# 4l3x4ndre/Metadata-Augmented-UNET-for-LST-NDVI

Hardware: AMD Instinct MI355X
Metric: train images/sec (256x256x6->2 U-Net, B=32/GPU) (higher is better)
Workload: dtype bf16; 1 GPU; metadata-unet base_filters=64, 32x6x256x256 tiles + 4-dim metadata per GPU, fwd+MSE+bwd+AdamW (src/train.py:243-256); global_batch=32, parallelism=dp1, sync_bn=False, launch=hipGraph replay of the captured step

## Files before the change

### include/mau_hip.h

```cpp
#ifndef MAU_HIP_H
#define MAU_HIP_H

#include <stddef.h>
#include <stdint.h>

#ifdef __cplusplus
extern "C" {
#endif

#define MAU_F32 0
#define MAU_BF16 1
#define MAU_F16 2

#define MAU_OK 0
#define MAU_ERR_ARG 1
#define MAU_ERR_HIP 2
#define MAU_ERR_DEVICE 3

typedef void* mau_stream_t;

#define MAU_ABI_VERSION 5
int mau_abi_version(void);
const char* mau_last_error(void);
int mau_device_check(void);

int mau_nchw_to_nhwc(const float* src, void* dst, int dtype, int N, int C, int H, int W, int ld,
                     mau_stream_t stream);
int mau_nhwc_to_nchw(const void* src, float* dst, int dtype, int N, int C, int H, int W, int ld,
                     mau_stream_t stream);

int mau_pack_tile_onehot(const unsigned char* cls_a, const unsigned char* cls_b, const float* cont,
                         const unsigned char* flip, void* out, int ldo, int dtype, int N, int H, int W,
                         int num_classes, int ncont, mau_stream_t stream);
int mau_flip_rows(const float* src, float* dst, const unsigned char* flip, int N, int C, int H, int W,
                  mau_stream_t stream);

int mau_conv3x3_kc(int dtype);
size_t mau_conv3x3_packed_elems(int dtype, int nout, int nin);
int mau_conv3x3_pack_weights(const float* w_oihw, void* wf, void* wd, int dtype, int Cout, int Cin,
                             mau_stream_t stream);
size_t mau_conv3x3_pack_desc_bytes(void);
int mau_conv3x3_pack_desc_fill(void* descs_host, int index, const float* w_oihw, void* wf, void* wd, int dtype, int Cout,
                               int Cin, int tile0, int* next_tile_host);
int mau_conv3x3_pack_weights_multi(const void* descs, int n, int total_tiles, int dtype, mau_stream_t stream);
int mau_conv3x3_num_pixel_tiles(int dtype, int N, int H, int W, int Cout);
int mau_conv3x3_fwd_pool(const void* x, int ldx, int C0, const void* wpk, const float* bias, const float* post_scale,
                         const float* post_shift, void* y, int ldy, int Cout, void* pooled, int ldpool, int dtype, int N, int H,
                         int W, mau_stream_t stream);
int mau_conv3x3_variant(int dtype, int N, int H, int W, int Cin, int Cout, int* tile_rows_host, int* waves_host, int* cout_block_host,
                        int* k_groups_host);
int mau_conv3x3_first_max_channels(void);
int mau_conv3x3_first_rows(int N, int H, int W);
size_t mau_conv3x3_first_wgrad_ws_elems(int N, int H, int W, int Cout);
int mau_conv3x3_first_wgrad(const void* x8, const void* dz, int lddz, float* dw_oihw, float* ws, int Cin, int Cout, int dtype, int N,
                            int H, int W, mau_stream_t stream);
int mau_conv3x3_first_fwd(const float* x_nchw, int Cin, const float* w_oihw, const float* bias, const float* post_scale,
                          const float* post_shift, void* y, int ldy, int Cout, float* slab, void* x8, int dtype, int N, int H,
                          int W, mau_stream_t stream);
int mau_conv3x3_fwd(const void* x, int ldx, int C0, const float* emb, void* emb_ws, int E, const void* wpk,
                    const float* bias, const float* post_scale, const float* post_shift, void* y, int ldy,
                    int Cout, float* slab, int dtype, int N, int H, int W, mau_stream_t stream);
int mau_conv3x3_fwd2(const void* x, int ldx, int C0, const void* x1, int ldx1, int C1, const float* emb, void* emb_ws,
                     int E, const void* wpk, const float* bias, const float* post_scale, const float* post_shift,
                     void* y, int ldy, int Cout, float* slab, int dtype, int N, int H, int W, mau_stream_t stream);
int mau_conv3x3_wgrad_splits(int dtype, int N, int H, int W, int Cout, int Cin);
size_t mau_conv3x3_wgrad_acc_elems(int dtype, int N, int H, int W, int Cout, int Cin);
int mau_conv3x3_wgrad(const void* x, int ldx, int C0, const float* emb, void* emb_ws, int E, const void* dy,
                      int lddy, int Cout, float* acc, int dtype, int N, int H, int W, mau_stream_t stream);
int mau_conv3x3_wgrad2(const void* x, int ldx, int C0, const void* x1, int ldx1, int C1, const float* emb, void* emb_ws,
                       int E, const void* dy, int lddy, int Cout, float* acc, int dtype, int N, int H, int W,
                       mau_stream_t stream);
int mau_conv3x3_unpack_wgrad(const float* acc, int nsplit, float* dw_oihw, int Cout, int Cin,
                             mau_stream_t stream);

size_t mau_reduce_rows_ws_elems(int rows, int M);
int mau_reduce_tickets_elems(void);
int mau_reduce_rows_f64(const float* slab, int rows, int M, int ldrow, double* sums, double* ws, unsigned* tickets,
                        mau_stream_t stream);
int mau_reduce_rows_f64_f32(const float* slab, int rows, int M, int ldrow, double* sums, float* sums32,
                            double* ws, unsigned* tickets, double append, mau_stream_t stream);
int mau_reduce_rows_f32(const float* slab, int rows, int M, int ldrow, float* out, double* ws, unsigned* tickets,
                        mau_stream_t stream);
int mau_bn_stats_sums_f64(const float* slab, int rows, int C, double* sums, double* ws, unsigned* tickets, double append,
                          mau_stream_t stream);
int mau_bn_finalize_train(const double* sums, double count, const float* gamma, const float* beta,
                          float* running_mean, float* running_var, int64_t* num_batches_tracked,
                          float momentum, float eps, float* scale, float* shift, float* mean,
                          float* invstd, int C, mau_stream_t stream);
size_t mau_bn_stats_ws_elems(int rows, int C);
int mau_bn_stats_finalize_train(const float* slab, int rows, double count, const float* gamma, const float* beta,
                                float* running_mean, float* running_var, int64_t* num_batches_tracked,
                                float momentum, float eps, float* scale, float* shift, float* mean, float* invstd,
                                double* ws, unsigned* tickets, int C, mau_stream_t stream);
int mau_bn_coeffs_eval(const float* gamma, const float* beta, const float* running_mean,
                       const float* running_var, float eps, float* scale, float* shift, float* mean,
                       float* invstd, int C, mau_stream_t stream);
int mau_bn_relu_apply(const void* y, int ldy, const float* scale, const float* shift, void* a, int lda,
                      int dtype, int64_t npix, int C, mau_stream_t stream);
int mau_bn_relu_apply_pool(const void* y, int ldy, const float* scale, const float* shift, void* a, int lda,
                           void* pooled, int ldp, unsigned short* argidx, int dtype, int N, int H, int W, int C,
                           mau_stream_t stream);
int mau_bn_relu_bwd_reduce(const void* da, int ldda, const void* y, int ldy, const float* scale,
                           const float* shift, const float* mean, const float* invstd, float* slab,
                           int ldslab, int dtype, int64_t npix, int C, mau_stream_t stream);
int mau_bn_relu_bwd_apply(const void* da, int ldda, const void* y, int ldy, const float* scale,
                          const float* shift, const float* mean, const float* invstd, const double* sums,
                          double count, void* dy, int lddy, int dtype, int64_t npix, int C,
                          mau_stream_t stream);
int mau_bn_bwd_rows(int64_t npix);

int mau_pool_bn_bwd_reduce(const void* y, int ldy, const void* dpl, int lddpl, const unsigned short* argidx,
                           const void* dskip, int lddskip,
                           const float* scale, const float* shift, const float* mean, const float* invstd, float* slab,
                           int ldslab, int dtype, int N, int H, int W, int C, mau_stream_t stream);
int mau_pool_bn_bwd_apply(const void* y, int ldy, const void* dpl, int lddpl, const unsigned short* argidx,
                          const void* dskip, int lddskip,
                          const float* scale, const float* shift, const float* mean, const float* invstd,
                          const double* sums, double count, void* dy, int lddy, int dtype, int N, int H, int W, int C,
                          mau_stream_t stream);
int mau_head_bn_max_channels(void);
int mau_head_bn_fwd(const void* y, int ldy, const float* scale, const float* shift, const float* w, const float* b, float* out,
                    int tanh0, int dtype, int N, int HW, int C, int Co, mau_stream_t stream);
int mau_head_bn_bwd_reduce(const void* y, int ldy, const float* scale, const float* shift, const float* mean,
                           const float* invstd, const float* w, const float* out, const float* dout, float* bn_slab,
                           int ldslab, float* head_slab, int tanh0, int dtype, int N, int HW, int C, int Co,
                           mau_stream_t stream);
int mau_head_bn_bwd_apply(const void* y, int ldy, const float* scale, const float* shift, const float* mean,
                          const float* invstd, const double* sums, double count, const float* w, const float* out,
                          const float* dout, void* dy, int lddy, int tanh0, int dtype, int N, int HW, int C, int Co,
                          mau_stream_t stream);

int mau_sum_tensors_max(void);
int mau_sum_tensors(const void* const* srcs, const int* lds, int k, void* dst, int lddst, int dtype, int64_t npix, int C,
                    mau_stream_t stream);

int mau_emb_fold_fwd(const float* w, const float* emb, float* weff, int Cout, int Ct, int E, int N, int Ep, mau_stream_t stream);
size_t mau_emb_fold_ws_elems(int Cout, int N, int E);
int mau_emb_fold_bwd(const float* w, const float* emb, const float* dweff, float* dw, float* demb, float* ws, int Cout, int Ct, int E,
                     int N, int Ep, mau_stream_t stream);

int mau_maxpool2x2_fwd(const void* x, int ldx, void* y, int ldy, int dtype, int N, int H, int W, int C,
                       mau_stream_t stream);
int mau_maxpool2x2_bwd(const void* x, int ldx, const void* dy, int lddy, void* dx, int lddx, int dtype,
                       int N, int H, int W, int C, mau_stream_t stream);
int mau_maxpool2x2_bwd_add(const void* x, int ldx, const void* dy, int lddy, const void* dskip, int lddskip, void* dx,
                           int lddx, int dtype, int N, int H, int W, int C, mau_stream_t stream);

int mau_resize_bilinear_fwd(const void* src, int ldsrc, int h, int w, void* dst, int lddst, int choff,
                            int dtype, int N, int H, int W, int C, mau_stream_t stream);
int mau_resize_bilinear_bn_fwd(const void* y, int ldy, int h, int w, const float* scale, const float* shift, void* dst,
                               int lddst, int choff, int dtype, int N, int H, int W, int C, mau_stream_t stream);
int mau_resize_bilinear_bwd(const void* ddst, int ldddst, int choff, int H, int W, void* dsrc, int lddsrc,
                            int dtype, int N, int h, int w, int C, mau_stream_t stream);
int mau_copy_channels(const void* src, int ldsrc, void* dst, int lddst, int choff, int zero_to, int dtype,
                      int64_t npix, int C, mau_stream_t stream);
int mau_bcast_fill(const float* emb, void* dst, int lddst, int choff, int zero_to, int dtype, int N, int HW,
                   int E, mau_stream_t stream);
size_t mau_bcast_bwd_ws_elems(int N, int HW, int E);
int mau_bcast_bwd(const void* dx, int lddx, int choff, float* demb, float* ws, int dtype, int N, int HW, int E,
                  mau_stream_t stream);

int mau_head_fwd(const void* a, int lda, const float* w, const float* b, float* out, int tanh0, int dtype,
                 int N, int HW, int C, int Co, mau_stream_t stream);
size_t mau_head_mean_ws_elems(int N, int HW, int Co);
int mau_head_mean(const void* a, int lda, const float* w, const float* b, const double* scale, const double* shift,
                  double* means, double* ws, unsigned* tickets, int tanh0, int dtype, int N, int HW, int C, int Co,
                  mau_stream_t stream);
int mau_head_bwd(const void* a, int lda, const float* w, const float* out, const float* dout, void* da,
                 int ldda, float* slab, int tanh0, int dtype, int N, int HW, int C, int Co,
                 mau_stream_t stream);
int mau_head_bwd_rows(int N, int HW);
int mau_head_bwd_rowlen(int C, int Co);

int mau_meta_mlp_fwd(const float* md, const float* w0, const float* b0, const float* w2, const float* b2,
                     float* hidden, float* emb, int N, int F, int Hd, int D, mau_stream_t stream);
int mau_meta_mlp_bwd(const float* md, const float* w0, const float* w2, const float* hidden,
                     const float* demb, float* dw0, float* db0, float* dw2, float* db2, float* dhidden_ws,
                     int N, int F, int Hd, int D, mau_stream_t stream);

int mau_lstm_max_hidden(void);
int mau_lstm_fwd(const float* x, const float* w_ih, const float* w_hh, const float* b_ih, const float* b_hh,
                 float* h_last, float* gates, float* cells, int B, int T, int H, mau_stream_t stream);
size_t mau_lstm_bwd_ws_elems(int B, int T, int H);
int mau_lstm_bwd(const float* x, const float* w_hh, const float* gates, const float* cells, const float* dh_last,
                 float* dw_ih, float* dw_hh, float* db_ih, float* db_hh, float* ws, int B, int T, int H,
                 mau_stream_t stream);

int mau_linear_fwd(const float* x, const float* w, const float* b, float* out, int N, int F, int D, mau_stream_t stream);
int mau_linear_bwd(const float* x, const float* w, const float* dout, float* dx, float* dw, float* db, int N, int F,
                   int D, mau_stream_t stream);

size_t mau_adamw_pack_desc_bytes(void);
int mau_adamw_pack_desc_fill(void* descs_host, int index, float* w, const float* grad, float* exp_avg, float* exp_avg_sq,
                             void* wf, void* wd, int Cout, int Cin, int tile0, int* next_tile_host);
int mau_adamw_pack_step(const void* descs, int n, int total_tiles, int dtype, const float* step, float lr, float beta1,
                        float beta2, float eps, float weight_decay, mau_stream_t stream);

#define MAU_OPT_ADAMW 0
#define MAU_OPT_ADAM 1
#define MAU_OPT_SGD 2
int mau_opt_pack_desc_fill(void* descs_host, int index, float* w, const float* grad, float* m, float* v, void* wf, void* wd,
                           int Cout, int Cin, int tile0, int* next_tile_host);
int mau_opt_pack_step(const void* descs, int n, int total_tiles, int dtype, int rule, const float* step, const float* grad_scale,
                      float lr, float beta1_or_momentum, float beta2, float eps, float weight_decay, int nesterov,
                      mau_stream_t stream);

int mau_grad_norm_chunk(void);
size_t mau_grad_norm_seg_bytes(void);
int mau_grad_norm_seg_fill(void* segs_host, int index, const float* ptr, int64_t n, int block0, int* next_block_host);
int mau_grad_norm_clip(const void* segs, int nsegs, int total_blocks, double* ws, unsigned* tickets, float max_norm,
                       float* norm_out, float* coef_out, mau_stream_t stream);

int mau_eval_metrics_row_elems(int ncls);
int mau_eval_metrics_chunks(int H, int W);
size_t mau_eval_metrics_ws_elems(int B, int C, int H, int W, int ncls);
int mau_eval_metrics(const float* out, const float* tgt, const unsigned char* cls, const double* scale, const double* shift,
                     double* rows, double* ws, unsigned* tickets, int B, int C, int H, int W, int ncls, mau_stream_t stream);

int mau_mse_blocks(int64_t n);
int mau_mse_fwd_bwd(const float* out, const float* tgt, double* partial, float* loss, float* dout, int64_t n,
                    mau_stream_t stream);

int mau_l1_gradient_blocks(int64_t n);
int mau_l1_gradient_loss(const float* out, const float* tgt, double* partial, float* terms, float* dout, float w_l1,
                         float w_grad, int B, int C, int H, int W, mau_stream_t stream);

size_t mau_ssim_ws_elems(int B, int C, int H, int W);
int mau_ssim_loss(const float* out, const float* tgt, double* ws, float* per_image, float* loss, int prep, int B, int C,
                  int H, int W, mau_stream_t stream);

#ifdef __cplusplus
}
#endif
#endif
```

### metadata-augmented-unet-for-lst-ndvi_amd/_lib.py

```python
from __future__ import annotations

import ctypes as C
import os

import torch

_HERE = os.path.dirname(os.path.abspath(__file__))
LIB_PATH = os.environ.get("MAU_LIB") or os.path.join(_HERE, "libmau_hip.so")

MAU_F32 = 0
MAU_BF16 = 1
MAU_F16 = 2
MAU_OPT_ADAMW, MAU_OPT_ADAM, MAU_OPT_SGD = 0, 1, 2

_p, _i, _i64, _f, _d, _sz = C.c_void_p, C.c_int, C.c_int64, C.c_float, C.c_double, C.c_size_t

PROTOTYPES = {
    "mau_abi_version": (_i, []),
    "mau_last_error": (C.c_char_p, []),
    "mau_device_check": (_i, []),
    "mau_nchw_to_nhwc": (_i, [_p, _p, _i, _i, _i, _i, _i, _i, _p]),
    "mau_pack_tile_onehot": (_i, [_p, _p, _p, _p, _p, _i, _i, _i, _i, _i, _i, _i, _p]),
    "mau_flip_rows": (_i, [_p, _p, _p, _i, _i, _i, _i, _p]),
    "mau_nhwc_to_nchw": (_i, [_p, _p, _i, _i, _i, _i, _i, _i, _p]),
    "mau_conv3x3_kc": (_i, [_i]),
    "mau_conv3x3_packed_elems": (_sz, [_i, _i, _i]),
    "mau_conv3x3_pack_weights": (_i, [_p, _p, _p, _i, _i, _i, _p]),
    "mau_conv3x3_pack_desc_bytes": (_sz, []),
    "mau_conv3x3_pack_desc_fill": (_i, [_p, _i, _p, _p, _p, _i, _i, _i, _i, _p]),
    "mau_conv3x3_pack_weights_multi": (_i, [_p, _i, _i, _i, _p]),
    "mau_conv3x3_num_pixel_tiles": (_i, [_i, _i, _i, _i, _i]),
    "mau_conv3x3_variant": (_i, [_i, _i, _i, _i, _i, _i, _p, _p, _p, _p]),
    "mau_conv3x3_first_max_channels": (_i, []),
    "mau_conv3x3_first_rows": (_i, [_i, _i, _i]),
    "mau_conv3x3_first_wgrad_ws_elems": (_sz, [_i, _i, _i, _i]),
    "mau_conv3x3_first_wgrad": (_i, [_p, _p, _i, _p, _p, _i, _i, _i, _i, _i, _i, _p]),
    "mau_conv3x3_first_fwd": (_i, [_p, _i, _p, _p, _p, _p, _p, _i, _i, _p, _p, _i, _i, _i, _i, _p]),
    "mau_conv3x3_fwd": (_i, [_p, _i, _i, _p, _p, _i, _p, _p, _p, _p, _p, _i, _i, _p, _i, _i, _i, _i, _p]),
    "mau_conv3x3_fwd_pool": (_i, [_p, _i, _i, _p, _p, _p, _p, _p, _i, _i, _p, _i, _i, _i, _i, _i, _p]),
    "mau_conv3x3_fwd2": (_i, [_p, _i, _i, _p, _i, _i, _p, _p, _i, _p, _p, _p, _p, _p, _i, _i, _p, _i, _i, _i, _i, _p]),
    "mau_conv3x3_wgrad_splits": (_i, [_i, _i, _i, _i, _i, _i]),
    "mau_conv3x3_wgrad_acc_elems": (_sz, [_i, _i, _i, _i, _i, _i]),
    "mau_conv3x3_wgrad": (_i, [_p, _i, _i, _p, _p, _i, _p, _i, _i, _p, _i, _i, _i, _i, _p]),
    "mau_conv3x3_wgrad2": (_i, [_p, _i, _i, _p, _i, _i, _p, _p, _i, _p, _i, _i, _p, _i, _i, _i, _i, _p]),
    "mau_conv3x3_unpack_wgrad": (_i, [_p, _i, _p, _i, _i, _p]),
    "mau_reduce_rows_ws_elems": (_sz, [_i, _i]),
    "mau_reduce_tickets_elems": (_i, []),
    "mau_reduce_rows_f64": (_i, [_p, _i, _i, _i, _p, _p, _p, _p]),
    "mau_reduce_rows_f64_f32": (_i, [_p, _i, _i, _i, _p, _p, _p, _p, _d, _p]),
    "mau_reduce_rows_f32": (_i, [_p, _i, _i, _i, _p, _p, _p, _p]),
    "mau_bn_stats_sums_f64": (_i, [_p, _i, _i, _p, _p, _p, _d, _p]),
    "mau_bn_finalize_train": (_i, [_p, _d, _p, _p, _p, _p, _p, _f, _f, _p, _p, _p, _p, _i, _p]),
    "mau_bn_stats_ws_elems": (_sz, [_i, _i]),
    "mau_bn_stats_finalize_train": (_i, [_p, _i, _d, _p, _p, _p, _p, _p, _f, _f, _p, _p, _p, _p, _p, _p, _i, _p]),
    "mau_bn_coeffs_eval": (_i, [_p, _p, _p, _p, _f, _p, _p, _p, _p, _i, _p]),
    "mau_bn_relu_apply": (_i, [_p, _i, _p, _p, _p, _i, _i, _i64, _i, _p]),
    "mau_bn_relu_apply_pool": (_i, [_p, _i, _p, _p, _p, _i, _p, _i, _p, _i, _i, _i, _i, _i, _p]),
    "mau_bn_relu_bwd_reduce": (_i, [_p, _i, _p, _i, _p, _p, _p, _p, _p, _i, _i, _i64, _i, _p]),
    "mau_bn_relu_bwd_apply": (_i, [_p, _i, _p, _i, _p, _p, _p, _p, _p, _d, _p, _i, _i, _i64, _i, _p]),
    "mau_bn_bwd_rows": (_i, [_i64]),
    "mau_pool_bn_bwd_reduce": (_i, [_p, _i, _p, _i, _p, _p, _i, _p, _p, _p, _p, _p, _i, _i, _i, _i, _i, _i, _p]),
    "mau_pool_bn_bwd_apply": (_i, [_p, _i, _p, _i, _p, _p, _i, _p, _p, _p, _p, _p, _d, _p, _i, _i, _i, _i, _i, _i, _p]),
    "mau_head_bn_max_channels": (_i, []),
    "mau_head_bn_fwd": (_i, [_p, _i, _p, _p, _p, _p, _p, _i, _i, _i, _i, _i, _i, _p]),
    "mau_head_bn_bwd_reduce": (_i, [_p, _i, _p, _p, _p, _p, _p, _p, _p, _p, _i, _p, _i, _i, _i, _i, _i, _i, _p]),
    "mau_head_bn_bwd_apply": (_i, [_p, _i, _p, _p, _p, _p, _p, _d, _p, _p, _p, _p, _i, _i, _i, _i, _i, _i, _i, _p]),
    "mau_resize_bilinear_bn_fwd": (_i, [_p, _i, _i, _i, _p, _p, _p, _i, _i, _i, _i, _i, _i, _i, _p]),
    "mau_maxpool2x2_fwd": (_i, [_p, _i, _p, _i, _i, _i, _i, _i, _i, _p]),
    "mau_maxpool2x2_bwd": (_i, [_p, _i, _p, _i, _p, _i, _i, _i, _i, _i, _i, _p]),
    "mau_maxpool2x2_bwd_add": (_i, [_p, _i, _p, _i, _p, _i, _p, _i, _i, _i, _i, _i, _i, _p]),
    "mau_resize_bilinear_fwd": (_i, [_p, _i, _i, _i, _p, _i, _i, _i, _i, _i, _i, _i, _p]),
    "mau_resize_bilinear_bwd": (_i, [_p, _i, _i, _i, _i, _p, _i, _i, _i, _i, _i, _i, _p]),
    "mau_copy_channels": (_i, [_p, _i, _p, _i, _i, _i, _i, _i64, _i, _p]),
    "mau_bcast_fill": (_i, [_p, _p, _i, _i, _i, _i, _i, _i, _i, _p]),
    "mau_bcast_bwd_ws_elems": (_sz, [_i, _i, _i]),
    "mau_bcast_bwd": (_i, [_p, _i, _i, _p, _p, _i, _i, _i, _i, _p]),
    "mau_head_fwd": (_i, [_p, _i, _p, _p, _p, _i, _i, _i, _i, _i, _i, _p]),
    "mau_head_mean_ws_elems": (_sz, [_i, _i, _i]),
    "mau_head_mean": (_i, [_p, _i, _p, _p, _p, _p, _p, _p, _p, _i, _i, _i, _i, _i, _i, _p]),
    "mau_head_bwd": (_i, [_p, _i, _p, _p, _p, _p, _i, _p, _i, _i, _i, _i, _i, _i, _p]),
    "mau_head_bwd_rows": (_i, [_i, _i]),
    "mau_head_bwd_rowlen": (_i, [_i, _i]),
    "mau_meta_mlp_fwd": (_i, [_p, _p, _p, _p, _p, _p, _p, _i, _i, _i, _i, _p]),
    "mau_meta_mlp_bwd": (_i, [_p, _p, _p, _p, _p, _p, _p, _p, _p, _p, _i, _i, _i, _i, _p]),
    "mau_lstm_max_hidden": (_i, []),
    "mau_lstm_fwd": (_i, [_p, _p, _p, _p, _p, _p, _p, _p, _i, _i, _i, _p]),
    "mau_lstm_bwd_ws_elems": (_sz, [_i, _i, _i]),
    "mau_lstm_bwd": (_i, [_p, _p, _p, _p, _p, _p, _p, _p, _p, _p, _i, _i, _i, _p]),
    "mau_linear_fwd": (_i, [_p, _p, _p, _p, _i, _i, _i, _p]),
    "mau_linear_bwd": (_i, [_p, _p, _p, _p, _p, _p, _i, _i, _i, _p]),
    "mau_adamw_pack_desc_bytes": (_sz, []),
    "mau_adamw_pack_desc_fill": (_i, [_p, _i, _p, _p, _p, _p, _p, _p, _i, _i, _i, _p]),
    "mau_adamw_pack_step": (_i, [_p, _i, _i, _i, _p, _f, _f, _f, _f, _f, _p]),
    "mau_opt_pack_desc_fill": (_i, [_p, _i, _p, _p, _p, _p, _p, _p, _i, _i, _i, _p]),
    "mau_opt_pack_step": (_i, [_p, _i, _i, _i, _i, _p, _p, _f, _f, _f, _f, _f, _i, _p]),
    "mau_grad_norm_chunk": (_i, []),
    "mau_grad_norm_seg_bytes": (_sz, []),
    "mau_grad_norm_seg_fill": (_i, [_p, _i, _p, _i64, _i, _p]),
    "mau_grad_norm_clip": (_i, [_p, _i, _i, _p, _p, _f, _p, _p, _p]),
    "mau_sum_tensors_max": (_i, []),
    "mau_sum_tensors": (_i, [_p, _p, _i, _p, _i, _i, _i64, _i, _p]),
    "mau_emb_fold_fwd": (_i, [_p, _p, _p, _i, _i, _i, _i, _i, _p]),
    "mau_emb_fold_ws_elems": (_sz, [_i, _i, _i]),
    "mau_emb_fold_bwd": (_i, [_p, _p, _p, _p, _p, _p, _i, _i, _i, _i, _i, _p]),
    "mau_eval_metrics_row_elems": (_i, [_i]),
    "mau_eval_metrics_chunks": (_i, [_i, _i]),
    "mau_eval_metrics_ws_elems": (_sz, [_i, _i, _i, _i, _i]),
    "mau_eval_metrics": (_i, [_p, _p, _p, _p, _p, _p, _p, _p, _i, _i, _i, _i, _i, _p]),
    "mau_mse_blocks": (_i, [_i64]),
    "mau_l1_gradient_blocks": (_i, [_i64]),
    "mau_l1_gradient_loss": (_i, [_p, _p, _p, _p, _p, _f, _f, _i, _i, _i, _i, _p]),
    "mau_ssim_ws_elems": (_sz, [_i, _i, _i, _i]),
    "mau_ssim_loss": (_i, [_p, _p, _p, _p, _p, _i, _i, _i, _i, _i, _p]),
    "mau_mse_fwd_bwd": (_i, [_p, _p, _p, _p, _p, _i64, _p]),
}


class MauError(RuntimeError):
    pass


def _load():
    if not os.path.exists(LIB_PATH):
        raise ImportError(
            f"{LIB_PATH} not found: the MI355X-native HIP library has not been built "
            f"(run `python -c 'import __graft_entry__ as g; g.build()'` or `make -C {os.path.join(_HERE, 'csrc')}`). "
            "There is no CPU or PyTorch fallback for this path.")
    lib = C.CDLL(LIB_PATH)
    missing = [n for n in PROTOTYPES if not hasattr(lib, n)]
    if missing:
        raise ImportError(f"{LIB_PATH} does not export {missing}; rebuild it")
    for name, (res, args) in PROTOTYPES.items():
        fn = getattr(lib, name)
        fn.restype = res
        fn.argtypes = args
    return lib


lib = _load()


def check(status: int, what: str = ""):
    if status != 0:
        msg = lib.mau_last_error()
        raise MauError(f"libmau_hip {what} failed (status {status}): {msg.decode() if msg else '?'}")


def conv3x3_variant(dtype: int, N: int, H: int, W: int, Cout: int, Cin: int = 0):
    th, nw, bn, kg = C.c_int(), C.c_int(), C.c_int(), C.c_int()
    check(lib.mau_conv3x3_variant(dtype, N, H, W, Cin, Cout, C.byref(th), C.byref(nw), C.byref(bn), C.byref(kg)), "mau_conv3x3_variant")
    return th.value, nw.value, bn.value, kg.value


def call(name: str, *args):
    check(getattr(lib, name)(*args), name)
```

### metadata-augmented-unet-for-lst-ndvi_amd/csrc/bn.hip

```cpp
#include <stdlib.h>
#include "mau_common.h"

namespace mau {

template <int G, typename Load>
__device__ __forceinline__ void ordered_group(int& k, int end, Load load, double& s0, double& s1) {
  for (; k + 8 * (G - 1) + 4 < end; k += 8 * G) {
    double a[G], b[G];
#pragma unroll
    for (int i = 0; i < G; ++i) {
      a[i] = load(k + 8 * i);
      b[i] = load(k + 8 * i + 4);
    }
#pragma unroll
    for (int i = 0; i < G; ++i) {
      s0 += a[i];
      s1 += b[i];
    }
  }
}
template <typename Load>
__device__ __forceinline__ void ordered_pair_sum(int first, int end, Load load, double& s0, double& s1) {
  int k = first;
#ifndef MAU_REDUCE_SERIAL
  ordered_group<16>(k, end, load, s0, s1);
  ordered_group<4>(k, end, load, s0, s1);
#endif
  for (; k + 4 < end; k += 8) {
    s0 += load(k);
    s1 += load(k + 4);
  }
  if (k < end) s0 += load(k);
}

template <typename InT, typename OutT>
__global__ __launch_bounds__(256) void reduce_rows_kernel(const InT* __restrict__ slab, int rows, int M, int ldrow,
                                                          OutT* __restrict__ out, int ldout, float* __restrict__ out32) {
  __shared__ double part[4][64];
  const int col = blockIdx.x * 64 + (threadIdx.x & 63);
  const int rl = threadIdx.x >> 6;
  const int per = (rows + gridDim.y - 1) / gridDim.y;
  const int r0 = blockIdx.y * per, r1 = min(rows, r0 + per);
  double s0 = 0.0, s1 = 0.0;
  if (col < M) {
    if (r0 + rl < r1) ordered_pair_sum(r0 + rl, r1, [&](int r) { return (double)slab[(size_t)r * ldrow + col]; }, s0, s1);
  }
  part[rl][threadIdx.x & 63] = s0 + s1;
  __syncthreads();
  if (rl == 0 && col < M) {
    const double v = part[0][threadIdx.x] + part[1][threadIdx.x] + part[2][threadIdx.x] + part[3][threadIdx.x];
    out[(size_t)blockIdx.y * ldout + col] = (OutT)v;
    if (out32 != nullptr) out32[col] = (float)v;
  }
}

constexpr int REDUCE_MAX_CHUNKS = 128;
static int reduce_chunks(int rows) {
  int c = rows / 32;
  if (c > REDUCE_MAX_CHUNKS) c = REDUCE_MAX_CHUNKS;
  return c < 1 ? 1 : c;
}

template <typename OutT>
static int reduce_rows_launch(const float* slab, int rows, int M, int ldrow, OutT* out, double* ws, hipStream_t st,
                              float* out32 = nullptr) {
  const int chunks = reduce_chunks(rows);
  float* const none = nullptr;
  if (chunks == 1 || ws == nullptr) {
    MAU_LAUNCH((reduce_rows_kernel<float, OutT>), dim3(ceil_div(M, 64), 1), dim3(256), 0, st, slab, rows, M, ldrow, out, M, out32);
  } else {
    MAU_LAUNCH((reduce_rows_kernel<float, double>), dim3(ceil_div(M, 64), chunks), dim3(256), 0, st, slab, rows, M, ldrow, ws, M, none);
    MAU_LAUNCH((reduce_rows_kernel<double, OutT>), dim3(ceil_div(M, 64), 1), dim3(256), 0, st, (const double*)ws, chunks, M, M, out, M, out32);
  }
  return check_launch("reduce_rows_kernel");
}


template <typename OutT>
__global__ __launch_bounds__(256) void reduce_rows_fused_kernel(const float* __restrict__ slab, int rows, int M, int ldrow, int split,
                                                                int gap, double* __restrict__ part, unsigned* __restrict__ tickets,
                                                                OutT* __restrict__ out, float* __restrict__ out32, double append) {
  __shared__ double ps[4][64];
  const int cl = threadIdx.x & 63, rl = threadIdx.x >> 6;
  const int j = blockIdx.x * 64 + cl;
  const int col = j < split ? j : j - split + gap;
  const int chunks = gridDim.y;
  const int per = (rows + chunks - 1) / chunks;
  const int r0 = blockIdx.y * per, r1 = min(rows, r0 + per);
  double s0 = 0.0, s1 = 0.0;
  if (j < M) {
    if (r0 + rl < r1) ordered_pair_sum(r0 + rl, r1, [&](int r) { return (double)slab[(size_t)r * ldrow + col]; }, s0, s1);
  }
  ps[rl][cl] = s0 + s1;
  __syncthreads();
  if (rl == 0 && j < M) part[(size_t)blockIdx.y * M + j] = ps[0][cl] + ps[1][cl] + ps[2][cl] + ps[3][cl];
  if (!last_block_of(tickets + blockIdx.x, (unsigned)chunks)) return;
  s0 = s1 = 0.0;
  if (j < M) {
    if (rl < chunks) ordered_pair_sum(rl, chunks, [&](int k) { return part[(size_t)k * M + j]; }, s0, s1);
  }
  ps[rl][cl] = s0 + s1;
  __syncthreads();
  if (rl == 0 && j < M) {
    const double v = ps[0][cl] + ps[1][cl] + ps[2][cl] + ps[3][cl];
    out[j] = (OutT)v;
    if (out32 != nullptr) out32[j] = (float)v;
  }
  if (append > 0.0 && blockIdx.x == 0 && threadIdx.x == 0) out[M] = (OutT)append;
}

template <typename OutT>
static int reduce_rows_fused_launch(const float* slab, int rows, int M, int ldrow, int split, int gap, OutT* out, double* ws,
                                    unsigned* tickets, hipStream_t st, float* out32 = nullptr, double append = 0.0) {
  const int chunks = reduce_chunks(rows);
  MAU_LAUNCH((reduce_rows_fused_kernel<OutT>), dim3(ceil_div(M, 64), chunks), dim3(256), 0, st, slab, rows, M, ldrow, split, gap, ws,
             tickets, out, out32, append);
  return check_launch("reduce_rows_fused_kernel");
}

__global__ void bn_finalize_train_kernel(const double* __restrict__ sums, double count, const float* __restrict__ gamma,
                                         const float* __restrict__ beta, float* __restrict__ rmean, float* __restrict__ rvar,
                                         int64_t* nbt, float momentum, float eps, float* __restrict__ scale,
                                         float* __restrict__ shift, float* __restrict__ mean_o, float* __restrict__ invstd_o,
                                         int C) {
  const int c = blockIdx.x * blockDim.x + threadIdx.x;
  if (c == 0 && nbt) *nbt += 1;
  if (c >= C) return;
  if (count <= 0.0) count = sums[2 * C];
  const double mean = sums[c] / count;
  double var = sums[C + c] / count - mean * mean;
  if (var < 0.0) var = 0.0;
  const float invstd = (float)(1.0 / sqrt(var + (double)eps));
  const float sc = gamma[c] * invstd;
  scale[c] = sc;
  shift[c] = beta[c] - (float)mean * sc;
  mean_o[c] = (float)mean;
  invstd_o[c] = invstd;
  if (rmean) {
    const double unbiased = count > 1.0 ? var * (count / (count - 1.0)) : var;
    rmean[c] = (1.f - momentum) * rmean[c] + momentum * (float)mean;
    rvar[c] = (1.f - momentum) * rvar[c] + momentum * (float)unbiased;
  }
}

__global__ __launch_bounds__(256) void bn_finalize_from_partials_kernel(const double* __restrict__ part, int chunks, int ldp, double count,
                                                 const float* __restrict__ gamma, const float* __restrict__ beta,
                                                 float* __restrict__ rmean, float* __restrict__ rvar, int64_t* nbt, float momentum,
                                                 float eps, float* __restrict__ scale, float* __restrict__ shift,
                                                 float* __restrict__ mean_o, float* __restrict__ invstd_o, int C) {
  __shared__ double ps[4][64], pq[4][64];
  const int cl = threadIdx.x & 63, kl = threadIdx.x >> 6;
  const int c = blockIdx.x * 64 + cl;
  if (blockIdx.x == 0 && threadIdx.x == 0 && nbt) *nbt += 1;
  double s0 = 0.0, q0 = 0.0, s1 = 0.0, q1 = 0.0;
  if (c < C && kl < chunks) {
    ordered_pair_sum(kl, chunks, [&](int k) { return part[(size_t)k * 2 * ldp + c]; }, s0, s1);
    ordered_pair_sum(kl, chunks, [&](int k) { return part[(size_t)k * 2 * ldp + ldp + c]; }, q0, q1);
  }
  ps[kl][cl] = s0 + s1;
  pq[kl][cl] = q0 + q1;
  __syncthreads();
  if (kl != 0 || c >= C) return;
  const double s = (ps[0][cl] + ps[1][cl]) + (ps[2][cl] + ps[3][cl]);
  const double q = (pq[0][cl] + pq[1][cl]) + (pq[2][cl] + pq[3][cl]);
  const double mean = s / count;
  double var = q / count - mean * mean;
  if (var < 0.0) var = 0.0;
  const float invstd = (float)(1.0 / sqrt(var + (double)eps));
  const float sc = gamma[c] * invstd;
  scale[c] = sc;
  shift[c] = beta[c] - (float)mean * sc;
  mean_o[c] = (float)mean;
  invstd_o[c] = invstd;
  if (rmean) {
    const double unbiased = count > 1.0 ? var * (count / (count - 1.0)) : var;
    rmean[c] = (1.f - momentum) * rmean[c] + momentum * (float)mean;
    rvar[c] = (1.f - momentum) * rvar[c] + momentum * (float)unbiased;
  }
}

__global__ __launch_bounds__(256) void bn_stats_finalize_fused_kernel(const float* __restrict__ slab, int rows, int cpad,
                                                                      double* __restrict__ part, unsigned* __restrict__ tickets,
                                                                      double count, const float* __restrict__ gamma,
                                                                      const float* __restrict__ beta, float* __restrict__ rmean,
                                                                      float* __restrict__ rvar, int64_t* nbt, float momentum,
                                                                      float eps, float* __restrict__ scale, float* __restrict__ shift,
                                                                      float* __restrict__ mean_o, float* __restrict__ invstd_o, int C) {
  __shared__ double ps[4][64], pq[4][64];
  const int cl = threadIdx.x & 63, kl = threadIdx.x >> 6;
  const int c = blockIdx.x * 64 + cl;
  const int chunks = gridDim.y, ld = 2 * cpad;
  const int per = (rows + chunks - 1) / chunks;
  const int r0 = blockIdx.y * per, r1 = min(rows, r0 + per);
  double s0 = 0.0, q0 = 0.0, s1 = 0.0, q1 = 0.0;
  if (r0 + kl < r1) {
    ordered_pair_sum(r0 + kl, r1, [&](int r) { return (double)slab[(size_t)r * ld + c]; }, s0, s1);
    ordered_pair_sum(r0 + kl, r1, [&](int r) { return (double)slab[(size_t)r * ld + cpad + c]; }, q0, q1);
  }
  ps[kl][cl] = s0 + s1;
  pq[kl][cl] = q0 + q1;
  __syncthreads();
  if (kl == 0) {
    part[(size_t)blockIdx.y * ld + c] = ps[0][cl] + ps[1][cl] + ps[2][cl] + ps[3][cl];
    part[(size_t)blockIdx.y * ld + cpad + c] = pq[0][cl] + pq[1][cl] + pq[2][cl] + pq[3][cl];
  }
  if (!last_block_of(tickets + blockIdx.x, (unsigned)chunks)) return;
  if (blockIdx.x == 0 && threadIdx.x == 0 && nbt) *nbt += 1;
  s0 = q0 = s1 = q1 = 0.0;
  if (c < C && kl < chunks) {
    ordered_pair_sum(kl, chunks, [&](int k) { return part[(size_t)k * ld + c]; }, s0, s1);
    ordered_pair_sum(kl, chunks, [&](int k) { return part[(size_t)k * ld + cpad + c]; }, q0, q1);
  }
  ps[kl][cl] = s0 + s1;
  pq[kl][cl] = q0 + q1;
  __syncthreads();
  if (kl != 0 || c >= C) return;
  const double s = (ps[0][cl] + ps[1][cl]) + (ps[2][cl] + ps[3][cl]);
  const double q = (pq[0][cl] + pq[1][cl]) + (pq[2][cl] + pq[3][cl]);
  const double mean = s / count;
  double var = q / count - mean * mean;
  if (var < 0.0) var = 0.0;
  const float invstd = (float)(1.0 / sqrt(var + (double)eps));
  const float sc = gamma[c] * invstd;
  scale[c] = sc;
  shift[c] = beta[c] - (float)mean * sc;
  mean_o[c] = (float)mean;
  invstd_o[c] = invstd;
  if (rmean) {
    const double unbiased = count > 1.0 ? var * (count / (count - 1.0)) : var;
    rmean[c] = (1.f - momentum) * rmean[c] + momentum * (float)mean;
    rvar[c] = (1.f - momentum) * rvar[c] + momentum * (float)unbiased;
  }
}

__global__ void bn_coeffs_eval_kernel(const float* __restrict__ gamma, const float* __restrict__ beta,
                                      const float* __restrict__ rmean, const float* __restrict__ rvar, float eps,
                                      float* __restrict__ scale, float* __restrict__ shift, float* __restrict__ mean_o,
                                      float* __restrict__ invstd_o, int C) {
  const int c = blockIdx.x * blockDim.x + threadIdx.x;
  if (c >= C) return;
  const float is = 1.f / sqrtf(rvar[c] + eps);
  const float sc = gamma[c] * is;
  scale[c] = sc;
  shift[c] = beta[c] - rmean[c] * sc;
  if (mean_o) mean_o[c] = rmean[c];
  if (invstd_o) invstd_o[c] = is;
}

struct PixVec {
  int nvl, PS, v, ps;
  __device__ __forceinline__ PixVec(int nv) {
    nvl = nv < 256 ? nv : 256;
    PS = 256 / nvl;
    v = threadIdx.x % nvl;
    ps = threadIdx.x / nvl;
  }
};
static inline int pixvec_pixels_per_block(int nv, int64_t npix, int max_per_thread, int min_blocks = 2048) {
  const int nvl = nv < 256 ? nv : 256;
  const int ps = 256 / nvl;
  int per_thread = max_per_thread;
  while (per_thread > 8 && npix / ((int64_t)ps * per_thread) < min_blocks) per_thread >>= 1;
  return ps * per_thread;
}

template <typename T>
__global__ __launch_bounds__(256) void bn_relu_apply_kernel(const T* __restrict__ y, int ldy, const float* __restrict__ scale,
                                                            const float* __restrict__ shift, T* __restrict__ a, int lda,
                                                            int64_t npix, int C, int C8, int pixb) {
  const int nv = C8 >> 3;
  const PixVec m(nv);
  if (m.ps >= m.PS) return;
  const int64_t p0 = (int64_t)blockIdx.x * pixb;
  const int64_t p1 = p0 + pixb < npix ? p0 + pixb : npix;
  for (int vv = m.v; vv < nv; vv += m.nvl) {
    const int c = vv * 8;
    float sc[8], sh[8];
#pragma unroll
    for (int j = 0; j < 8; ++j) {
      sc[j] = coef(scale, c + j, C);
      sh[j] = coef(shift, c + j, C);
    }
    int64_t pix = p0 + m.ps;
    for (; pix + 3 * m.PS < p1; pix += 4 * m.PS) {
      F8 v[4];
#pragma unroll
      for (int u = 0; u < 4; ++u) v[u] = load8<T>(y + (pix + u * m.PS) * ldy + c);
#pragma unroll
      for (int u = 0; u < 4; ++u) {
        F8 o;
#pragma unroll
        for (int j = 0; j < 8; ++j) o.v[j] = fmaxf(fmaf(v[u].v[j], sc[j], sh[j]), 0.f);
        store8<T>(a + (pix + u * m.PS) * lda + c, o);
      }
    }
    for (; pix < p1; pix += m.PS) {
      const F8 v = load8<T>(y + pix * ldy + c);
      F8 o;
#pragma unroll
      for (int j = 0; j < 8; ++j) o.v[j] = fmaxf(fmaf(v.v[j], sc[j], sh[j]), 0.f);
      store8<T>(a + pix * lda + c, o);
    }
  }
}

template <typename T>
__global__ __launch_bounds__(256) void bn_relu_apply_pool_kernel(const T* __restrict__ y, int ldy, const float* __restrict__ scale,
                                                                 const float* __restrict__ shift, T* __restrict__ a, int lda,
                                                                 T* __restrict__ pl, int ldp, unsigned short* __restrict__ argidx, int H, int W,
                                                                 int C, int C8) {
  const int nv = C8 >> 3, Wc = (W + 1) >> 1, Ho = H >> 1, Wo = W >> 1;
  const int idx = blockIdx.x * 256 + threadIdx.x;
  if (idx >= Wc * nv) return;
  const int xo = idx / nv, c = (idx - xo * nv) * 8;
  const int yo = blockIdx.y, n = blockIdx.z;
  float sc[8], sh[8];
#pragma unroll
  for (int j = 0; j < 8; ++j) {
    sc[j] = coef(scale, c + j, C);
    sh[j] = coef(shift, c + j, C);
  }
  const int y0 = 2 * yo, x0 = 2 * xo;
  const bool hasx = x0 + 1 < W, hasy = y0 + 1 < H;
  const size_t row0 = ((size_t)n * H + y0) * W, row1 = row0 + W;
  F8 v[4];
  v[0] = load8<T>(y + (row0 + x0) * ldy + c);
  v[1] = hasx ? load8<T>(y + (row0 + x0 + 1) * ldy + c) : zero8();
  v[2] = hasy ? load8<T>(y + (row1 + x0) * ldy + c) : zero8();
  v[3] = (hasx && hasy) ? load8<T>(y + (row1 + x0 + 1) * ldy + c) : zero8();
  F8 o[4];
#pragma unroll
  for (int u = 0; u < 4; ++u)
#pragma unroll
    for (int j = 0; j < 8; ++j) o[u].v[j] = fmaxf(fmaf(v[u].v[j], sc[j], sh[j]), 0.f);
  store8<T>(a + (row0 + x0) * lda + c, o[0]);
  if (hasx) store8<T>(a + (row0 + x0 + 1) * lda + c, o[1]);
  if (hasy) store8<T>(a + (row1 + x0) * lda + c, o[2]);
  if (hasx && hasy) store8<T>(a + (row1 + x0 + 1) * lda + c, o[3]);
  if (yo < Ho && xo < Wo) {
    F8 m;
    unsigned bits = 0;
#pragma unroll
    for (int j = 0; j < 8; ++j) {
      const float a0 = opaque((float)(T)opaque(o[0].v[j])), a1 = opaque((float)(T)opaque(o[1].v[j]));
      const float a2 = opaque((float)(T)opaque(o[2].v[j])), a3 = opaque((float)(T)opaque(o[3].v[j]));
      unsigned arg = 0;
      float mx = a0;
      arg = a1 > mx ? 1u : arg;
      mx = fmaxf(mx, a1);
      arg = a2 > mx ? 2u : arg;
      mx = fmaxf(mx, a2);
      arg = a3 > mx ? 3u : arg;
      mx = fmaxf(mx, a3);
      m.v[j] = mx;
      bits |= arg << (2 * j);
    }
    store8<T>(pl + (((size_t)n * Ho + yo) * Wo + xo) * ldp + c, m);
    if (argidx != nullptr) argidx[(((size_t)n * Ho + yo) * Wo + xo) * nv + (c >> 3)] = (unsigned short)bits;
  }
}


template <typename T>
__global__ __launch_bounds__(256) void bn_relu_bwd_reduce_kernel(const T* __restrict__ da, int ldda, const T* __restrict__ y,
                                                                 int ldy, const float* __restrict__ scale,
                                                                 const float* __restrict__ shift, const float* __restrict__ mean,
                                                                 const float* __restrict__ invstd, float* __restrict__ slab,
                                                                 int ldslab, int64_t npix, int C) {
  __shared__ float red[2][32][64 + 1];
  const int cv = threadIdx.x & 7, ps = threadIdx.x >> 3;
  const int c0 = blockIdx.y * 64 + cv * 8;
  const int64_t p0 = (int64_t)blockIdx.x * BWD_PIX_PER_BLOCK;
  const int64_t p1 = p0 + BWD_PIX_PER_BLOCK < npix ? p0 + BWD_PIX_PER_BLOCK : npix;
  float s1[8], s2[8], sc[8], sh[8], mu[8], is[8];
#pragma unroll
  for (int j = 0; j < 8; ++j) {
    s1[j] = s2[j] = 0.f;
    const int cc = c0 + j;
    sc[j] = coef(scale, cc, C);
    sh[j] = coef(shift, cc, C);
    mu[j] = coef(mean, cc, C);
    is[j] = coef(invstd, cc, C);
  }
  if (c0 < C) {
    int64_t p = p0 + ps;
    for (; p + 32 < p1; p += 64) {
      F8 g[2], v[2];
#pragma unroll
      for (int u = 0; u < 2; ++u) {
        g[u] = load8<T>(da + (p + 32 * u) * ldda + c0);
        v[u] = load8<T>(y + (p + 32 * u) * ldy + c0);
      }
#pragma unroll
      for (int u = 0; u < 2; ++u)
#pragma unroll
        for (int j = 0; j < 8; ++j) {
          const float act = fmaf(v[u].v[j], sc[j], sh[j]);
          const float dz = act > 0.f ? g[u].v[j] : 0.f;
          s1[j] += dz;
          s2[j] = fmaf(dz, (v[u].v[j] - mu[j]) * is[j], s2[j]);
        }
    }
    for (; p < p1; p += 32) {
      const F8 g = load8<T>(da + p * ldda + c0);
      const F8 v = load8<T>(y + p * ldy + c0);
#pragma unroll
      for (int j = 0; j < 8; ++j) {
        const float act = fmaf(v.v[j], sc[j], sh[j]);
        const float dz = act > 0.f ? g.v[j] : 0.f;
        s1[j] += dz;
        s2[j] = fmaf(dz, (v.v[j] - mu[j]) * is[j], s2[j]);
      }
    }
  }
#pragma unroll
  for (int j = 0; j < 8; ++j) {
    red[0][ps][cv * 8 + j] = s1[j];
    red[1][ps][cv * 8 + j] = s2[j];
  }
  __syncthreads();
  if (threadIdx.x < 128) {
    const int which = threadIdx.x >> 6, c = threadIdx.x & 63;
    float s = 0.f;
#pragma unroll 8
    for (int r = 0; r < 32; ++r) s += red[which][r][c];
    const int cc = blockIdx.y * 64 + c;
    if (cc < ldslab) slab[((size_t)blockIdx.x * 2 + which) * ldslab + cc] = s;
  }
}

template <typename T, bool NT>
__global__ __launch_bounds__(256) void bn_relu_bwd_apply_kernel(const T* __restrict__ da, int ldda, const T* __restrict__ y,
                                                                int ldy, const float* __restrict__ scale,
                                                                const float* __restrict__ shift, const float* __restrict__ mean,
                                                                const float* __restrict__ invstd, const double* __restrict__ sums,
                                                                double inv_count, T* __restrict__ dy, int lddy, int64_t npix,
                                                                int C, int C8, int pixb) {
  const int nv = C8 >> 3;
  const PixVec m(nv);
  if (m.ps >= m.PS) return;
  if (inv_count <= 0.0) inv_count = 1.0 / sums[2 * C];
  const int64_t p0 = (int64_t)blockIdx.x * pixb;
  const int64_t p1 = p0 + pixb < npix ? p0 + pixb : npix;
  for (int vv = m.v; vv < nv; vv += m.nvl) {
    const int c = vv * 8;
    float sc[8], sh[8], k0[8], k1[8];
    double d1[8], d2[8];
#pragma unroll
    for (int j = 0; j < 8; ++j) {
      sc[j] = coef(scale, c + j, C);
      sh[j] = coef(shift, c + j, C);
      k0[j] = coef(mean, c + j, C);
      k1[j] = coef(invstd, c + j, C);
      d1[j] = coef(sums, c + j, C);
      d2[j] = coef(sums + C, c + j, C);
    }
#pragma unroll
    for (int j = 0; j < 8; ++j) {
      const float mu = k0[j], is = k1[j];
      const float m1 = (float)(d1[j] * inv_count), m2 = (float)(d2[j] * inv_count);
      k1[j] = __fmul_rn(__fmul_rn(sc[j], m2), is);
      k0[j] = fmaf(sc[j], m1, -__fmul_rn(k1[j], mu));
    }
    int64_t pix = p0 + m.ps;
    for (; pix + 3 * m.PS < p1; pix += 4 * m.PS) {
      F8 g[4], v[4];
#pragma unroll
      for (int u = 0; u < 4; ++u) {
        g[u] = NT ? load8_nt<T>(da + (pix + u * m.PS) * ldda + c) : load8<T>(da + (pix + u * m.PS) * ldda + c);
        v[u] = NT ? load8_nt<T>(y + (pix + u * m.PS) * ldy + c) : load8<T>(y + (pix + u * m.PS) * ldy + c);
      }
#pragma unroll
      for (int u = 0; u < 4; ++u) {
        F8 o;
#pragma unroll
        for (int j = 0; j < 8; ++j) {
          const float act = fmaf(v[u].v[j], sc[j], sh[j]);
          const float dz = act > 0.f ? g[u].v[j] : 0.f;
          o.v[j] = fmaf(sc[j], dz, -fmaf(k1[j], v[u].v[j], k0[j]));
        }
        if (NT) store8_nt<T>(dy + (pix + u * m.PS) * lddy + c, o); else store8<T>(dy + (pix + u * m.PS) * lddy + c, o);
      }
    }
    for (; pix < p1; pix += m.PS) {
      const F8 g = load8<T>(da + pix * ldda + c);
      const F8 v = load8<T>(y + pix * ldy + c);
      F8 o;
#pragma unroll
      for (int j = 0; j < 8; ++j) {
        const float act = fmaf(v.v[j], sc[j], sh[j]);
        const float dz = act > 0.f ? g.v[j] : 0.f;
        o.v[j] = fmaf(sc[j], dz, -fmaf(k1[j], v.v[j], k0[j]));
      }
      store8<T>(dy + pix * lddy + c, o);
    }
  }
}

}

using namespace mau;

extern "C" {

size_t mau_reduce_rows_ws_elems(int rows, int M) { return (size_t)reduce_chunks(rows) * M; }

int mau_reduce_tickets_elems(void) { return 64; }

#define MAU_REQUIRE_TICKETS(M) MAU_REQUIRE(tickets == nullptr || ceil_div((M), 64) <= mau_reduce_tickets_elems(), "reduce_rows: more than 4096 columns")

int mau_reduce_rows_f64(const float* slab, int rows, int M, int ldrow, double* sums, double* ws, unsigned* tickets,
                        mau_stream_t stream) {
  MAU_REQUIRE(slab && sums && rows > 0 && M > 0 && ldrow >= M, "reduce_rows: bad arguments");
  MAU_REQUIRE_TICKETS(M);
  if (tickets && ws) return reduce_rows_fused_launch<double>(slab, rows, M, ldrow, M, 0, sums, ws, tickets, (hipStream_t)stream);
  return reduce_rows_launch<double>(slab, rows, M, ldrow, sums, ws, (hipStream_t)stream);
}

int mau_reduce_rows_f64_f32(const float* slab, int rows, int M, int ldrow, double* sums, float* sums32, double* ws,
                            unsigned* tickets, double append, mau_stream_t stream) {
  MAU_REQUIRE(slab && sums && sums32 && rows > 0 && M > 0 && ldrow >= M, "reduce_rows: bad arguments");
  MAU_REQUIRE_TICKETS(M);
  MAU_REQUIRE(append <= 0.0 || (tickets && ws), "reduce_rows: the appended count needs the single-launch form (ws and tickets)");
  if (tickets && ws)
    return reduce_rows_fused_launch<double>(slab, rows, M, ldrow, M, 0, sums, ws, tickets, (hipStream_t)stream, sums32, append);
  return reduce_rows_launch<double>(slab, rows, M, ldrow, sums, ws, (hipStream_t)stream, sums32);
}

int mau_reduce_rows_f32(const float* slab, int rows, int M, int ldrow, float* out, double* ws, unsigned* tickets,
                        mau_stream_t stream) {
  MAU_REQUIRE(slab && out && rows > 0 && M > 0 && ldrow >= M, "reduce_rows: bad arguments");
  MAU_REQUIRE_TICKETS(M);
  if (tickets && ws) return reduce_rows_fused_launch<float>(slab, rows, M, ldrow, M, 0, out, ws, tickets, (hipStream_t)stream);
  return reduce_rows_launch<float>(slab, rows, M, ldrow, out, ws, (hipStream_t)stream);
}

int mau_bn_stats_sums_f64(const float* slab, int rows, int C, double* sums, double* ws, unsigned* tickets, double append,
                          mau_stream_t stream) {
  MAU_REQUIRE(slab && sums && ws && tickets && rows > 0 && C > 0, "bn_stats_sums: bad arguments");
  MAU_REQUIRE_TICKETS(2 * C);
  const int cpad = round_up(C, 64);
  return reduce_rows_fused_launch<double>(slab, rows, 2 * C, 2 * cpad, C, cpad, sums, ws, tickets, (hipStream_t)stream, nullptr, append);
}

int mau_bn_finalize_train(const double* sums, double count, const float* gamma, const float* beta,
                          float* running_mean, float* running_var, int64_t* nbt, float momentum, float eps,
                          float* scale, float* shift, float* mean, float* invstd, int C, mau_stream_t stream) {
  MAU_REQUIRE(sums && gamma && beta && scale && shift && mean && invstd && C > 0 && count >= 0, "bn_finalize_train: bad arguments");
  MAU_REQUIRE((running_mean == nullptr) == (running_var == nullptr), "bn_finalize_train: running_mean/var must come together");
  MAU_LAUNCH(bn_finalize_train_kernel, dim3(ceil_div(C, 256)), dim3(256), 0, (hipStream_t)stream, sums, count, gamma,
                     beta, running_mean, running_var, nbt, momentum, eps, scale, shift, mean, invstd, C);
  return check_launch("bn_finalize_train_kernel");
}

size_t mau_bn_stats_ws_elems(int rows, int C) { return (size_t)reduce_chunks(rows) * 2 * round_up(C, 64); }

int mau_bn_stats_finalize_train(const float* slab, int rows, double count, const float* gamma, const float* beta,
                                float* running_mean, float* running_var, int64_t* nbt, float momentum, float eps,
                                float* scale, float* shift, float* mean, float* invstd, double* ws, unsigned* tickets, int C,
                                mau_stream_t stream) {
  MAU_REQUIRE(slab && ws && gamma && beta && scale && shift && mean && invstd && rows > 0 && C > 0 && count > 0, "bn_stats_finalize_train: bad arguments");
  MAU_REQUIRE((running_mean == nullptr) == (running_var == nullptr), "bn_stats_finalize_train: running_mean/var must come together");
  hipStream_t st = (hipStream_t)stream;
  const int cpad = round_up(C, 64), M = 2 * cpad, chunks = reduce_chunks(rows);
  MAU_REQUIRE_TICKETS(cpad);
  if (tickets) {
    MAU_LAUNCH(bn_stats_finalize_fused_kernel, dim3(cpad / 64, chunks), dim3(256), 0, st, slab, rows, cpad, ws, tickets, count, gamma,
               beta, running_mean, running_var, nbt, momentum, eps, scale, shift, mean, invstd, C);
    return check_launch("bn_stats_finalize_fused_kernel");
  }
  MAU_LAUNCH((reduce_rows_kernel<float, double>), dim3(ceil_div(M, 64), chunks), dim3(256), 0, st, slab, rows, M, M, ws, M, (float*)nullptr);
  MAU_LAUNCH(bn_finalize_from_partials_kernel, dim3(ceil_div(C, 64)), dim3(256), 0, st, (const double*)ws, chunks, cpad, count, gamma,
             beta, running_mean, running_var, nbt, momentum, eps, scale, shift, mean, invstd, C);
  return check_launch("bn_stats_finalize_train");
}

int mau_bn_coeffs_eval(const float* gamma, const float* beta, const float* running_mean, const float* running_var,
                       float eps, float* scale, float* shift, float* mean, float* invstd, int C, mau_stream_t stream) {
  MAU_REQUIRE(gamma && beta && running_mean && running_var && scale && shift && C > 0, "bn_coeffs_eval: bad arguments");
  MAU_LAUNCH(bn_coeffs_eval_kernel, dim3(ceil_div(C, 256)), dim3(256), 0, (hipStream_t)stream, gamma, beta,
                     running_mean, running_var, eps, scale, shift, mean, invstd, C);
  return check_launch("bn_coeffs_eval_kernel");
}

int mau_bn_relu_apply(const void* y, int ldy, const float* scale, const float* shift, void* a, int lda, int dtype,
                      int64_t npix, int C, mau_stream_t stream) {
  MAU_REQUIRE(y && a && scale && shift && npix > 0 && C > 0, "bn_relu_apply: bad arguments");
  const int C8 = round_up(C, 8);
  MAU_REQUIRE(ldy % 8 == 0 && lda % 8 == 0 && ldy >= C8 && lda >= C8, "bn_relu_apply: bad ld");
  const bool big = npix >= (int64_t)1 << 20;
  const int pixb = pixvec_pixels_per_block(C8 / 8, npix, big ? 8 : 32, big ? 2048 : 256);
  MAU_DISPATCH_DTYPE(dtype, MAU_LAUNCH(bn_relu_apply_kernel<T>, dim3(ceil_div(npix, pixb)), dim3(256), 0, (hipStream_t)stream,
                                               (const T*)y, ldy, scale, shift, (T*)a, lda, npix, C, C8, pixb));
  return check_launch("bn_relu_apply_kernel");
}

int mau_bn_relu_apply_pool(const void* y, int ldy, const float* scale, const float* shift, void* a, int lda, void* pooled,
                           int ldp, unsigned short* argidx, int dtype, int N, int H, int W, int C, mau_stream_t stream) {
  MAU_REQUIRE(y && a && pooled && scale && shift && N > 0 && H >= 2 && W >= 2 && C > 0, "bn_relu_apply_pool: bad arguments");
  const int C8 = round_up(C, 8);
  MAU_REQUIRE(ldy % 8 == 0 && lda % 8 == 0 && ldp % 8 == 0 && ldy >= C8 && lda >= C8 && ldp >= C8, "bn_relu_apply_pool: bad ld");
  MAU_REQUIRE((H + 1) / 2 <= 65535 && N <= 65535, "bn_relu_apply_pool: H/2 and N must fit a grid dimension");
  dim3 grid(ceil_div(((W + 1) / 2) * (C8 / 8), 256), (H + 1) / 2, N);
  MAU_DISPATCH_DTYPE(dtype, MAU_LAUNCH(bn_relu_apply_pool_kernel<T>, grid, dim3(256), 0, (hipStream_t)stream, (const T*)y, ldy, scale,
                                       shift, (T*)a, lda, (T*)pooled, ldp, argidx, H, W, C, C8));
  return check_launch("bn_relu_apply_pool_kernel");
}

int mau_bn_bwd_rows(int64_t npix) { return ceil_div(npix, BWD_PIX_PER_BLOCK); }

int mau_bn_relu_bwd_reduce(const void* da, int ldda, const void* y, int ldy, const float* scale, const float* shift,
                           const float* mean, const float* invstd, float* slab, int ldslab, int dtype, int64_t npix,
                           int C, mau_stream_t stream) {
  MAU_REQUIRE(da && y && scale && shift && mean && invstd && slab && npix > 0 && C > 0, "bn_relu_bwd_reduce: bad arguments");
  MAU_REQUIRE(ldda % 8 == 0 && ldy % 8 == 0 && ldslab >= C, "bn_relu_bwd_reduce: bad ld");
  dim3 grid(mau_bn_bwd_rows(npix), ceil_div(C, 64));
  MAU_DISPATCH_DTYPE(dtype, MAU_LAUNCH(bn_relu_bwd_reduce_kernel<T>, grid, dim3(256), 0, (hipStream_t)stream,
                                               (const T*)da, ldda, (const T*)y, ldy, scale, shift, mean, invstd, slab,
                                               ldslab, npix, C));
  return check_launch("bn_relu_bwd_reduce_kernel");
}

int mau_bn_relu_bwd_apply(const void* da, int ldda, const void* y, int ldy, const float* scale, const float* shift,
                          const float* mean, const float* invstd, const double* sums, double count, void* dy, int lddy,
                          int dtype, int64_t npix, int C, mau_stream_t stream) {
  MAU_REQUIRE(da && y && dy && sums && npix > 0 && C > 0 && count >= 0, "bn_relu_bwd_apply: bad arguments");
  const int C8 = round_up(C, 8);
  MAU_REQUIRE(ldda % 8 == 0 && ldy % 8 == 0 && lddy % 8 == 0 && lddy >= C8, "bn_relu_bwd_apply: bad ld");
  const int pixb = pixvec_pixels_per_block(C8 / 8, npix, 64, 256);
  MAU_DISPATCH_DTYPE(dtype, MAU_LAUNCH((bn_relu_bwd_apply_kernel<T, false>), dim3(ceil_div(npix, pixb)), dim3(256), 0, (hipStream_t)stream,
                                               (const T*)da, ldda, (const T*)y, ldy, scale, shift, mean, invstd, sums,
                                               count > 0 ? 1.0 / count : 0.0, (T*)dy, lddy, npix, C, C8, pixb));
  return check_launch("bn_relu_bwd_apply_kernel");
}

}
```

### metadata-augmented-unet-for-lst-ndvi_amd/csrc/bn_fused.hip

```cpp
#include "mau_common.h"

namespace mau {

template <typename T>
__device__ __forceinline__ float round_to(float v) {
  return opaque((float)(T)opaque(v));
}

typedef float f2 __attribute__((ext_vector_type(2)));
__device__ __forceinline__ f2 pk_fma(f2 a, f2 b, f2 c) { return __builtin_elementwise_fma(a, b, c); }
__device__ __forceinline__ f2 splat(float v) { return f2{v, v}; }
template <typename T>
__device__ __forceinline__ f2 round_to2(f2 v) {
  if constexpr (sizeof(T) == 4) return v;
  else if constexpr (__is_same(T, bf16)) {
    typedef __bf16 b2 __attribute__((ext_vector_type(2)));
    asm("" : "+v"(v));
    f2 r = __builtin_convertvector(__builtin_convertvector(v, b2), f2);
    asm("" : "+v"(r));
    return r;
  } else return f2{round_to<T>(v[0]), round_to<T>(v[1])};
}
template <typename T>
struct P4 {
  f2 p[4];
  __device__ __forceinline__ static P4 load(const T* ptr) {
    const F8 v = load8<T>(ptr);
    P4 r;
#pragma unroll
    for (int i = 0; i < 4; ++i) r.p[i] = f2{v.v[2 * i], v.v[2 * i + 1]};
    return r;
  }
};

struct Coef8 {
  float sc[8], sh[8], mu[8], is[8];
  __device__ __forceinline__ void load(const float* scale, const float* shift, const float* mean, const float* invstd, int c0, int C) {
#pragma unroll
    for (int j = 0; j < 8; ++j) {
      sc[j] = coef(scale, c0 + j, C);
      sh[j] = coef(shift, c0 + j, C);
      mu[j] = mean ? coef(mean, c0 + j, C) : 0.f;
      is[j] = invstd ? coef(invstd, c0 + j, C) : 0.f;
    }
  }
};

template <typename T>
struct PoolLoads {
  F8 g, sk;
  unsigned bits;
  bool inpool;
  int me;
};
template <typename T, bool POOL, bool SKIP>
__device__ __forceinline__ PoolLoads<T> pool_load(const T* __restrict__ dpl, int lddpl, const unsigned short* __restrict__ argidx, int nv,
                                                  const T* __restrict__ dskip, int lddskip, int n, int yi, int xi, int H, int W, int c0) {
  PoolLoads<T> L;
  const int Ho = H >> 1, Wo = W >> 1, yo = yi >> 1, xo = xi >> 1;
  L.inpool = POOL && yo < Ho && xo < Wo;
  L.me = (yi & 1) * 2 + (xi & 1);
  L.bits = 0;
  if constexpr (POOL) {
    const int yc = yo < Ho ? yo : Ho - 1, xc = xo < Wo ? xo : Wo - 1;
    const size_t win = ((size_t)n * Ho + yc) * Wo + xc;
    L.g = load8<T>(dpl + win * lddpl + c0);
    L.bits = argidx[win * nv + (c0 >> 3)];
  }
  if constexpr (SKIP) L.sk = load8<T>(dskip + (((size_t)n * H + yi) * W + xi) * lddskip + c0);
  return L;
}
template <typename T, bool POOL, bool SKIP>
__device__ __forceinline__ F8 pool_eval(const PoolLoads<T>& L) {
  F8 o;
#pragma unroll
  for (int j = 0; j < 8; ++j) {
    float r = 0.f;
    if constexpr (POOL) r = (L.inpool && (int)((L.bits >> (2 * j)) & 3u) == L.me) ? L.g.v[j] : 0.f;
    if constexpr (SKIP) r += L.sk.v[j];
    o.v[j] = round_to<T>(r);
  }
  return o;
}

__device__ __forceinline__ void bn_sums_to_slab(float (*red)[32][64 + 1], const float* s1, const float* s2, int cv, int ps, float* slab,
                                                int ldslab) {
#pragma unroll
  for (int j = 0; j < 8; ++j) {
    red[0][ps][cv * 8 + j] = s1[j];
    red[1][ps][cv * 8 + j] = s2[j];
  }
  __syncthreads();
  if (threadIdx.x < 128) {
    const int which = threadIdx.x >> 6, c = threadIdx.x & 63;
    float s = 0.f;
#pragma unroll 8
    for (int r = 0; r < 32; ++r) s += red[which][r][c];
    const int cc = blockIdx.y * 64 + c;
    if (cc < ldslab) slab[((size_t)blockIdx.x * 2 + which) * ldslab + cc] = s;
  }
}

__device__ __forceinline__ void advance32(int& n, int& yi, int& xi, int H, int W) {
  xi += 32;
  while (xi >= W) {
    xi -= W;
    if (++yi == H) {
      yi = 0;
      ++n;
    }
  }
}
template <typename T, bool POOL, bool SKIP>
__global__ __launch_bounds__(256) void pool_bn_bwd_reduce_kernel(const T* __restrict__ y, int ldy, const T* __restrict__ dpl, int lddpl,
                                                                 const unsigned short* __restrict__ argidx,
                                                                 const T* __restrict__ dskip, int lddskip, const float* __restrict__ scale,
                                                                 const float* __restrict__ shift, const float* __restrict__ mean,
                                                                 const float* __restrict__ invstd, float* __restrict__ slab, int ldslab,
                                                                 int H, int W, int64_t npix, int C) {
  __shared__ float red[2][32][64 + 1];
  const int cv = threadIdx.x & 7, ps = threadIdx.x >> 3;
  const int c0 = blockIdx.y * 64 + cv * 8;
  const int64_t p0 = (int64_t)blockIdx.x * BWD_PIX_PER_BLOCK;
  const int64_t p1 = p0 + BWD_PIX_PER_BLOCK < npix ? p0 + BWD_PIX_PER_BLOCK : npix;
  Coef8 k;
  k.load(scale, shift, mean, invstd, c0, C);
  float s1[8], s2[8];
#pragma unroll
  for (int j = 0; j < 8; ++j) s1[j] = s2[j] = 0.f;
  auto accumulate = [&](const F8& v, const F8& g) {
#pragma unroll
    for (int j = 0; j < 8; ++j) {
      const float act = fmaf(v.v[j], k.sc[j], k.sh[j]);
      const float dz = act > 0.f ? g.v[j] : 0.f;
      s1[j] += dz;
      s2[j] = fmaf(dz, (v.v[j] - k.mu[j]) * k.is[j], s2[j]);
    }
  };
  if (c0 < C) {
    int64_t p = p0 + ps;
    const int HW = H * W, nv = (C + 7) >> 3;
    int n = (int)(p / HW), r = (int)(p - (int64_t)n * HW);
    int yi = r / W, xi = r - yi * W;
    for (; p + 32 < p1; p += 64) {
      int n2 = n, yi2 = yi, xi2 = xi;
      advance32(n2, yi2, xi2, H, W);
      const F8 va = load8<T>(y + p * ldy + c0), vb = load8<T>(y + (p + 32) * ldy + c0);
      const PoolLoads<T> La = pool_load<T, POOL, SKIP>(dpl, lddpl, argidx, nv, dskip, lddskip, n, yi, xi, H, W, c0);
      const PoolLoads<T> Lb = pool_load<T, POOL, SKIP>(dpl, lddpl, argidx, nv, dskip, lddskip, n2, yi2, xi2, H, W, c0);
      accumulate(va, pool_eval<T, POOL, SKIP>(La));
      accumulate(vb, pool_eval<T, POOL, SKIP>(Lb));
      n = n2, yi = yi2, xi = xi2;
      advance32(n, yi, xi, H, W);
    }
    for (; p < p1; p += 32) {
      const F8 v = load8<T>(y + p * ldy + c0);
      const PoolLoads<T> L = pool_load<T, POOL, SKIP>(dpl, lddpl, argidx, nv, dskip, lddskip, n, yi, xi, H, W, c0);
      accumulate(v, pool_eval<T, POOL, SKIP>(L));
      advance32(n, yi, xi, H, W);
    }
  }
  bn_sums_to_slab(red, s1, s2, cv, ps, slab, ldslab);
}

struct Apply8 {
  float sc[8], sh[8], k0[8], k1[8];
  __device__ __forceinline__ void load(const float* scale, const float* shift, const float* mean, const float* invstd, const double* sums,
                                       double inv_count, int c0, int C) {
    double d1[8], d2[8];
#pragma unroll
    for (int j = 0; j < 8; ++j) {
      sc[j] = coef(scale, c0 + j, C);
      sh[j] = coef(shift, c0 + j, C);
      k0[j] = coef(mean, c0 + j, C);
      k1[j] = coef(invstd, c0 + j, C);
      d1[j] = coef(sums, c0 + j, C);
      d2[j] = coef(sums + C, c0 + j, C);
    }
#pragma unroll
    for (int j = 0; j < 8; ++j) {
      const float mu = k0[j], is = k1[j];
      const float m1 = (float)(d1[j] * inv_count), m2 = (float)(d2[j] * inv_count);
      k1[j] = __fmul_rn(__fmul_rn(sc[j], m2), is);
      k0[j] = fmaf(sc[j], m1, -__fmul_rn(k1[j], mu));
    }
  }
  __device__ __forceinline__ float dy(int j, float yv, float da) const {
    const float act = fmaf(yv, sc[j], sh[j]);
    const float dz = act > 0.f ? da : 0.f;
    return fmaf(sc[j], dz, -fmaf(k1[j], yv, k0[j]));
  }
};

template <typename T, bool POOL, bool SKIP>
__global__ __launch_bounds__(256) void pool_bn_bwd_apply_kernel(const T* __restrict__ y, int ldy, const T* __restrict__ dpl, int lddpl,
                                                                const unsigned short* __restrict__ argidx,
                                                                const T* __restrict__ dskip, int lddskip, const float* __restrict__ scale,
                                                                const float* __restrict__ shift, const float* __restrict__ mean,
                                                                const float* __restrict__ invstd, const double* __restrict__ sums,
                                                                double inv_count, T* __restrict__ dyo, int lddy, int H, int W, int C, int C8,
                                                                int RY) {
  const int nv = C8 >> 3, Wc = (W + 1) >> 1, Hc = (H + 1) >> 1, Ho = H >> 1, Wo = W >> 1;
  const int idx = blockIdx.x * 256 + threadIdx.x;
  if (idx >= Wc * nv) return;
  const int xo = idx / nv, c = (idx - xo * nv) * 8;
  const int n = blockIdx.z;
  if (inv_count <= 0.0) inv_count = 1.0 / sums[2 * C];
  Apply8 k;
  k.load(scale, shift, mean, invstd, sums, inv_count, c, C);
  const int x0 = 2 * xo;
  const bool hasx = x0 + 1 < W;
  const int x1 = hasx ? x0 + 1 : x0;
  const int xpc = xo < Wo ? xo : Wo - 1;
  for (int yo = blockIdx.y * RY; yo < min(Hc, (int)(blockIdx.y + 1) * RY); ++yo) {
    const int y0 = 2 * yo;
    const bool hasy = y0 + 1 < H;
    const size_t row0 = ((size_t)n * H + y0) * W, row1 = ((size_t)n * H + (hasy ? y0 + 1 : y0)) * W;
    F8 v[4], d[4], g;
    v[0] = load8<T>(y + (row0 + x0) * ldy + c);
    v[1] = load8<T>(y + (row0 + x1) * ldy + c);
    v[2] = load8<T>(y + (row1 + x0) * ldy + c);
    v[3] = load8<T>(y + (row1 + x1) * ldy + c);
    if constexpr (SKIP) {
      d[0] = load8<T>(dskip + (row0 + x0) * lddskip + c);
      d[1] = load8<T>(dskip + (row0 + x1) * lddskip + c);
      d[2] = load8<T>(dskip + (row1 + x0) * lddskip + c);
      d[3] = load8<T>(dskip + (row1 + x1) * lddskip + c);
    }
    const bool inpool = POOL && yo < Ho && xo < Wo;
    unsigned bits = 0;
    if constexpr (POOL) {
      const size_t win = ((size_t)n * Ho + (yo < Ho ? yo : Ho - 1)) * Wo + xpc;
      g = load8<T>(dpl + win * lddpl + c);
      bits = argidx[win * nv + (c >> 3)];
    }
    F8 o[4];
#pragma unroll
    for (int j = 0; j < 8; ++j) {
      const int arg = inpool ? (int)((bits >> (2 * j)) & 3u) : -1;
#pragma unroll
      for (int u = 0; u < 4; ++u) {
        float r = 0.f;
        if constexpr (POOL) r = arg == u ? g.v[j] : 0.f;
        if constexpr (SKIP) r += d[u].v[j];
        o[u].v[j] = k.dy(j, v[u].v[j], round_to<T>(r));
      }
    }
    store8<T>(dyo + (row0 + x0) * lddy + c, o[0]);
    if (hasx) store8<T>(dyo + (row0 + x0 + 1) * lddy + c, o[1]);
    if (hasy) store8<T>(dyo + (row1 + x0) * lddy + c, o[2]);
    if (hasx && hasy) store8<T>(dyo + (row1 + x0 + 1) * lddy + c, o[3]);
  }
}

__device__ __forceinline__ void pos_step32(int& n, int& q, int HW) {
  q += 32;
  const bool w = q >= HW;
  q -= w ? HW : 0;
  n += w ? 1 : 0;
}

template <typename T, int MC, bool EX, bool BN = true>
__global__ __launch_bounds__(256) void head_bn_fwd_kernel(const T* __restrict__ y, int ldy, const float* __restrict__ scale,
                                                          const float* __restrict__ shift, const float* __restrict__ w,
                                                          const float* __restrict__ b, float* __restrict__ out, int tanh0, int HW, int C,
                                                          int Co, int64_t npix, int pixb) {
  const int sub = threadIdx.x & 7, ps = threadIdx.x >> 3;
  float wr[MC][8];
#pragma unroll
  for (int o = 0; o < MC; ++o)
#pragma unroll
    for (int j = 0; j < 8; ++j) wr[o][j] = (EX || o < Co) ? coef(w + o * C, sub * 8 + j, C) : 0.f;
  Coef8 k;
  if (BN) k.load(scale, shift, nullptr, nullptr, sub * 8, C);
  float bo[MC];
#pragma unroll
  for (int o = 0; o < MC; ++o) bo[o] = (EX || o < Co) ? b[o] : 0.f;
  const int64_t p0 = (int64_t)blockIdx.x * pixb;
  const int64_t p1 = p0 + pixb < npix ? p0 + pixb : npix;
  int n = (int)((p0 + ps) / HW);
  int q = (int)((p0 + ps) - (int64_t)n * HW);
  for (int64_t p = p0 + ps; p - ps < p1; p += 128) {
    F8 x[4];
    int nn[4], qq[4];
#pragma unroll
    for (int u = 0; u < 4; ++u) {
      const int64_t pix = p + 32 * u;
      const int64_t pc = pix < npix ? pix : npix - 1;
      x[u] = load8<T>(y + pc * ldy + (sub * 8 < C ? sub * 8 : 0));
      nn[u] = n;
      qq[u] = q;
      pos_step32(n, q, HW);
    }
    float acc[4][MC];
#pragma unroll
    for (int u = 0; u < 4; ++u) {
#pragma unroll
      for (int o = 0; o < MC; ++o) acc[u][o] = 0.f;
      if (sub * 8 < C) {
#pragma unroll
        for (int j = 0; j < 8; ++j) {
          const float a = BN ? round_to<T>(fmaxf(fmaf(x[u].v[j], k.sc[j], k.sh[j]), 0.f)) : x[u].v[j];
#pragma unroll
          for (int o = 0; o < MC; ++o) acc[u][o] = fmaf(a, wr[o][j], acc[u][o]);
        }
      }
#pragma unroll
      for (int o = 0; o < MC; ++o) {
        acc[u][o] += __shfl_xor(acc[u][o], 1);
        acc[u][o] += __shfl_xor(acc[u][o], 2);
        acc[u][o] += __shfl_xor(acc[u][o], 4);
      }
    }
    const int us = sub & 3;
    const int nu = us == 0 ? nn[0] : us == 1 ? nn[1] : us == 2 ? nn[2] : nn[3];
    const int qu = us == 0 ? qq[0] : us == 1 ? qq[1] : us == 2 ? qq[2] : qq[3];
    const bool live = sub < 4 && p + 32 * us < p1;
#pragma unroll
    for (int o = 0; o < MC; ++o) {
      if (EX || o < Co) {
        float r = us == 0 ? acc[0][o] : us == 1 ? acc[1][o] : us == 2 ? acc[2][o] : acc[3][o];
        r += bo[o];
        if (o == 0 && tanh0) r = tanhf(r);
        if (live) out[((size_t)nu * Co + o) * HW + qu] = r;
      }
    }
  }
}

template <int MC, bool EX>
__device__ __forceinline__ void head_dz(const float* __restrict__ out, const float* __restrict__ dout, int tanh0, int Co, int HW, int n,
                                        int q, float* dz) {
  const size_t base = (size_t)n * Co * HW + q;
  const float t = out[base];
  const float f0 = tanh0 ? fmaf(-t, t, 1.f) : 1.f;
#pragma unroll
  for (int o = 0; o < MC; ++o) {
    const float g = dout[base + (size_t)((EX || o < Co) ? o : Co - 1) * HW];
    dz[o] = (EX || o < Co) ? (o == 0 ? g * f0 : g) : 0.f;
  }
}

#ifndef MAU_HEAD_WAVES
#define MAU_HEAD_WAVES 3
#endif
template <typename T, int MC, bool EX>
__global__ __launch_bounds__(256, MAU_HEAD_WAVES) void head_bn_bwd_reduce_kernel(const T* __restrict__ y, int ldy, const float* __restrict__ scale,
                                                                 const float* __restrict__ shift, const float* __restrict__ mean,
                                                                 const float* __restrict__ invstd, const float* __restrict__ w,
                                                                 const float* __restrict__ out, const float* __restrict__ dout,
                                                                 float* __restrict__ bn_slab, int ldslab, float* __restrict__ head_slab,
                                                                 int tanh0, int HW, int C, int C8, int Co, int64_t npix) {
  __shared__ float red[2][32][64 + 1];
  __shared__ float hred[32 * HEAD_MAX_CO * 65];
  const int cv = threadIdx.x & 7, ps = threadIdx.x >> 3;
  const int c0 = cv * 8;
  const int64_t p0 = (int64_t)blockIdx.x * BWD_PIX_PER_BLOCK;
  const int64_t p1 = p0 + BWD_PIX_PER_BLOCK < npix ? p0 + BWD_PIX_PER_BLOCK : npix;
  const int rowlen = Co * (C8 + 8);
  float* row = head_slab + (size_t)blockIdx.x * rowlen;
  Coef8 k;
  k.load(scale, shift, mean, invstd, c0, C);
  f2 sc2[4], sh2[4], mu2[4], is2[4], s1p[4], s2p[4], dwq[MC][4], wq[MC][4];
  float dbp[MC];
#pragma unroll
  for (int i = 0; i < 4; ++i) {
    sc2[i] = f2{k.sc[2 * i], k.sc[2 * i + 1]};
    sh2[i] = f2{k.sh[2 * i], k.sh[2 * i + 1]};
    mu2[i] = f2{k.mu[2 * i], k.mu[2 * i + 1]};
    is2[i] = f2{k.is[2 * i], k.is[2 * i + 1]};
    s1p[i] = s2p[i] = f2{0.f, 0.f};
  }
#pragma unroll
  for (int o = 0; o < MC; ++o) {
    dbp[o] = 0.f;
#pragma unroll
    for (int i = 0; i < 4; ++i) {
      dwq[o][i] = f2{0.f, 0.f};
      wq[o][i] = f2{o < Co ? coef(w + o * C, c0 + 2 * i, C) : 0.f, o < Co ? coef(w + o * C, c0 + 2 * i + 1, C) : 0.f};
    }
  }
  auto one = [&](const P4<T>& v, const float* dz) {
#pragma unroll
    for (int o = 0; o < MC; ++o) dbp[o] += dz[o];
#pragma unroll
    for (int i = 0; i < 4; ++i) {
      const f2 act = pk_fma(v.p[i], sc2[i], sh2[i]);
      const f2 a = round_to2<T>(f2{fmaxf(act[0], 0.f), fmaxf(act[1], 0.f)});
      f2 s = f2{0.f, 0.f};
#pragma unroll
      for (int o = 0; o < MC; ++o)
        if (EX || o < Co) {
          s = pk_fma(splat(dz[o]), wq[o][i], s);
          dwq[o][i] = pk_fma(splat(dz[o]), a, dwq[o][i]);
        }
      const f2 da = round_to2<T>(s);
      const f2 dzb = f2{act[0] > 0.f ? da[0] : 0.f, act[1] > 0.f ? da[1] : 0.f};
      s1p[i] += dzb;
      s2p[i] = pk_fma(dzb, (v.p[i] - mu2[i]) * is2[i], s2p[i]);
    }
  };
  struct Raw {
    P4<T> v;
    float t, g[MC];
  };
  auto fetch = [&](int64_t pa, int na, int qa, Raw& r) {
    r.v = P4<T>::load(y + pa * ldy + c0);
    const size_t base = (size_t)na * Co * HW + qa;
    r.t = out[base];
#pragma unroll
    for (int o = 0; o < MC; ++o) r.g[o] = dout[base + (size_t)((EX || o < Co) ? o : Co - 1) * HW];
  };
  auto eval = [&](const Raw& r) {
    float dz[MC];
    const float f0 = tanh0 ? fmaf(-r.t, r.t, 1.f) : 1.f;
#pragma unroll
    for (int o = 0; o < MC; ++o) dz[o] = (EX || o < Co) ? (o == 0 ? r.g[o] * f0 : r.g[o]) : 0.f;
    one(r.v, dz);
  };
  if (c0 < C8) {
    int n = (int)((p0 + ps) / HW);
    int q = (int)((p0 + ps) - (int64_t)n * HW);
    int64_t p = p0 + ps;
    if (p + 32 < p1) {
      Raw a, b;
      int n2 = n, q2 = q;
      pos_step32(n2, q2, HW);
      fetch(p, n, q, a);
      fetch(p + 32, n2, q2, b);
      n = n2;
      q = q2;
      pos_step32(n, q, HW);
      for (; p + 96 < p1; p += 64) {
        Raw na, nb;
        n2 = n;
        q2 = q;
        pos_step32(n2, q2, HW);
        fetch(p + 64, n, q, na);
        fetch(p + 96, n2, q2, nb);
        eval(a);
        eval(b);
        a = na;
        b = nb;
        n = n2;
        q = q2;
        pos_step32(n, q, HW);
      }
      eval(a);
      eval(b);
      p += 64;
    }
    for (; p < p1; p += 32) {
      Raw r;
      fetch(p, n, q, r);
      eval(r);
      pos_step32(n, q, HW);
    }
  }
  float s1[8], s2[8], dwp[MC][8];
#pragma unroll
  for (int i = 0; i < 4; ++i) {
    s1[2 * i] = s1p[i][0];
    s1[2 * i + 1] = s1p[i][1];
    s2[2 * i] = s2p[i][0];
    s2[2 * i + 1] = s2p[i][1];
#pragma unroll
    for (int o = 0; o < MC; ++o) {
      dwp[o][2 * i] = dwq[o][i][0];
      dwp[o][2 * i + 1] = dwq[o][i][1];
    }
  }
#pragma unroll
  for (int o = 0; o < MC; ++o)
    if (EX || o < Co) {
#pragma unroll
      for (int j = 0; j < 8; ++j) hred[(ps * HEAD_MAX_CO + o) * 65 + cv * 8 + j] = dwp[o][j];
    }
  __syncthreads();
  for (int t = threadIdx.x; t < Co * 64; t += 256) {
    const int o = t >> 6, c = t & 63;
    float s = 0.f;
    for (int r = 0; r < 32; ++r) s += hred[(r * HEAD_MAX_CO + o) * 65 + c];
    if (c < C8) row[o * (C8 + 8) + c] = s;
  }
  __syncthreads();
  if (cv == 0) {
#pragma unroll
    for (int o = 0; o < MC; ++o)
      if (o < Co) hred[ps * HEAD_MAX_CO + o] = dbp[o];
  }
  __syncthreads();
  if (threadIdx.x < Co) {
    float s = 0.f;
    for (int r = 0; r < 32; ++r) s += hred[r * HEAD_MAX_CO + threadIdx.x];
    row[threadIdx.x * (C8 + 8) + C8] = s;
  }
  bn_sums_to_slab(red, s1, s2, cv, ps, bn_slab, ldslab);
}

template <typename T, int MC, bool EX>
__global__ __launch_bounds__(256) void head_bn_bwd_apply_kernel(const T* __restrict__ y, int ldy, const float* __restrict__ scale,
                                                                const float* __restrict__ shift, const float* __restrict__ mean,
                                                                const float* __restrict__ invstd, const double* __restrict__ sums,
                                                                double inv_count, const float* __restrict__ w, const float* __restrict__ out,
                                                                const float* __restrict__ dout, T* __restrict__ dyo, int lddy, int tanh0,
                                                                int HW, int C, int Co, int64_t npix, int pixb) {
  const int cv = threadIdx.x & 7, ps = threadIdx.x >> 3;
  const int c0 = cv * 8;
  if (c0 >= ((C + 7) & ~7)) return;
  if (inv_count <= 0.0) inv_count = 1.0 / sums[2 * C];
  Apply8 k;
  k.load(scale, shift, mean, invstd, sums, inv_count, c0, C);
  float wr[MC][8];
#pragma unroll
  for (int o = 0; o < MC; ++o)
#pragma unroll
    for (int j = 0; j < 8; ++j) wr[o][j] = o < Co ? coef(w + o * C, c0 + j, C) : 0.f;
  const int64_t p0 = (int64_t)blockIdx.x * pixb;
  const int64_t p1 = p0 + pixb < npix ? p0 + pixb : npix;
  int n = (int)((p0 + ps) / HW);
  int q = (int)((p0 + ps) - (int64_t)n * HW);
  auto one = [&](int64_t p, const F8& v, const float* dz) {
    F8 o8;
#pragma unroll
    for (int j = 0; j < 8; ++j) {
      float s = 0.f;
#pragma unroll
      for (int o = 0; o < MC; ++o)
        if (EX || o < Co) s = fmaf(dz[o], wr[o][j], s);
      o8.v[j] = k.dy(j, v.v[j], round_to<T>(s));
    }
    store8<T>(dyo + p * lddy + c0, o8);
  };
  int64_t p = p0 + ps;
  for (; p + 96 < p1; p += 128) {
    int nn[4], qq[4];
    F8 v[4];
    float dz[4][MC];
#pragma unroll
    for (int u = 0; u < 4; ++u) {
      nn[u] = n;
      qq[u] = q;
      pos_step32(n, q, HW);
    }
#pragma unroll
    for (int u = 0; u < 4; ++u) {
      v[u] = load8<T>(y + (p + 32 * u) * ldy + c0);
      head_dz<MC, EX>(out, dout, tanh0, Co, HW, nn[u], qq[u], dz[u]);
    }
#pragma unroll
    for (int u = 0; u < 4; ++u) one(p + 32 * u, v[u], dz[u]);
  }
  for (; p < p1; p += 32) {
    float dz[MC];
    const F8 v = load8<T>(y + p * ldy + c0);
    head_dz<MC, EX>(out, dout, tanh0, Co, HW, n, q, dz);
    one(p, v, dz);
    pos_step32(n, q, HW);
  }
}

int head_fwd_fast(const void* a, int lda, const float* w, const float* b, float* out, int tanh0, int dtype, int64_t npix, int HW, int C, int Co,
                  hipStream_t stream) {
  const int pixb = npix >= ((int64_t)1 << 20) ? 1024 : 128;
  const dim3 grid(ceil_div(npix, pixb));
  const float* none = nullptr;
#define MAU_HEAD_PLAIN(MC_, EX_)                                                                                                            \
  MAU_DISPATCH_DTYPE(dtype, MAU_LAUNCH((head_bn_fwd_kernel<T, MC_, EX_, false>), grid, dim3(256), 0, stream, (const T*)a, lda, none, none, w, b, out, \
                                       tanh0, HW, C, Co, npix, pixb))
  if (Co == 2) MAU_HEAD_PLAIN(2, true);
  else if (Co == 1) MAU_HEAD_PLAIN(2, false);
  else if (Co == HEAD_MAX_CO) MAU_HEAD_PLAIN(HEAD_MAX_CO, true);
  else MAU_HEAD_PLAIN(HEAD_MAX_CO, false);
#undef MAU_HEAD_PLAIN
  return check_launch("head_fwd_kernel");
}

}

using namespace mau;

extern "C" {

int mau_pool_bn_bwd_reduce(const void* y, int ldy, const void* dpl, int lddpl, const unsigned short* argidx, const void* dskip, int lddskip, const float* scale,
                           const float* shift, const float* mean, const float* invstd, float* slab, int ldslab, int dtype, int N, int H,
                           int W, int C, mau_stream_t stream) {
  MAU_REQUIRE(y && (dpl || dskip) && (!dpl || argidx) && scale && shift && mean && invstd && slab && N > 0 && H >= 2 && W >= 2 && C > 0, "pool_bn_bwd_reduce: bad arguments");
  const int C8 = round_up(C, 8);
  MAU_REQUIRE(ldy % 8 == 0 && ldy >= C8 && (!dpl || (lddpl % 8 == 0 && lddpl >= C8)) && (!dskip || (lddskip % 8 == 0 && lddskip >= C8)) && ldslab >= C,
              "pool_bn_bwd_reduce: bad ld");
  const int64_t npix = (int64_t)N * H * W;
  dim3 grid(ceil_div(npix, BWD_PIX_PER_BLOCK), ceil_div(C, 64));
#define MAU_POOL_REDUCE(P, S)                                                                                                                  \
  MAU_DISPATCH_DTYPE(dtype, MAU_LAUNCH((pool_bn_bwd_reduce_kernel<T, P, S>), grid, dim3(256), 0, (hipStream_t)stream, (const T*)y, ldy, (const T*)dpl, \
                                       lddpl, argidx, (const T*)dskip, lddskip, scale, shift, mean, invstd, slab, ldslab, H, W, npix, C))
  if (dpl && dskip) MAU_POOL_REDUCE(true, true);
  else if (dpl) MAU_POOL_REDUCE(true, false);
  else MAU_POOL_REDUCE(false, true);
#undef MAU_POOL_REDUCE
  return check_launch("pool_bn_bwd_reduce_kernel");
}

int mau_pool_bn_bwd_apply(const void* y, int ldy, const void* dpl, int lddpl, const unsigned short* argidx, const void* dskip, int lddskip, const float* scale,
                          const float* shift, const float* mean, const float* invstd, const double* sums, double count, void* dy, int lddy,
                          int dtype, int N, int H, int W, int C, mau_stream_t stream) {
  MAU_REQUIRE(y && (dpl || dskip) && (!dpl || argidx) && dy && sums && scale && shift && mean && invstd && N > 0 && H >= 2 && W >= 2 && C > 0 && count >= 0,
              "pool_bn_bwd_apply: bad arguments");
  const int C8 = round_up(C, 8);
  MAU_REQUIRE(ldy % 8 == 0 && ldy >= C8 && lddy % 8 == 0 && lddy >= C8 && (!dpl || (lddpl % 8 == 0 && lddpl >= C8)) &&
                  (!dskip || (lddskip % 8 == 0 && lddskip >= C8)), "pool_bn_bwd_apply: bad ld");
  MAU_REQUIRE((H + 1) / 2 <= 65535 && N <= 65535, "pool_bn_bwd_apply: H/2 and N must fit a grid dimension");
  const int xb = ceil_div(((W + 1) / 2) * (C8 / 8), 256), Hc = (H + 1) / 2;
  int RY = 8;
  while (RY > 1 && (int64_t)xb * ceil_div(Hc, RY) * N < 1024) RY >>= 1;
  dim3 grid(xb, ceil_div(Hc, RY), N);
#define MAU_POOL_APPLY(P, S)                                                                                                                   \
  MAU_DISPATCH_DTYPE(dtype, MAU_LAUNCH((pool_bn_bwd_apply_kernel<T, P, S>), grid, dim3(256), 0, (hipStream_t)stream, (const T*)y, ldy, (const T*)dpl, lddpl, \
                                       argidx, (const T*)dskip, lddskip, scale, shift, mean, invstd, sums, count > 0 ? 1.0 / count : 0.0, (T*)dy, lddy, \
                                       H, W, C, C8, RY))
  if (dpl && dskip) MAU_POOL_APPLY(true, true);
  else if (dpl) MAU_POOL_APPLY(true, false);
  else MAU_POOL_APPLY(false, true);
#undef MAU_POOL_APPLY
  return check_launch("pool_bn_bwd_apply_kernel");
}

int mau_head_bn_max_channels(void) { return 64; }

int mau_head_bn_fwd(const void* y, int ldy, const float* scale, const float* shift, const float* w, const float* b, float* out, int tanh0,
                    int dtype, int N, int HW, int C, int Co, mau_stream_t stream) {
  MAU_REQUIRE(y && scale && shift && w && b && out && N > 0 && HW > 0 && C > 0, "head_bn_fwd: bad arguments");
  MAU_REQUIRE(Co >= 1 && Co <= HEAD_MAX_CO && C <= mau_head_bn_max_channels(), "head_bn_fwd: out_channels in [1,%d], C <= %d", HEAD_MAX_CO,
              mau_head_bn_max_channels());
  MAU_REQUIRE(ldy % 8 == 0 && ldy >= round_up(C, 8), "head_bn_fwd: bad ld");
  MAU_REQUIRE(HW >= 32 && (int64_t)N * HW < ((int64_t)1 << 31), "head_bn_fwd: images of at least 32 pixels, fewer than 2^31 pixels in all");
  const int64_t npix = (int64_t)N * HW;
  const int pixb = npix >= ((int64_t)1 << 20) ? 1024 : 128;
  const dim3 grid(ceil_div(npix, pixb));
#define MAU_HEAD_FWD(MC_, EX_)                                                                                                              \
  MAU_DISPATCH_DTYPE(dtype, MAU_LAUNCH((head_bn_fwd_kernel<T, MC_, EX_>), grid, dim3(256), 0, (hipStream_t)stream, (const T*)y, ldy, scale, shift, w, b, \
                                       out, tanh0, HW, C, Co, npix, pixb))
  if (Co == 2) MAU_HEAD_FWD(2, true);
  else if (Co == 1) MAU_HEAD_FWD(2, false);
  else if (Co == HEAD_MAX_CO) MAU_HEAD_FWD(HEAD_MAX_CO, true);
  else MAU_HEAD_FWD(HEAD_MAX_CO, false);
#undef MAU_HEAD_FWD
  return check_launch("head_bn_fwd_kernel");
}

int mau_head_bn_bwd_reduce(const void* y, int ldy, const float* scale, const float* shift, const float* mean, const float* invstd,
                           const float* w, const float* out, const float* dout, float* bn_slab, int ldslab, float* head_slab, int tanh0,
                           int dtype, int N, int HW, int C, int Co, mau_stream_t stream) {
  MAU_REQUIRE(y && scale && shift && mean && invstd && w && out && dout && bn_slab && head_slab && N > 0 && HW > 0 && C > 0,
              "head_bn_bwd_reduce: bad arguments");
  MAU_REQUIRE(Co >= 1 && Co <= HEAD_MAX_CO && C <= mau_head_bn_max_channels(), "head_bn_bwd_reduce: out_channels in [1,%d], C <= %d", HEAD_MAX_CO,
              mau_head_bn_max_channels());
  const int C8 = round_up(C, 8);
  MAU_REQUIRE(ldy % 8 == 0 && ldy >= C8 && ldslab >= C, "head_bn_bwd_reduce: bad ld");
  MAU_REQUIRE(HW >= 32 && (int64_t)N * HW < ((int64_t)1 << 31), "head_bn_bwd_reduce: images of at least 32 pixels, fewer than 2^31 pixels in all");
  const int64_t npix = (int64_t)N * HW;
#define MAU_HEAD_RED(MC_, EX_)                                                                                                              \
  MAU_DISPATCH_DTYPE(dtype, MAU_LAUNCH((head_bn_bwd_reduce_kernel<T, MC_, EX_>), dim3(ceil_div(npix, BWD_PIX_PER_BLOCK)), dim3(256), 0, (hipStream_t)stream, \
                                       (const T*)y, ldy, scale, shift, mean, invstd, w, out, dout, bn_slab, ldslab, head_slab, tanh0, HW, C, C8, Co, npix))
  if (Co == 2) MAU_HEAD_RED(2, true);
  else if (Co == 1) MAU_HEAD_RED(2, false);
  else if (Co == HEAD_MAX_CO) MAU_HEAD_RED(HEAD_MAX_CO, true);
  else MAU_HEAD_RED(HEAD_MAX_CO, false);
#undef MAU_HEAD_RED
  return check_launch("head_bn_bwd_reduce_kernel");
}

int mau_head_bn_bwd_apply(const void* y, int ldy, const float* scale, const float* shift, const float* mean, const float* invstd,
                          const double* sums, double count, const float* w, const float* out, const float* dout, void* dy, int lddy,
                          int tanh0, int dtype, int N, int HW, int C, int Co, mau_stream_t stream) {
  MAU_REQUIRE(y && scale && shift && mean && invstd && sums && w && out && dout && dy && N > 0 && HW > 0 && C > 0 && count >= 0,
              "head_bn_bwd_apply: bad arguments");
  MAU_REQUIRE(Co >= 1 && Co <= HEAD_MAX_CO && C <= mau_head_bn_max_channels(), "head_bn_bwd_apply: out_channels in [1,%d], C <= %d", HEAD_MAX_CO,
              mau_head_bn_max_channels());
  const int C8 = round_up(C, 8);
  MAU_REQUIRE(ldy % 8 == 0 && ldy >= C8 && lddy % 8 == 0 && lddy >= C8, "head_bn_bwd_apply: bad ld");
  MAU_REQUIRE(HW >= 32 && (int64_t)N * HW < ((int64_t)1 << 31), "head_bn_bwd_apply: images of at least 32 pixels, fewer than 2^31 pixels in all");
  const int64_t npix = (int64_t)N * HW;
  const int pixb = npix >= ((int64_t)1 << 20) ? 2048 : 256;
#define MAU_HEAD_APPLY(MC_, EX_)                                                                                                            \
  MAU_DISPATCH_DTYPE(dtype, MAU_LAUNCH((head_bn_bwd_apply_kernel<T, MC_, EX_>), dim3(ceil_div(npix, pixb)), dim3(256), 0, (hipStream_t)stream, (const T*)y, ldy, \
                                       scale, shift, mean, invstd, sums, count > 0 ? 1.0 / count : 0.0, w, out, dout, (T*)dy, lddy, tanh0, HW, C, Co, npix, pixb))
  if (Co == 2) MAU_HEAD_APPLY(2, true);
  else if (Co == 1) MAU_HEAD_APPLY(2, false);
  else if (Co == HEAD_MAX_CO) MAU_HEAD_APPLY(HEAD_MAX_CO, true);
  else MAU_HEAD_APPLY(HEAD_MAX_CO, false);
#undef MAU_HEAD_APPLY
  return check_launch("head_bn_bwd_apply_kernel");
}

}
```

### metadata-augmented-unet-for-lst-ndvi_amd/csrc/mau_common.h

```cpp
#pragma once
#include <hip/hip_runtime.h>
#include <stdint.h>
#include <stdio.h>
#include "../../include/mau_hip.h"

typedef __bf16 bf16;
typedef _Float16 f16;
typedef __attribute__((ext_vector_type(8))) __bf16 bf16x8;
typedef __attribute__((ext_vector_type(8))) _Float16 f16x8;
typedef __attribute__((ext_vector_type(4))) __bf16 bf16x4;
typedef __attribute__((ext_vector_type(4))) short s16x4;
typedef __attribute__((ext_vector_type(4))) float f32x4;
typedef __attribute__((ext_vector_type(16))) float f32x16;

namespace mau {

void set_error(const char* fmt, ...);
int check_launch(const char* what);

#define MAU_LAUNCH(...)               \
  do {                                \
    (void)hipGetLastError();          \
    hipLaunchKernelGGL(__VA_ARGS__);  \
  } while (0)

#define MAU_REQUIRE(cond, ...)                      \
  do {                                              \
    if (!(cond)) {                                  \
      ::mau::set_error(__VA_ARGS__);                \
      return MAU_ERR_ARG;                           \
    }                                               \
  } while (0)

static inline int ceil_div(int64_t a, int64_t b) { return (int)((a + b - 1) / b); }
static inline int round_up(int a, int b) { return (a + b - 1) / b * b; }

struct F8 {
  float v[8];
};

__device__ __forceinline__ float opaque(float v) {
  asm("" : "+v"(v));
  return v;
}

template <typename T>
__device__ __forceinline__ F8 load8(const T* p);
template <>
__device__ __forceinline__ F8 load8<float>(const float* p) {
  F8 r;
  f32x4 a = *reinterpret_cast<const f32x4*>(p);
  f32x4 b = *reinterpret_cast<const f32x4*>(p + 4);
#pragma unroll
  for (int i = 0; i < 4; ++i) {
    r.v[i] = a[i];
    r.v[4 + i] = b[i];
  }
  return r;
}
template <>
__device__ __forceinline__ F8 load8<bf16>(const bf16* p) {
  F8 r;
  bf16x8 a = *reinterpret_cast<const bf16x8*>(p);
#pragma unroll
  for (int i = 0; i < 8; ++i) r.v[i] = (float)a[i];
  return r;
}
template <>
__device__ __forceinline__ F8 load8<f16>(const f16* p) {
  F8 r;
  f16x8 a = *reinterpret_cast<const f16x8*>(p);
#pragma unroll
  for (int i = 0; i < 8; ++i) r.v[i] = opaque((float)a[i]);
  return r;
}
template <typename T>
__device__ __forceinline__ void store8(T* p, const F8& r);
template <>
__device__ __forceinline__ void store8<float>(float* p, const F8& r) {
  f32x4 a, b;
#pragma unroll
  for (int i = 0; i < 4; ++i) {
    a[i] = r.v[i];
    b[i] = r.v[4 + i];
  }
  *reinterpret_cast<f32x4*>(p) = a;
  *reinterpret_cast<f32x4*>(p + 4) = b;
}
template <>
__device__ __forceinline__ void store8<bf16>(bf16* p, const F8& r) {
  bf16x8 a;
#pragma unroll
  for (int i = 0; i < 8; ++i) a[i] = (bf16)r.v[i];
  *reinterpret_cast<bf16x8*>(p) = a;
}

template <>
__device__ __forceinline__ void store8<f16>(f16* p, const F8& r) {
  f16x8 a;
#pragma unroll
  for (int i = 0; i < 8; ++i) a[i] = (f16)opaque(r.v[i]);
  *reinterpret_cast<f16x8*>(p) = a;
}

template <typename T>
__device__ __forceinline__ F8 load8_nt(const T* p);
template <>
__device__ __forceinline__ F8 load8_nt<float>(const float* p) {
  F8 r;
  const f32x4 a = __builtin_nontemporal_load(reinterpret_cast<const f32x4*>(p));
  const f32x4 b = __builtin_nontemporal_load(reinterpret_cast<const f32x4*>(p + 4));
#pragma unroll
  for (int i = 0; i < 4; ++i) {
    r.v[i] = a[i];
    r.v[4 + i] = b[i];
  }
  return r;
}
template <>
__device__ __forceinline__ F8 load8_nt<bf16>(const bf16* p) {
  F8 r;
  const bf16x8 a = __builtin_nontemporal_load(reinterpret_cast<const bf16x8*>(p));
#pragma unroll
  for (int i = 0; i < 8; ++i) r.v[i] = (float)a[i];
  return r;
}
template <>
__device__ __forceinline__ F8 load8_nt<f16>(const f16* p) {
  F8 r;
  const f16x8 a = __builtin_nontemporal_load(reinterpret_cast<const f16x8*>(p));
#pragma unroll
  for (int i = 0; i < 8; ++i) r.v[i] = opaque((float)a[i]);
  return r;
}
template <typename T>
__device__ __forceinline__ void store8_nt(T* p, const F8& r);
template <>
__device__ __forceinline__ void store8_nt<float>(float* p, const F8& r) {
  f32x4 a, b;
#pragma unroll
  for (int i = 0; i < 4; ++i) {
    a[i] = r.v[i];
    b[i] = r.v[4 + i];
  }
  __builtin_nontemporal_store(a, reinterpret_cast<f32x4*>(p));
  __builtin_nontemporal_store(b, reinterpret_cast<f32x4*>(p + 4));
}
template <>
__device__ __forceinline__ void store8_nt<bf16>(bf16* p, const F8& r) {
  bf16x8 a;
#pragma unroll
  for (int i = 0; i < 8; ++i) a[i] = (bf16)r.v[i];
  __builtin_nontemporal_store(a, reinterpret_cast<bf16x8*>(p));
}

template <>
__device__ __forceinline__ void store8_nt<f16>(f16* p, const F8& r) {
  f16x8 a;
#pragma unroll
  for (int i = 0; i < 8; ++i) a[i] = (f16)opaque(r.v[i]);
  __builtin_nontemporal_store(a, reinterpret_cast<f16x8*>(p));
}

__device__ __forceinline__ float coef(const float* __restrict__ p, int c, int C) {
  const float v = p[c < C ? c : C - 1];
  return c < C ? v : 0.f;
}
__device__ __forceinline__ double coef(const double* __restrict__ p, int c, int C) {
  const double v = p[c < C ? c : C - 1];
  return c < C ? v : 0.0;
}

__device__ __forceinline__ F8 zero8() {
  F8 r;
#pragma unroll
  for (int i = 0; i < 8; ++i) r.v[i] = 0.f;
  return r;
}

template <typename T>
__device__ __forceinline__ float to_f(T x) {
  return (float)x;
}

constexpr int BWD_PIX_PER_BLOCK = 1024;
constexpr int HEAD_MAX_CO = 4;
constexpr int HEAD_PIX_PER_BLOCK = BWD_PIX_PER_BLOCK;

struct DeviceShape {
  int cus, xcds, xcd_shift;
};
static inline DeviceShape device_shape() {
  static DeviceShape cache[64];
  static bool have[64];
  int dev = 0;
  if (hipGetDevice(&dev) != hipSuccess || dev < 0 || dev >= 64) return DeviceShape{256, 8, 3};
  if (!have[dev]) {
    int cus = 0;
    if (hipDeviceGetAttribute(&cus, hipDeviceAttributeMultiprocessorCount, dev) != hipSuccess || cus <= 0) cus = 256;
    int x = 1, s = 0;
    while (x < 8 && x * 2 * 32 <= cus) {
      x *= 2;
      ++s;
    }
    cache[dev] = DeviceShape{cus, x, s};
    have[dev] = true;
  }
  return cache[dev];
}
static inline int launch_cus() { return device_shape().cus; }
#define MAU_LDS_ATTR(bytes, ...)                                                                                        \
  do {                                                                                                                  \
    static bool done_[64];                                                                                              \
    int d_ = 0;                                                                                                         \
    if (hipGetDevice(&d_) == hipSuccess && d_ >= 0 && d_ < 64 && !done_[d_]) {                                          \
      (void)hipFuncSetAttribute(reinterpret_cast<const void*>(__VA_ARGS__), hipFuncAttributeMaxDynamicSharedMemorySize, \
                                (int)(bytes));                                                                          \
      done_[d_] = true;                                                                                                 \
    }                                                                                                                   \
  } while (0)

static inline int stream_grid(int64_t work_items, int block) {
  int64_t g = (work_items + block - 1) / block;
  const int64_t cap = (int64_t)device_shape().cus * 8;
  if (g > cap) g = cap;
  if (g < 1) g = 1;
  return (int)g;
}

__device__ __forceinline__ bool last_block_of(unsigned* ticket, unsigned n) {
  __shared__ unsigned s_last;
  asm volatile("s_waitcnt vmcnt(0)" ::: "memory");
  __syncthreads();
  if (threadIdx.x == 0) {
    __builtin_amdgcn_fence(__ATOMIC_RELEASE, "agent");
    asm volatile("s_waitcnt vmcnt(0)" ::: "memory");
    const unsigned t = __hip_atomic_fetch_add(ticket, 1u, __ATOMIC_RELAXED, __HIP_MEMORY_SCOPE_AGENT);
    const unsigned last = t == n - 1 ? 1u : 0u;
    if (last) {
      __builtin_amdgcn_fence(__ATOMIC_ACQUIRE, "agent");
      asm volatile("s_waitcnt vmcnt(0)" ::: "memory");
      __hip_atomic_store(ticket, 0u, __ATOMIC_RELAXED, __HIP_MEMORY_SCOPE_AGENT);
    }
    s_last = last;
  }
  __syncthreads();
  return s_last != 0;
}

int head_fwd_fast(const void* a, int lda, const float* w, const float* b, float* out, int tanh0, int dtype, int64_t npix, int HW, int C, int Co,
                  hipStream_t stream);

}

#define MAU_DISPATCH_DTYPE(dtype, ...)              \
  do {                                              \
    if ((dtype) == MAU_F32) {                       \
      using T = float;                              \
      __VA_ARGS__;                                  \
    } else if ((dtype) == MAU_BF16) {               \
      using T = bf16;                               \
      __VA_ARGS__;                                  \
    } else if ((dtype) == MAU_F16) {                \
      using T = f16;                                \
      __VA_ARGS__;                                  \
    } else {                                        \
      ::mau::set_error("bad dtype %d", (int)dtype); \
      return MAU_ERR_ARG;                           \
    }                                               \
  } while (0)
```

### metadata-augmented-unet-for-lst-ndvi_amd/functional.py

```python
from __future__ import annotations

import contextlib
import dataclasses

import os
from dataclasses import dataclass
from typing import List, Optional, Sequence, Tuple

import torch

from . import _lib
from ._lib import MAU_BF16, MAU_F16, MAU_F32, call, lib

BN_EPS = 1e-5
BN_MOMENTUM = 0.1


def pad8(c: int) -> int:
    return (c + 7) // 8 * 8


def dtype_code(dt: torch.dtype) -> int:
    if dt == torch.float32:
        return MAU_F32
    if dt == torch.bfloat16:
        return MAU_BF16
    if dt == torch.float16:
        return MAU_F16
    raise TypeError(f"unsupported activation dtype {dt}")


def _stream() -> int:
    return torch.cuda.current_stream().cuda_stream


def _require_cuda(t: torch.Tensor, what: str):
    if not t.is_cuda:
        raise RuntimeError(
            f"{what}: tensor is on '{t.device}'. This is the MI355X-native HIP path; it has no CPU "
            "fallback. Move the module and its inputs to a 'cuda' (ROCm) device.")


def _ld(t: torch.Tensor) -> int:
    n, h, w, _ = t.shape
    ld = t.stride(2)
    if t.stride(3) != 1 or t.stride(1) != w * ld or (n > 1 and t.stride(0) != h * w * ld) or ld % 8:
        raise RuntimeError(f"not an NHWC-ld tensor: shape {tuple(t.shape)} strides {t.stride()}")
    return ld


def _as_nhwc(t: torch.Tensor) -> torch.Tensor:
    try:
        _ld(t)
        if t.data_ptr() % 16 == 0:
            return t
    except RuntimeError:
        pass
    return t.contiguous()


@dataclass
class Act:
    t: torch.Tensor
    C: int
    nchw: bool = False

    @property
    def N(self):
        return self.t.shape[0]

    @property
    def H(self):
        return self.t.shape[2 if self.nchw else 1]

    @property
    def W(self):
        return self.t.shape[3 if self.nchw else 2]


_DT = {MAU_F32: torch.float32, MAU_BF16: torch.bfloat16, MAU_F16: torch.float16}
_GENERATION = [0]


_ZERO_ARENA = {"gen": -1, "buf": None, "cur": 0}


def _zero_bias_grad(n, dev):
    z = _ZERO_ARENA
    need = (n + 63) // 64 * 64
    if z["gen"] != _GENERATION[0] or z["buf"] is None or z["buf"].device != dev or z["cur"] + need > z["buf"].numel():
        z["buf"] = torch.zeros(max(8192, need), dtype=torch.float32, device=dev)
        z["cur"] = 0
        z["gen"] = _GENERATION[0]
    out = z["buf"][z["cur"]:z["cur"] + n]
    z["cur"] += need
    return out


def mark_params_updated(*_args, **_kwargs):
    _GENERATION[0] += 1


from torch.optim.optimizer import register_optimizer_step_post_hook as _reg_step_hook

_reg_step_hook(mark_params_updated)


_TICKETS = {}


def _tickets(dev) -> torch.Tensor:
    key = (dev.index if dev.index is not None else torch.cuda.current_device(), _stream())
    t = _TICKETS.get(key)
    if t is None:
        t = _TICKETS[key] = torch.zeros(lib.mau_reduce_tickets_elems(), dtype=torch.int32, device=dev)
    return t


class PackGroup:

    def __init__(self):
        self.params: List[torch.Tensor] = []
        self._state = {}
        self.fresh_after_step = -1

    def add(self, w: torch.Tensor):
        if not any(w is q for q in self.params):
            self.params.append(w)
            self._state = {}
        w._mau_group = self

    def _build(self, code: int, ptrs):
        import ctypes
        dev = self.params[0].device
        dt = _DT[code]
        wf = [torch.empty(lib.mau_conv3x3_packed_elems(code, w.shape[0], w.shape[1]), dtype=dt, device=dev) for w in self.params]
        wd = [torch.empty(lib.mau_conv3x3_packed_elems(code, w.shape[1], w.shape[0]), dtype=dt, device=dev) for w in self.params]
        nbytes = lib.mau_conv3x3_pack_desc_bytes()
        host = ctypes.create_string_buffer(nbytes * len(self.params))
        nxt = ctypes.c_int(0)
        for i, w in enumerate(self.params):
            call("mau_conv3x3_pack_desc_fill", ctypes.addressof(host), i, w.data_ptr(), wf[i].data_ptr(), wd[i].data_ptr(), code,
                 w.shape[0], w.shape[1], nxt.value, ctypes.addressof(nxt))
        table = torch.frombuffer(bytearray(host.raw), dtype=torch.uint8).to(dev)
        return {"ptrs": ptrs, "wf": wf, "wd": wd, "table": table, "tiles": nxt.value, "key": None}

    def ensure(self, code: int):
        ptrs = tuple(w.data_ptr() for w in self.params)
        st = self._state.get(code)
        if st is None or st["ptrs"] != ptrs:
            st = self._state[code] = self._build(code, ptrs)
        key = (_GENERATION[0], tuple(w._version for w in self.params))
        if st["key"] != key:
            if not (self.fresh_after_step == _GENERATION[0] and st["key"] is not None and st["key"][1] == key[1] and len(self._state) == 1):
                call("mau_conv3x3_pack_weights_multi", st["table"].data_ptr(), len(self.params), st["tiles"], code, _stream())
            st["key"] = key
            for w, f, d in zip(self.params, st["wf"], st["wd"]):
                w._mau_pack = [(key[0], w._version, w.data_ptr(), code), f, d]
        return st


def pack_conv_weights(w: torch.Tensor, code: int, forward: bool = True, dgrad: bool = False):
    cout, cin = w.shape[0], w.shape[1]
    key = (_GENERATION[0], w._version, w.data_ptr(), code)
    cache = getattr(w, "_mau_pack", None)
    if cache is not None and cache[0] == key and (cache[1] is not None or not forward) and (cache[2] is not None or not dgrad):
        return (cache[1] if forward else None), (cache[2] if dgrad else None)
    group = getattr(w, "_mau_group", None)
    if group is not None and _PACK_MULTI:
        group.ensure(code)
        cache = w._mau_pack
        return (cache[1] if forward else None), (cache[2] if dgrad else None)
    dt = _DT[code]
    if cache is None:
        cache = [None, None, None]
        try:
            w._mau_pack = cache
        except (AttributeError, RuntimeError):
            pass

    def buf(old, n):
        if old is not None and old.dtype == dt and old.device == w.device and old.numel() == n:
            return old
        return torch.empty(n, dtype=dt, device=w.device)

    stale = cache[0] != key
    need_f = forward and (stale or cache[1] is None or cache[1].dtype != dt)
    need_d = dgrad and (stale or cache[2] is None or cache[2].dtype != dt)
    wf = buf(cache[1], lib.mau_conv3x3_packed_elems(code, cout, cin)) if need_f else None
    wd = buf(cache[2], lib.mau_conv3x3_packed_elems(code, cin, cout)) if need_d else None
    if need_f or need_d:
        call("mau_conv3x3_pack_weights", w.detach().data_ptr(), wf.data_ptr() if need_f else None, wd.data_ptr() if need_d else None,
             code, cout, cin, _stream())
    if stale:
        cache[1] = wf
        cache[2] = wd
    else:
        if need_f:
            cache[1] = wf
        if need_d:
            cache[2] = wd
    cache[0] = key
    return (cache[1] if forward else None), (cache[2] if dgrad else None)


class ToNHWC(torch.autograd.Function):

    @staticmethod
    def forward(ctx, x: torch.Tensor, dt: torch.dtype):
        _require_cuda(x, "UrbanPredictor.forward(maps)")
        x = x.contiguous().float()
        N, Cc, H, W = x.shape
        ld = pad8(Cc)
        out = torch.empty((N, H, W, ld), dtype=dt, device=x.device)
        call("mau_nchw_to_nhwc", x.data_ptr(), out.data_ptr(), dtype_code(dt), N, Cc, H, W, ld, _stream())
        ctx.C = Cc
        return out

    @staticmethod
    def backward(ctx, g):
        g = _as_nhwc(g)
        N, H, W, _ = g.shape
        out = torch.empty((N, ctx.C, H, W), dtype=torch.float32, device=g.device)
        call("mau_nhwc_to_nchw", g.data_ptr(), out.data_ptr(), dtype_code(g.dtype), N, ctx.C, H, W, _ld(g), _stream())
        return out, None


def to_nchw(a: Act) -> torch.Tensor:
    t = _as_nhwc(a.t.detach())
    N, H, W, _ = t.shape
    out = torch.empty((N, a.C, H, W), dtype=torch.float32, device=t.device)
    call("mau_nhwc_to_nchw", t.data_ptr(), out.data_ptr(), dtype_code(t.dtype), N, a.C, H, W, _ld(t), _stream())
    return out


@dataclass
class BNState:
    training: bool
    C0: int
    momentum: float = BN_MOMENTUM
    eps: float = BN_EPS
    group: object = None
    comm: object = None
    world: int = 1
    grad_enabled: bool = True
    frozen: object = None
    C1: int = 0
    pool: bool = False
    out_view: object = None
    head: object = None
    up_to: object = None
    first: bool = False
    dtype: object = None
    dgrad_first: bool = False


def _all_reduce_(t: torch.Tensor, st: BNState):
    if st.comm is not None:
        st.comm.all_reduce(t, 0, _stream())
    elif st.group is not None:
        from .dist import all_reduce_sum
        all_reduce_sum(t, st.group)


_OVERLAP_WGRAD = int(os.environ.get("MAU_OVERLAP_WGRAD", "2") or 0)
_FUSED_REDUCE = True
_FUSED_BN = True
_FUSED_UP = True
_PACK_MULTI = True
_INFER_POOL_FUSED = True
_FIRST_WGRAD = True
_SIDE_STREAMS = {}


def _side_stream(dev) -> "torch.cuda.Stream":
    s = _SIDE_STREAMS.get(dev)
    if s is None:
        s = _SIDE_STREAMS[dev] = torch.cuda.Stream(device=dev)
    return s


def _join_side_when_backward_ends(dev):
    def join():
        torch.cuda.current_stream(dev).wait_stream(_side_stream(dev))

    torch.autograd.Variable._execution_engine.queue_callback(join)


_DGRAD_FIRST = None


def _conv_fwd(x, x1, st, emb, emb_ws, E, wpk, bias, post, y, Cout, slab, code, N, H, W, stream):
    scale, shift = post if post is not None else (None, None)
    call("mau_conv3x3_fwd2", x.data_ptr(), _ld(x), st.C0, x1.data_ptr() if x1 is not None else None,
         _ld(x1) if x1 is not None else 0, st.C1 if x1 is not None else 0, emb.data_ptr() if E else None,
         emb_ws.data_ptr() if E else None, E, wpk.data_ptr(), bias.data_ptr() if bias is not None else None,
         scale.data_ptr() if scale is not None else None, shift.data_ptr() if shift is not None else None,
         y.data_ptr(), _ld(y), Cout, slab.data_ptr() if slab is not None else None, code, N, H, W, stream)


class ConvBNReLU(torch.autograd.Function):

    @staticmethod
    def forward(ctx, x, x1, emb, weight, bias, gamma, beta, rmean, rvar, nbt, hw, hb, st: BNState):
        _require_cuda(x, "conv3x3")
        first = st.first
        if first:
            if x1 is not None or emb is not None or x.dim() != 4 or x.shape[1] != st.C0 or st.C0 > lib.mau_conv3x3_first_max_channels():
                raise RuntimeError("conv3x3 (first layer): expects one (N, C <= 8, H, W) fp32 input")
            xin = x.contiguous().float()
            N, _, H, W = xin.shape
            act_dt = st.dtype
        else:
            x = _as_nhwc(x)
            if x1 is not None:
                x1 = _as_nhwc(x1)
            N, H, W, _ = x.shape
            act_dt = x.dtype
        code = dtype_code(act_dt)
        dev = x.device
        Cout, Cin = weight.shape[0], weight.shape[1]
        E = 0 if emb is None else emb.shape[1]
        C1 = st.C1 if x1 is not None else 0
        if st.C0 + C1 + E != Cin:
            raise RuntimeError(f"conv3x3: input has {st.C0}+{C1}+{E} channels, weight expects {Cin}")
        if emb is not None:
            emb = emb.contiguous().float()
        ldy = pad8(Cout)
        stream = _stream()
        needs = ctx.needs_input_grad
        inference = (not st.training) and (not st.grad_enabled or not any(needs))
        emb_ws = torch.empty((N, E), dtype=act_dt, device=dev) if E else None
        f32 = dict(dtype=torch.float32, device=dev)
        dst = st.out_view
        if dst is not None and (tuple(dst.shape) != (N, H, W, ldy) or dst.dtype != act_dt or Cout % 64 != 0):
            raise RuntimeError("conv3x3: out_view must be an (N,H,W,Cout) NHWC-ld view of the activation dtype with Cout % 64 == 0")
        if sum((st.pool, st.head is not None, st.up_to is not None)) > 1 or ((st.head is not None or st.up_to is not None) and dst is not None):
            raise RuntimeError("conv3x3: pool / head / up_to are exclusive, and head / up_to write no activation (no out_view)")
        Co = tanh0 = 0
        w2 = None
        if st.head is not None:
            Co = hw.shape[0]
            tanh0 = 1 if (Co == 2 and st.head) else 0
            w2 = hw.detach().reshape(Co, Cout).contiguous().float()

        def first_fwd(post, y_, slab_, x8_):
            scale_, shift_ = post if post is not None else (None, None)
            call("mau_conv3x3_first_fwd", xin.data_ptr(), st.C0, weight.detach().data_ptr(), bias.detach().data_ptr() if bias is not None else None,
                 scale_.data_ptr() if scale_ is not None else None, shift_.data_ptr() if shift_ is not None else None, y_.data_ptr(), _ld(y_),
                 Cout, slab_.data_ptr() if slab_ is not None else None, x8_.data_ptr() if x8_ is not None else None, code, N, H, W, stream)

        def pooled_of(a):
            pl = torch.empty((N, H // 2, W // 2, ldy), dtype=act_dt, device=dev)
            call("mau_maxpool2x2_fwd", a.data_ptr(), _ld(a), pl.data_ptr(), ldy, code, N, H, W, Cout, stream)
            return pl

        def head_of(a):
            out = torch.empty((N, Co, H, W), **f32)
            call("mau_head_fwd", a.data_ptr(), _ld(a), w2.data_ptr(), hb.detach().data_ptr(), out.data_ptr(), tanh0, code, N, H * W,
                 Cout, Co, stream)
            return out

        def up_of(a):
            Hu, Wu = st.up_to
            up = torch.empty((N, Hu, Wu, ldy), dtype=act_dt, device=dev)
            call("mau_resize_bilinear_fwd", a.data_ptr(), _ld(a), H, W, up.data_ptr(), ldy, 0, code, N, Hu, Wu, Cout, stream)
            return up

        if inference:
            y = dst if dst is not None else torch.empty((N, H, W, ldy), dtype=act_dt, device=dev)
            fz = st.frozen if st.frozen is not None else {}
            fkey = (_GENERATION[0], weight._version, gamma._version, rmean._version, rvar._version)
            if "wf" not in fz or fz["wf"].dtype != act_dt or fz.get("key") != fkey:
                fz["key"] = fkey
                fz["wf"] = weight if first else pack_conv_weights(weight, code, forward=True, dgrad=False)[0]
                if "scale" not in fz or fz["scale"].device != dev or fz["scale"].numel() != Cout:
                    fz["scale"], fz["shift"] = torch.empty(Cout, **f32), torch.empty(Cout, **f32)
                call("mau_bn_coeffs_eval", gamma.data_ptr(), beta.data_ptr(), rmean.data_ptr(), rvar.data_ptr(),
                     st.eps, fz["scale"].data_ptr(), fz["shift"].data_ptr(), None, None, Cout, stream)
            pl = None
            if first:
                first_fwd((fz["scale"], fz["shift"]), y, None, None)
            elif st.pool and _INFER_POOL_FUSED and x1 is None and not E and H >= 2 and W >= 2:
                pl = torch.empty((N, H // 2, W // 2, ldy), dtype=act_dt, device=dev)
                call("mau_conv3x3_fwd_pool", x.data_ptr(), _ld(x), st.C0, fz["wf"].data_ptr(), bias.data_ptr() if bias is not None else None,
                     fz["scale"].data_ptr(), fz["shift"].data_ptr(), y.data_ptr(), _ld(y), Cout, pl.data_ptr(), ldy, code, N, H, W, stream)
            else:
                _conv_fwd(x, x1, st, emb, emb_ws, E, fz["wf"], bias, (fz["scale"], fz["shift"]), y, Cout, None, code, N, H, W, stream)
            if st.head is not None:
                out = head_of(y)
                ctx.mark_non_differentiable(out)
                return out
            if st.up_to is not None:
                up = up_of(y)
                ctx.mark_non_differentiable(up)
                return up
            ctx.mark_non_differentiable(y)
            if st.pool:
                if pl is None:
                    pl = pooled_of(y)
                ctx.mark_non_differentiable(pl)
                return y, pl
            return y
        y = torch.empty((N, H, W, ldy), dtype=act_dt, device=dev)
        need_dx = needs[0] or (x1 is not None and needs[1]) or (E > 0 and needs[2])
        if first:
            if need_dx:
                raise RuntimeError("conv3x3 (first layer): no gradient w.r.t. the network input on this path")
            wf = wd = None
            x = torch.empty((N, H, W, 8), dtype=act_dt, device=dev) if (st.grad_enabled and needs[3]) else None
        else:
            wf, wd = pack_conv_weights(weight, code, forward=True, dgrad=st.grad_enabled and need_dx)
        scale, shift = torch.empty(Cout, **f32), torch.empty(Cout, **f32)
        mean, invstd = torch.empty(Cout, **f32), torch.empty(Cout, **f32)
        npix = N * H * W
        if st.training:
            tiles = lib.mau_conv3x3_first_rows(N, H, W) if first else lib.mau_conv3x3_num_pixel_tiles(code, N, H, W, Cout)
            cpad = (Cout + 63) // 64 * 64
            slab = torch.empty((tiles, 2 * cpad), **f32)
            if first:
                first_fwd(None, y, slab, x)
            else:
                _conv_fwd(x, x1, st, emb, emb_ws, E, wf, bias, None, y, Cout, slab, code, N, H, W, stream)
            nbt_ptr = nbt.data_ptr() if nbt is not None else None
            tk = _tickets(dev).data_ptr() if _FUSED_REDUCE else None
            if st.group is None:
                ws = torch.empty(lib.mau_bn_stats_ws_elems(tiles, Cout), dtype=torch.float64, device=dev)
                call("mau_bn_stats_finalize_train", slab.data_ptr(), tiles, float(npix), gamma.data_ptr(), beta.data_ptr(),
                     rmean.data_ptr(), rvar.data_ptr(), nbt_ptr, st.momentum, st.eps, scale.data_ptr(), shift.data_ptr(),
                     mean.data_ptr(), invstd.data_ptr(), ws.data_ptr(), tk, Cout, stream)
            else:
                sums = torch.empty(2 * Cout + 1, dtype=torch.float64, device=dev)
                ws = torch.empty(lib.mau_reduce_rows_ws_elems(tiles, 2 * Cout), dtype=torch.float64, device=dev)
                call("mau_bn_stats_sums_f64", slab.data_ptr(), tiles, Cout, sums.data_ptr(), ws.data_ptr(), _tickets(dev).data_ptr(),
                     float(npix), stream)
                _all_reduce_(sums, st)
                call("mau_bn_finalize_train", sums.data_ptr(), 0.0, gamma.data_ptr(), beta.data_ptr(),
                     rmean.data_ptr(), rvar.data_ptr(), nbt_ptr, st.momentum, st.eps, scale.data_ptr(), shift.data_ptr(),
                     mean.data_ptr(), invstd.data_ptr(), Cout, stream)
        else:
            call("mau_bn_coeffs_eval", gamma.data_ptr(), beta.data_ptr(), rmean.data_ptr(), rvar.data_ptr(),
                 st.eps, scale.data_ptr(), shift.data_ptr(), mean.data_ptr(), invstd.data_ptr(), Cout, stream)
            if first:
                first_fwd(None, y, None, x)
            else:
                _conv_fwd(x, x1, st, emb, emb_ws, E, wf, bias, None, y, Cout, None, code, N, H, W, stream)

        fused = _FUSED_BN
        fuse_head = fused and st.head is not None and Cout <= lib.mau_head_bn_max_channels() and H * W >= 32
        fuse_up = fused and _FUSED_UP and st.up_to is not None and H <= st.up_to[0] and W <= st.up_to[1]
        a = pl = out = up = argidx = None
        if fuse_head:
            out = torch.empty((N, Co, H, W), **f32)
            call("mau_head_bn_fwd", y.data_ptr(), ldy, scale.data_ptr(), shift.data_ptr(), w2.data_ptr(), hb.detach().data_ptr(),
                 out.data_ptr(), tanh0, code, N, H * W, Cout, Co, stream)
        elif fuse_up:
            Hu, Wu = st.up_to
            up = torch.empty((N, Hu, Wu, ldy), dtype=act_dt, device=dev)
            call("mau_resize_bilinear_bn_fwd", y.data_ptr(), ldy, H, W, scale.data_ptr(), shift.data_ptr(), up.data_ptr(), ldy, 0, code,
                 N, Hu, Wu, Cout, stream)
        else:
            a = dst if dst is not None else torch.empty_like(y)
            lda = _ld(a)
            if st.pool and H >= 2 and W >= 2:
                pl = torch.empty((N, H // 2, W // 2, ldy), dtype=act_dt, device=dev)
                argidx = torch.empty((N, H // 2, W // 2, ldy // 8), dtype=torch.int16, device=dev) if fused else None
                call("mau_bn_relu_apply_pool", y.data_ptr(), ldy, scale.data_ptr(), shift.data_ptr(), a.data_ptr(), lda,
                     pl.data_ptr(), ldy, argidx.data_ptr() if argidx is not None else None, code, N, H, W, Cout, stream)
            else:
                call("mau_bn_relu_apply", y.data_ptr(), ldy, scale.data_ptr(), shift.data_ptr(), a.data_ptr(), lda, code,
                     npix, Cout, stream)
            if st.head is not None:
                out = head_of(a)
            elif st.up_to is not None:
                up = up_of(a)
        ctx.st = st if st.out_view is None else dataclasses.replace(st, out_view=None)
        ctx.E = E
        ctx.C1 = C1
        ctx.wd = wd
        ctx.pooled = pl is not None
        ctx.head = (Co, tanh0, tuple(hw.shape), fuse_head) if st.head is not None else None
        ctx.up = (st.up_to, fuse_up) if st.up_to is not None else None
        keep_a = a if ((pl is not None and not fused) or (st.head is not None and not fuse_head)) else None
        ctx.save_for_backward(x, x1, emb, weight, y, scale, shift, mean, invstd, keep_a, w2, out, argidx)
        if st.head is not None:
            return out
        if st.up_to is not None:
            return up
        if st.pool:
            return a, pl
        return a

    @staticmethod
    def backward(ctx, da, dpl=None):
        x, x1, emb, weight, y, scale, shift, mean, invstd, a, w2, out, argidx = ctx.saved_tensors
        st: BNState = ctx.st
        E, C1 = ctx.E, ctx.C1
        N, H, W, ldy = y.shape
        code = dtype_code(y.dtype)
        dev = y.device
        Cout, Cin = weight.shape[0], weight.shape[1]
        npix = N * H * W
        stream = _stream()
        f32 = dict(dtype=torch.float32, device=dev)
        needs = ctx.needs_input_grad
        sync = st.training and st.group is not None
        rows = lib.mau_bn_bwd_rows(npix)
        slab = torch.empty((rows, 2 * Cout), **f32)
        sums = torch.empty(2 * Cout + 1, dtype=torch.float64, device=dev)
        g32 = torch.empty(2 * Cout, **f32)
        dy = torch.empty_like(y)
        dhw = dhb = None
        cptrs = (scale.data_ptr(), shift.data_ptr(), mean.data_ptr(), invstd.data_ptr())

        def finish_sums():
            ws = torch.empty(lib.mau_reduce_rows_ws_elems(rows, 2 * Cout), dtype=torch.float64, device=dev)
            call("mau_reduce_rows_f64_f32", slab.data_ptr(), rows, 2 * Cout, 2 * Cout, sums.data_ptr(), g32.data_ptr(), ws.data_ptr(),
                 _tickets(dev).data_ptr() if (_FUSED_REDUCE or sync) else None, float(npix) if sync else 0.0, stream)
            if not st.training:
                return torch.zeros_like(sums), float(npix)
            if sync:
                _all_reduce_(sums, st)
                return sums, 0.0
            return sums, float(npix)

        fused_pool = ctx.pooled and dpl is not None and argidx is not None
        if ctx.head is not None and ctx.head[3]:
            Co, tanh0, hshape, _ = ctx.head
            dout = da.contiguous().float()
            hrows, rowlen = lib.mau_head_bwd_rows(N, H * W), lib.mau_head_bwd_rowlen(Cout, Co)
            hslab = torch.empty((hrows, rowlen), **f32)
            call("mau_head_bn_bwd_reduce", y.data_ptr(), ldy, *cptrs, w2.data_ptr(), out.data_ptr(), dout.data_ptr(), slab.data_ptr(), Cout,
                 hslab.data_ptr(), tanh0, code, N, H * W, Cout, Co, stream)
            sums_apply, count = finish_sums()
            red = torch.empty(rowlen, **f32)
            hws = torch.empty(lib.mau_reduce_rows_ws_elems(hrows, rowlen), dtype=torch.float64, device=dev)
            call("mau_reduce_rows_f32", hslab.data_ptr(), hrows, rowlen, rowlen, red.data_ptr(), hws.data_ptr(),
                 _tickets(dev).data_ptr() if _FUSED_REDUCE else None, stream)
            red = red.view(Co, pad8(Cout) + 8)
            dhw = red[:, :Cout].reshape(hshape).contiguous()
            dhb = red[:, pad8(Cout)].contiguous()
            call("mau_head_bn_bwd_apply", y.data_ptr(), ldy, *cptrs, sums_apply.data_ptr(), count, w2.data_ptr(), out.data_ptr(),
                 dout.data_ptr(), dy.data_ptr(), ldy, tanh0, code, N, H * W, Cout, Co, stream)
        elif fused_pool:
            dpl = _as_nhwc(dpl)
            dsk = _as_nhwc(da) if da is not None else None
            pargs = (y.data_ptr(), ldy, dpl.data_ptr(), _ld(dpl), argidx.data_ptr(), dsk.data_ptr() if dsk is not None else None,
                     _ld(dsk) if dsk is not None else 0)
            call("mau_pool_bn_bwd_reduce", *pargs, *cptrs, slab.data_ptr(), Cout, code, N, H, W, Cout, stream)
            sums_apply, count = finish_sums()
            call("mau_pool_bn_bwd_apply", *pargs, *cptrs, sums_apply.data_ptr(), count, dy.data_ptr(), ldy, code, N, H, W, Cout, stream)
        else:
            if ctx.head is not None:
                Co, tanh0, hshape, _ = ctx.head
                dout = da.contiguous().float()
                da = torch.empty((N, H, W, ldy), dtype=y.dtype, device=dev)
                hrows, rowlen = lib.mau_head_bwd_rows(N, H * W), lib.mau_head_bwd_rowlen(Cout, Co)
                hslab = torch.empty((hrows, rowlen), **f32)
                call("mau_head_bwd", a.data_ptr(), _ld(a), w2.data_ptr(), out.data_ptr(), dout.data_ptr(), da.data_ptr(), ldy,
                     hslab.data_ptr(), tanh0, code, N, H * W, Cout, Co, stream)
                red = torch.empty(rowlen, **f32)
                hws = torch.empty(lib.mau_reduce_rows_ws_elems(hrows, rowlen), dtype=torch.float64, device=dev)
                call("mau_reduce_rows_f32", hslab.data_ptr(), hrows, rowlen, rowlen, red.data_ptr(), hws.data_ptr(),
                     _tickets(dev).data_ptr() if _FUSED_REDUCE else None, stream)
                red = red.view(Co, pad8(Cout) + 8)
                dhw = red[:, :Cout].reshape(hshape).contiguous()
                dhb = red[:, pad8(Cout)].contiguous()
            elif ctx.up is not None:
                (Hu, Wu), _ = ctx.up
                g = _as_nhwc(da)
                da = torch.empty((N, H, W, ldy), dtype=y.dtype, device=dev)
                call("mau_resize_bilinear_bwd", g.data_ptr(), _ld(g), 0, Hu, Wu, da.data_ptr(), ldy, code, N, H, W, Cout, stream)
            elif ctx.pooled and dpl is not None:
                dpl = _as_nhwc(dpl)
                act = a
                if act is None:
                    act = torch.empty_like(y)
                    call("mau_bn_relu_apply", y.data_ptr(), ldy, scale.data_ptr(), shift.data_ptr(), act.data_ptr(), ldy, code, npix, Cout, stream)
                dsum = torch.empty((N, H, W, ldy), dtype=y.dtype, device=dev)
                if da is None:
                    call("mau_maxpool2x2_bwd", act.data_ptr(), _ld(act), dpl.data_ptr(), _ld(dpl), dsum.data_ptr(), ldy, code, N, H, W, Cout, stream)
                else:
                    da = _as_nhwc(da)
                    call("mau_maxpool2x2_bwd_add", act.data_ptr(), _ld(act), dpl.data_ptr(), _ld(dpl), da.data_ptr(), _ld(da),
                         dsum.data_ptr(), ldy, code, N, H, W, Cout, stream)
                da = dsum
            elif da is None:
                da = torch.zeros((N, H, W, ldy), dtype=y.dtype, device=dev)
            da = _as_nhwc(da)
            call("mau_bn_relu_bwd_reduce", da.data_ptr(), _ld(da), y.data_ptr(), ldy, *cptrs, slab.data_ptr(), Cout, code, npix, Cout, stream)
            sums_apply, count = finish_sums()
            call("mau_bn_relu_bwd_apply", da.data_ptr(), _ld(da), y.data_ptr(), ldy, *cptrs, sums_apply.data_ptr(), count, dy.data_ptr(), ldy,
                 code, npix, Cout, stream)
        dgamma = g32[Cout:]
        dbeta = g32[:Cout]
        dw = None
        need_dx = needs[0] or (x1 is not None and needs[1]) or (E and needs[2])
        overlap = _OVERLAP_WGRAD
        side = _side_stream(dev) if (needs[3] and overlap and (need_dx or overlap >= 2)) else None
        deferred = False
        dfull = None
        if (st.dgrad_first if _DGRAD_FIRST is None else _DGRAD_FIRST == "1") and need_dx and needs[3] and side is not None:
            dy_ready = torch.cuda.Event()
            dy_ready.record()
            wd = ctx.wd if ctx.wd is not None else pack_conv_weights(weight, code, forward=False, dgrad=True)[1]
            dfull = torch.empty((N, H, W, pad8(Cin)), dtype=y.dtype, device=dev)
            call("mau_conv3x3_fwd", dy.data_ptr(), ldy, Cout, None, None, 0, wd.data_ptr(), None, None, None, dfull.data_ptr(),
                 pad8(Cin), Cin, None, code, N, H, W, stream)
            side.wait_event(dy_ready)
        if needs[3]:
            if side is not None and dfull is None:
                side.wait_stream(torch.cuda.current_stream())
            with torch.cuda.stream(side) if side is not None else contextlib.nullcontext():
                acc = torch.empty(max(lib.mau_conv3x3_wgrad_acc_elems(code, N, H, W, Cout, Cin),
                                      lib.mau_conv3x3_first_wgrad_ws_elems(N, H, W, Cout) if st.first else 0), **f32)
                emb_ws = torch.empty((N, E), dtype=y.dtype, device=dev) if E else None
            slot = getattr(weight, "_mau_grad_slot", None)
            dw = slot.view_as(weight) if (slot is not None and weight.is_leaf and weight.grad is None and slot.device == dev) else torch.empty_like(weight)
            wstream = side.cuda_stream if side is not None else stream
            deferred = side is not None and overlap >= 2 and weight.is_leaf and weight.grad is None
            if st.first and _FIRST_WGRAD:
                call("mau_conv3x3_first_wgrad", x.data_ptr(), dy.data_ptr(), ldy, dw.data_ptr(), acc.data_ptr(), Cin, Cout, code, N, H, W, wstream)
            else:
                call("mau_conv3x3_wgrad2", x.data_ptr(), _ld(x), st.C0, x1.data_ptr() if x1 is not None else None,
                     _ld(x1) if x1 is not None else 0, C1, emb.data_ptr() if E else None,
                     emb_ws.data_ptr() if E else None, E, dy.data_ptr(), ldy, Cout, acc.data_ptr(), code, N, H, W, wstream)
                call("mau_conv3x3_unpack_wgrad", acc.data_ptr(), lib.mau_conv3x3_wgrad_splits(code, N, H, W, Cout, Cin),
                     dw.data_ptr(), Cout, Cin, wstream)
            if deferred:
                for t in (x, x1, emb, dy, dw):
                    if t is not None:
                        t.record_stream(side)
                weight._mau_grad_stream = side
                _join_side_when_backward_ends(dev)
        dx = dx1 = demb = None
        if need_dx:
            wd = ctx.wd if ctx.wd is not None else pack_conv_weights(weight, code, forward=False, dgrad=True)[1]
            ldd = pad8(Cin)
            if dfull is None:
                dfull = torch.empty((N, H, W, ldd), dtype=y.dtype, device=dev)
                call("mau_conv3x3_fwd", dy.data_ptr(), ldy, Cout, None, None, 0, wd.data_ptr(), None, None, None, dfull.data_ptr(),
                     ldd, Cin, None, code, N, H, W, stream)
            Ct = st.C0 + C1
            if E and needs[2]:
                demb = torch.empty((N, E), **f32)
                ws = torch.empty(lib.mau_bcast_bwd_ws_elems(N, H * W, E), **f32)
                call("mau_bcast_bwd", dfull.data_ptr(), ldd, Ct, demb.data_ptr(), ws.data_ptr(), code, N, H * W, E, stream)
            if C1:
                if needs[0]:
                    dx = dfull[..., :st.C0]
                if needs[1]:
                    dx1 = dfull[..., st.C0:st.C0 + pad8(C1)]
            elif needs[0]:
                dx = dfull[..., :pad8(st.C0)] if E else dfull
        if side is not None and not deferred:
            torch.cuda.current_stream().wait_stream(side)
        dbias = None
        if needs[4]:
            if st.training:
                dbias = _zero_bias_grad(Cout, dev)
            else:
                dbias = scale * dbeta
        return dx, dx1, demb, dw, dbias, dgamma, dbeta, None, None, None, dhw, dhb, None


class MaxPool2x2(torch.autograd.Function):

    @staticmethod
    def forward(ctx, x, C):
        x = _as_nhwc(x)
        N, H, W, _ = x.shape
        ldy = pad8(C)
        y = torch.empty((N, H // 2, W // 2, ldy), dtype=x.dtype, device=x.device)
        call("mau_maxpool2x2_fwd", x.data_ptr(), _ld(x), y.data_ptr(), ldy, dtype_code(x.dtype), N, H, W, C, _stream())
        ctx.save_for_backward(x)
        ctx.C = C
        return y

    @staticmethod
    def backward(ctx, dy):
        (x,) = ctx.saved_tensors
        dy = _as_nhwc(dy)
        N, H, W, _ = x.shape
        dx = torch.empty((N, H, W, pad8(ctx.C)), dtype=x.dtype, device=x.device)
        call("mau_maxpool2x2_bwd", x.data_ptr(), _ld(x), dy.data_ptr(), _ld(dy), dx.data_ptr(), pad8(ctx.C),
             dtype_code(x.dtype), N, H, W, ctx.C, _stream())
        return dx, None


class PoolSkip(torch.autograd.Function):

    @staticmethod
    def forward(ctx, x, C):
        x = _as_nhwc(x)
        N, H, W, _ = x.shape
        ldy = pad8(C)
        y = torch.empty((N, H // 2, W // 2, ldy), dtype=x.dtype, device=x.device)
        call("mau_maxpool2x2_fwd", x.data_ptr(), _ld(x), y.data_ptr(), ldy, dtype_code(x.dtype), N, H, W, C, _stream())
        ctx.save_for_backward(x)
        ctx.C = C
        return y, x.view_as(x)

    @staticmethod
    def backward(ctx, dy, dskip):
        (x,) = ctx.saved_tensors
        if dy is None:
            return dskip, None
        dy = _as_nhwc(dy)
        N, H, W, _ = x.shape
        dx = torch.empty((N, H, W, pad8(ctx.C)), dtype=x.dtype, device=x.device)
        if dskip is None:
            call("mau_maxpool2x2_bwd", x.data_ptr(), _ld(x), dy.data_ptr(), _ld(dy), dx.data_ptr(), pad8(ctx.C),
                 dtype_code(x.dtype), N, H, W, ctx.C, _stream())
        else:
            dskip = _as_nhwc(dskip)
            call("mau_maxpool2x2_bwd_add", x.data_ptr(), _ld(x), dy.data_ptr(), _ld(dy), dskip.data_ptr(), _ld(dskip),
                 dx.data_ptr(), pad8(ctx.C), dtype_code(x.dtype), N, H, W, ctx.C, _stream())
        return dx, None


def _resize_into(src, Cs, h, w, dst, choff, N, H, W, code, stream):
    if choff % 8 == 0:
        call("mau_resize_bilinear_fwd", src.data_ptr(), _ld(src), h, w, dst.data_ptr(), _ld(dst), choff, code, N, H, W, Cs, stream)
    else:
        tmp = torch.empty((N, H, W, pad8(Cs)), dtype=dst.dtype, device=dst.device)
        call("mau_resize_bilinear_fwd", src.data_ptr(), _ld(src), h, w, tmp.data_ptr(), pad8(Cs), 0, code, N, H, W, Cs, stream)
        call("mau_copy_channels", tmp.data_ptr(), pad8(Cs), dst.data_ptr(), _ld(dst), choff, 0, code, N * H * W, Cs, stream)


class RowPrefix(torch.autograd.Function):

    @staticmethod
    def forward(ctx, C, *xs):
        base = xs[0]
        ld, esz = base.stride(2), base.element_size()
        for j, t in enumerate(xs):
            if t.data_ptr() != base.data_ptr() + j * C * esz or t.stride() != base.stride() or t.shape != base.shape:
                raise RuntimeError("RowPrefix: inputs are not adjacent channel slots of one row buffer")
        N, H, W, _ = base.shape
        ctx.C, ctx.k = C, len(xs)
        return base.as_strided((N, H, W, C * len(xs)), base.stride())

    @staticmethod
    def backward(ctx, g):
        g = _as_nhwc(g)
        return (None, *[g[..., j * ctx.C:(j + 1) * ctx.C] for j in range(ctx.k)])


class Fanout(torch.autograd.Function):

    @staticmethod
    def forward(ctx, x, k: int):
        ctx.k = k
        ctx.meta = (x.shape, x.dtype, x.device)
        return tuple(x.as_strided(x.shape, x.stride()) for _ in range(k))

    @staticmethod
    def backward(ctx, *gs):
        import ctypes
        shape, dtype, dev = ctx.meta
        live = [_as_nhwc(g) for g in gs if g is not None]
        if not live:
            return None, None
        if len(live) == 1:
            return live[0], None
        N, H, W, C = shape
        ld = pad8(C)
        kmax = lib.mau_sum_tensors_max()
        out = torch.empty((N, H, W, ld), dtype=dtype, device=dev)
        while True:
            part = live[:kmax]
            ptrs = (ctypes.c_void_p * len(part))(*[g.data_ptr() for g in part])
            lds = (ctypes.c_int * len(part))(*[_ld(g) for g in part])
            call("mau_sum_tensors", ctypes.addressof(ptrs), ctypes.addressof(lds), len(part), out.data_ptr(), ld, dtype_code(dtype),
                 N * H * W, C, _stream())
            live = [out] + live[kmax:]
            if len(live) == 1:
                break
            out = torch.empty((N, H, W, ld), dtype=dtype, device=dev)
        res = live[0]
        return (res if ld == C else res[..., :C]), None


class EmbFold(torch.autograd.Function):

    @staticmethod
    def forward(ctx, weight, emb, Ct: int, Ep: int):
        _require_cuda(weight, "EmbFold")
        w = weight.detach().contiguous().float()
        e = emb.detach().contiguous().float()
        Cout, Cf = w.shape[0], w.shape[1]
        N, E = e.shape
        if Cf != Ct + E or Ep < N:
            raise RuntimeError(f"EmbFold: weight has {Cf} input channels, expected {Ct}+{E}; Ep={Ep} must cover the batch of {N}")
        weff = torch.empty((Cout, Ct + Ep, 3, 3), dtype=torch.float32, device=w.device)
        call("mau_emb_fold_fwd", w.data_ptr(), e.data_ptr(), weff.data_ptr(), Cout, Ct, E, N, Ep, _stream())
        ctx.save_for_backward(weight, emb)
        ctx.dims = (Cout, Ct, E, N, Ep)
        return weff

    @staticmethod
    def backward(ctx, dweff):
        weight, emb = ctx.saved_tensors
        Cout, Ct, E, N, Ep = ctx.dims
        dweff = dweff.contiguous().float()
        w = weight.detach().contiguous().float()
        e = emb.detach().contiguous().float()
        dw = demb = None
        if ctx.needs_input_grad[0]:
            slot = getattr(weight, "_mau_grad_slot", None)
            dw = slot.view_as(weight) if (slot is not None and weight.is_leaf and weight.grad is None and slot.device == w.device) else torch.empty_like(w)
        ws = None
        if ctx.needs_input_grad[1]:
            demb = torch.empty((N, E), dtype=torch.float32, device=w.device)
            ws = torch.empty(lib.mau_emb_fold_ws_elems(Cout, N, E), dtype=torch.float32, device=w.device)
        call("mau_emb_fold_bwd", w.data_ptr(), e.data_ptr(), dweff.data_ptr(), dw.data_ptr() if dw is not None else None,
             demb.data_ptr() if demb is not None else None, ws.data_ptr() if ws is not None else None, Cout, Ct, E, N, Ep, _stream())
        return dw, demb, None, None


_EMB_IDENTITY = {}
_EMB_FOLD = True
_EMB_FOLD_MIN_WORK = 1 << 20


def emb_identity(N: int, Ep: int, dev) -> torch.Tensor:
    key = (N, Ep, str(dev))
    t = _EMB_IDENTITY.get(key)
    if t is None:
        t = torch.zeros((N, Ep), dtype=torch.float32, device=dev)
        t[torch.arange(N), torch.arange(N)] = 1.0
        _EMB_IDENTITY[key] = t
    return t


def fold_embedding(weight: torch.Tensor, emb: torch.Tensor, Ct: int, pixels: int):
    N, E = emb.shape
    Ep = (N + 15) // 16 * 16
    if ((Ct + Ep) // 16) % 2 == 1 and Ct % 16 == 0:
        Ep += 16
    if not _EMB_FOLD or Ep + 16 > E or Ct % 8 != 0 or N * pixels < _EMB_FOLD_MIN_WORK:
        return None
    return EmbFold.apply(weight, emb, Ct, Ep), emb_identity(N, Ep, emb.device)


class UpsampleTo(torch.autograd.Function):

    @staticmethod
    def forward(ctx, low, C_low, two_step, H, W):
        low = _as_nhwc(low)
        N, h, w, _ = low.shape
        code = dtype_code(low.dtype)
        stream = _stream()
        ld = pad8(C_low)
        src, sh, sw = low, h, w
        mid = None
        if two_step and (2 * h, 2 * w) != (H, W):
            mid = torch.empty((N, 2 * h, 2 * w, ld), dtype=low.dtype, device=low.device)
            call("mau_resize_bilinear_fwd", low.data_ptr(), _ld(low), h, w, mid.data_ptr(), ld, 0, code, N, 2 * h, 2 * w, C_low, stream)
            src, sh, sw = mid, 2 * h, 2 * w
        out = torch.empty((N, H, W, ld), dtype=low.dtype, device=low.device)
        call("mau_resize_bilinear_fwd", src.data_ptr(), _ld(src), sh, sw, out.data_ptr(), ld, 0, code, N, H, W, C_low, stream)
        ctx.meta = (C_low, (h, w), (H, W), mid is not None)
        return out

    @staticmethod
    def backward(ctx, g):
        C_low, (h, w), (H, W), two = ctx.meta
        g = _as_nhwc(g)
        N = g.shape[0]
        code = dtype_code(g.dtype)
        stream = _stream()
        ld = pad8(C_low)
        gsrc, gld, sH, sW = g, _ld(g), H, W
        if two:
            dmid = torch.empty((N, 2 * h, 2 * w, ld), dtype=g.dtype, device=g.device)
            call("mau_resize_bilinear_bwd", g.data_ptr(), gld, 0, H, W, dmid.data_ptr(), ld, code, N, 2 * h, 2 * w, C_low, stream)
            gsrc, gld, sH, sW = dmid, ld, 2 * h, 2 * w
        dlow = torch.empty((N, h, w, ld), dtype=g.dtype, device=g.device)
        call("mau_resize_bilinear_bwd", gsrc.data_ptr(), gld, 0, sH, sW, dlow.data_ptr(), ld, code, N, h, w, C_low, stream)
        return dlow, None, None, None, None


class ConcatUp(torch.autograd.Function):

    @staticmethod
    def forward(ctx, low, C_low, two_step, skip_Cs, *skips):
        low = _as_nhwc(low)
        skips = [_as_nhwc(s) for s in skips]
        N, H, W, _ = skips[0].shape
        h, w = low.shape[1], low.shape[2]
        code = dtype_code(low.dtype)
        stream = _stream()
        Ctot = sum(skip_Cs) + C_low
        ld = pad8(Ctot)
        out = torch.empty((N, H, W, ld), dtype=low.dtype, device=low.device)
        choff = 0
        npix = N * H * W
        for s, cs in zip(skips, skip_Cs):
            call("mau_copy_channels", s.data_ptr(), _ld(s), out.data_ptr(), ld, choff, 0, code, npix, cs, stream)
            choff += cs
        mid = None
        src, sh, sw = low, h, w
        if two_step and (2 * h, 2 * w) != (H, W):
            mid = torch.empty((N, 2 * h, 2 * w, pad8(C_low)), dtype=low.dtype, device=low.device)
            call("mau_resize_bilinear_fwd", low.data_ptr(), _ld(low), h, w, mid.data_ptr(), pad8(C_low), 0, code, N, 2 * h, 2 * w, C_low, stream)
            src, sh, sw = mid, 2 * h, 2 * w
        _resize_into(src, C_low, sh, sw, out, choff, N, H, W, code, stream)
        if ld > Ctot:
            out[..., Ctot:].zero_()
        ctx.meta = (C_low, tuple(skip_Cs), (h, w), (H, W), mid is not None)
        return out

    @staticmethod
    def backward(ctx, g):
        C_low, skip_Cs, (h, w), (H, W), two = ctx.meta
        g = _as_nhwc(g)
        N = g.shape[0]
        code = dtype_code(g.dtype)
        stream = _stream()
        ldg = _ld(g)
        npix = N * H * W
        grads = []
        choff = 0
        for cs in skip_Cs:
            if cs % 8 == 0 and choff % 8 == 0:
                grads.append(g[..., choff:choff + cs])
            else:
                t = torch.empty((N, H, W, pad8(cs)), dtype=g.dtype, device=g.device)
                call("mau_copy_channels", g.data_ptr() + choff * g.element_size(), ldg,
                     t.data_ptr(), pad8(cs), 0, pad8(cs), code, npix, cs, stream)
                grads.append(t)
            choff += cs
        if choff % 8 == 0:
            gsrc, goff, gld = g, choff, ldg
        else:
            gsrc = torch.empty((N, H, W, pad8(C_low)), dtype=g.dtype, device=g.device)
            call("mau_copy_channels", g.data_ptr() + choff * g.element_size(), ldg, gsrc.data_ptr(), pad8(C_low), 0,
                 pad8(C_low), code, npix, C_low, stream)
            goff, gld = 0, pad8(C_low)
        if two:
            dmid = torch.empty((N, 2 * h, 2 * w, pad8(C_low)), dtype=g.dtype, device=g.device)
            call("mau_resize_bilinear_bwd", gsrc.data_ptr(), gld, goff, H, W, dmid.data_ptr(), pad8(C_low), code, N, 2 * h, 2 * w, C_low, stream)
            gsrc, goff, gld, sH, sW = dmid, 0, pad8(C_low), 2 * h, 2 * w
        else:
            sH, sW = H, W
        dlow = torch.empty((N, h, w, pad8(C_low)), dtype=g.dtype, device=g.device)
        call("mau_resize_bilinear_bwd", gsrc.data_ptr(), gld, goff, sH, sW, dlow.data_ptr(), pad8(C_low), code, N, h, w, C_low, stream)
        return (dlow, None, None, None, *grads)


class BcastCat(torch.autograd.Function):

    @staticmethod
    def forward(ctx, x, C, emb):
        x = _as_nhwc(x)
        emb = emb.contiguous().float()
        N, H, W, _ = x.shape
        E = emb.shape[1]
        ld = pad8(C + E)
        code = dtype_code(x.dtype)
        out = torch.empty((N, H, W, ld), dtype=x.dtype, device=x.device)
        stream = _stream()
        call("mau_copy_channels", x.data_ptr(), _ld(x), out.data_ptr(), ld, 0, 0, code, N * H * W, C, stream)
        call("mau_bcast_fill", emb.data_ptr(), out.data_ptr(), ld, C, ld, code, N, H * W, E, stream)
        ctx.meta = (C, E)
        return out

    @staticmethod
    def backward(ctx, g):
        C, E = ctx.meta
        g = _as_nhwc(g)
        N, H, W, _ = g.shape
        code = dtype_code(g.dtype)
        stream = _stream()
        dx = torch.empty((N, H, W, pad8(C)), dtype=g.dtype, device=g.device)
        call("mau_copy_channels", g.data_ptr(), _ld(g), dx.data_ptr(), pad8(C), 0, pad8(C), code, N * H * W, C, stream)
        demb = torch.empty((N, E), dtype=torch.float32, device=g.device)
        ws = torch.empty(lib.mau_bcast_bwd_ws_elems(N, H * W, E), dtype=torch.float32, device=g.device)
        call("mau_bcast_bwd", g.data_ptr(), _ld(g), C, demb.data_ptr(), ws.data_ptr(), code, N, H * W, E, stream)
        return dx, None, demb


class Head(torch.autograd.Function):

    @staticmethod
    def forward(ctx, a, C, weight, bias, activate=True):
        a = _as_nhwc(a)
        N, H, W, _ = a.shape
        Co = weight.shape[0]
        tanh0 = 1 if (Co == 2 and activate) else 0
        out = torch.empty((N, Co, H, W), dtype=torch.float32, device=a.device)
        w2 = weight.detach().reshape(Co, C).contiguous().float()
        call("mau_head_fwd", a.data_ptr(), _ld(a), w2.data_ptr(), bias.detach().data_ptr(), out.data_ptr(), tanh0,
             dtype_code(a.dtype), N, H * W, C, Co, _stream())
        ctx.save_for_backward(a, w2, out)
        ctx.meta = (C, Co, tanh0, tuple(weight.shape))
        return out

    @staticmethod
    def backward(ctx, dout):
        a, w2, out = ctx.saved_tensors
        C, Co, tanh0, wshape = ctx.meta
        N, H, W, _ = a.shape
        dout = dout.contiguous().float()
        da = torch.empty((N, H, W, pad8(C)), dtype=a.dtype, device=a.device)
        rows, rowlen = lib.mau_head_bwd_rows(N, H * W), lib.mau_head_bwd_rowlen(C, Co)
        slab = torch.empty((rows, rowlen), dtype=torch.float32, device=a.device)
        stream = _stream()
        call("mau_head_bwd", a.data_ptr(), _ld(a), w2.data_ptr(), out.data_ptr(), dout.data_ptr(), da.data_ptr(), pad8(C),
             slab.data_ptr(), tanh0, dtype_code(a.dtype), N, H * W, C, Co, stream)
        red = torch.empty(rowlen, dtype=torch.float32, device=a.device)
        ws = torch.empty(lib.mau_reduce_rows_ws_elems(rows, rowlen), dtype=torch.float64, device=a.device)
        call("mau_reduce_rows_f32", slab.data_ptr(), rows, rowlen, rowlen, red.data_ptr(), ws.data_ptr(),
             _tickets(a.device).data_ptr() if _FUSED_REDUCE else None, stream)
        red = red.view(Co, pad8(C) + 8)
        dw = red[:, :C].reshape(wshape).contiguous()
        db = red[:, pad8(C)].contiguous()
        return da, None, dw, db, None


class MetaMLP(torch.autograd.Function):

    @staticmethod
    def forward(ctx, md, w0, b0, w2, b2):
        _require_cuda(md, "MetadataEncoder")
        md = md.contiguous().float()
        N, F = md.shape
        Hd, D = w0.shape[0], w2.shape[0]
        hidden = torch.empty((N, Hd), dtype=torch.float32, device=md.device)
        emb = torch.empty((N, D), dtype=torch.float32, device=md.device)
        call("mau_meta_mlp_fwd", md.data_ptr(), w0.detach().data_ptr(), b0.detach().data_ptr(), w2.detach().data_ptr(),
             b2.detach().data_ptr(), hidden.data_ptr(), emb.data_ptr(), N, F, Hd, D, _stream())
        ctx.save_for_backward(md, w0, w2, hidden)
        return emb

    @staticmethod
    def backward(ctx, demb):
        md, w0, w2, hidden = ctx.saved_tensors
        demb = demb.contiguous().float()
        N, F = md.shape
        Hd, D = w0.shape[0], w2.shape[0]
        dw0, db0 = torch.empty_like(w0), torch.empty(Hd, dtype=torch.float32, device=md.device)
        dw2, db2 = torch.empty_like(w2), torch.empty(D, dtype=torch.float32, device=md.device)
        ws = torch.empty((N, Hd), dtype=torch.float32, device=md.device)
        call("mau_meta_mlp_bwd", md.data_ptr(), w0.detach().data_ptr(), w2.detach().data_ptr(), hidden.data_ptr(),
             demb.data_ptr(), dw0.data_ptr(), db0.data_ptr(), dw2.data_ptr(), db2.data_ptr(), ws.data_ptr(), N, F, Hd, D,
             _stream())
        return None, dw0, db0, dw2, db2


class LSTMLast(torch.autograd.Function):

    @staticmethod
    def forward(ctx, x, w_ih, w_hh, b_ih, b_hh):
        _require_cuda(x, "TemporalEncoder")
        x = x.contiguous().float()
        B, T = x.shape
        H = w_hh.shape[1]
        dev = x.device
        need = any(ctx.needs_input_grad[1:])
        h = torch.empty((B, H), dtype=torch.float32, device=dev)
        gates = torch.empty((B, T, 4 * H), dtype=torch.float32, device=dev) if need else None
        cells = torch.empty((B, T, H), dtype=torch.float32, device=dev) if need else None
        wi, wh = w_ih.detach().contiguous().float(), w_hh.detach().contiguous().float()
        call("mau_lstm_fwd", x.data_ptr(), wi.data_ptr(), wh.data_ptr(), b_ih.detach().data_ptr(), b_hh.detach().data_ptr(),
             h.data_ptr(), gates.data_ptr() if need else None, cells.data_ptr() if need else None, B, T, H, _stream())
        if need:
            ctx.save_for_backward(x, wh, gates, cells)
        ctx.shapes = (tuple(w_ih.shape), B, T, H)
        return h

    @staticmethod
    def backward(ctx, dh):
        x, wh, gates, cells = ctx.saved_tensors
        wshape, B, T, H = ctx.shapes
        dev = x.device
        dh = dh.contiguous().float()
        f32 = dict(dtype=torch.float32, device=dev)
        dw_ih, dw_hh = torch.empty(4 * H, **f32), torch.empty((4 * H, H), **f32)
        db_ih, db_hh = torch.empty(4 * H, **f32), torch.empty(4 * H, **f32)
        ws = torch.empty(lib.mau_lstm_bwd_ws_elems(B, T, H), **f32)
        call("mau_lstm_bwd", x.data_ptr(), wh.data_ptr(), gates.data_ptr(), cells.data_ptr(), dh.data_ptr(), dw_ih.data_ptr(),
             dw_hh.data_ptr(), db_ih.data_ptr(), db_hh.data_ptr(), ws.data_ptr(), B, T, H, _stream())
        return None, dw_ih.view(wshape), dw_hh, db_ih, db_hh


class Linear(torch.autograd.Function):

    @staticmethod
    def forward(ctx, x, w, b):
        _require_cuda(x, "Linear")
        x = x.contiguous().float()
        N, F = x.shape
        D = w.shape[0]
        out = torch.empty((N, D), dtype=torch.float32, device=x.device)
        wc = w.detach().contiguous().float()
        call("mau_linear_fwd", x.data_ptr(), wc.data_ptr(), b.detach().data_ptr() if b is not None else None, out.data_ptr(), N, F, D, _stream())
        ctx.save_for_backward(x, wc)
        ctx.has_bias = b is not None
        return out

    @staticmethod
    def backward(ctx, dout):
        x, wc = ctx.saved_tensors
        N, F = x.shape
        D = wc.shape[0]
        dout = dout.contiguous().float()
        dx = torch.empty_like(x) if ctx.needs_input_grad[0] else None
        dw, db = torch.empty_like(wc), torch.empty(D, dtype=torch.float32, device=x.device)
        call("mau_linear_bwd", x.data_ptr(), wc.data_ptr(), dout.data_ptr(), dx.data_ptr() if dx is not None else None, dw.data_ptr(),
             db.data_ptr(), N, F, D, _stream())
        return dx, dw, (db if ctx.has_bias else None)


class MSELoss(torch.autograd.Function):

    @staticmethod
    def forward(ctx, out, tgt):
        _require_cuda(out, "compute_loss_mse")
        out = out.contiguous().float()
        tgt = tgt.contiguous().float()
        n = out.numel()
        partial = torch.empty(lib.mau_mse_blocks(n), dtype=torch.float64, device=out.device)
        loss = torch.empty(1, dtype=torch.float32, device=out.device)
        dout = torch.empty_like(out) if ctx.needs_input_grad[0] else None
        call("mau_mse_fwd_bwd", out.data_ptr(), tgt.data_ptr(), partial.data_ptr(), loss.data_ptr(),
             dout.data_ptr() if dout is not None else None, n, _stream())
        ctx.save_for_backward(dout)
        return loss.reshape(())

    @staticmethod
    def backward(ctx, g):
        (d,) = ctx.saved_tensors
        return (d * g if d is not None else None), None


class L1GradientLoss(torch.autograd.Function):

    @staticmethod
    def forward(ctx, out, tgt):
        _require_cuda(out, "gradient_loss")
        out = out.contiguous().float()
        tgt = tgt.contiguous().float()
        B, Cc, H, W = out.shape
        n = out.numel()
        need = ctx.needs_input_grad[0]
        partial = torch.empty(3 * lib.mau_l1_gradient_blocks(n), dtype=torch.float64, device=out.device)
        terms = torch.empty(3, dtype=torch.float32, device=out.device)
        d_l1 = torch.empty_like(out) if need else None
        d_gr = torch.empty_like(out) if need else None
        call("mau_l1_gradient_loss", out.data_ptr(), tgt.data_ptr(), partial.data_ptr(), terms.data_ptr(),
             d_l1.data_ptr() if need else None, 1.0, 0.0, B, Cc, H, W, _stream())
        if need:
            terms2 = torch.empty(3, dtype=torch.float32, device=out.device)
            call("mau_l1_gradient_loss", out.data_ptr(), tgt.data_ptr(), partial.data_ptr(), terms2.data_ptr(),
                 d_gr.data_ptr(), 0.0, 1.0, B, Cc, H, W, _stream())
        ctx.save_for_backward(d_l1, d_gr)
        return terms[0], terms[1] + terms[2]

    @staticmethod
    def backward(ctx, g_l1, g_grad):
        d_l1, d_gr = ctx.saved_tensors
        if d_l1 is None:
            return None, None
        return g_l1 * d_l1 + g_grad * d_gr, None
```

Baseline: 2558 images/s.

## Fuse BN backward sum reduction into reduce kernels via last-block tickets

```diff
diff --git a/include/mau_hip.h b/include/mau_hip.h
--- a/include/mau_hip.h
+++ b/include/mau_hip.h
@@ -108,11 +108,20 @@
                           double count, void* dy, int lddy, int dtype, int64_t npix, int C,
                           mau_stream_t stream);
 int mau_bn_bwd_rows(int64_t npix);
+size_t mau_bn_bwd_tickets_elems(int64_t npix, int C);
+int mau_bn_relu_bwd_reduce_sums(const void* da, int ldda, const void* y, int ldy, const float* scale, const float* shift,
+                                const float* mean, const float* invstd, float* slab, int ldslab, double* sums, float* sums32,
+                                double* ws, unsigned* tickets, double append, int dtype, int64_t npix, int C,
+                                mau_stream_t stream);
 
 int mau_pool_bn_bwd_reduce(const void* y, int ldy, const void* dpl, int lddpl, const unsigned short* argidx,
                            const void* dskip, int lddskip,
                            const float* scale, const float* shift, const float* mean, const float* invstd, float* slab,
                            int ldslab, int dtype, int N, int H, int W, int C, mau_stream_t stream);
+int mau_pool_bn_bwd_reduce_sums(const void* y, int ldy, const void* dpl, int lddpl, const unsigned short* argidx,
+                                const void* dskip, int lddskip, const float* scale, const float* shift, const float* mean,
+                                const float* invstd, float* slab, int ldslab, double* sums, float* sums32, double* ws,
+                                unsigned* tickets, double append, int dtype, int N, int H, int W, int C, mau_stream_t stream);
 int mau_pool_bn_bwd_apply(const void* y, int ldy, const void* dpl, int lddpl, const unsigned short* argidx,
                           const void* dskip, int lddskip,
                           const float* scale, const float* shift, const float* mean, const float* invstd,
@@ -125,6 +134,10 @@
                            const float* invstd, const float* w, const float* out, const float* dout, float* bn_slab,
                            int ldslab, float* head_slab, int tanh0, int dtype, int N, int HW, int C, int Co,
                            mau_stream_t stream);
+int mau_head_bn_bwd_reduce_sums(const void* y, int ldy, const float* scale, const float* shift, const float* mean,
+                                const float* invstd, const float* w, const float* out, const float* dout, float* bn_slab,
+                                int ldslab, float* head_slab, double* sums, float* sums32, double* ws, unsigned* tickets,
+                                double append, int tanh0, int dtype, int N, int HW, int C, int Co, mau_stream_t stream);
 int mau_head_bn_bwd_apply(const void* y, int ldy, const float* scale, const float* shift, const float* mean,
                           const float* invstd, const double* sums, double count, const float* w, const float* out,
                           const float* dout, void* dy, int lddy, int tanh0, int dtype, int N, int HW, int C, int Co,
diff --git a/metadata-augmented-unet-for-lst-ndvi_amd/_lib.py b/metadata-augmented-unet-for-lst-ndvi_amd/_lib.py
--- a/metadata-augmented-unet-for-lst-ndvi_amd/_lib.py
+++ b/metadata-augmented-unet-for-lst-ndvi_amd/_lib.py
@@ -59,6 +59,10 @@
     "mau_bn_relu_bwd_reduce": (_i, [_p, _i, _p, _i, _p, _p, _p, _p, _p, _i, _i, _i64, _i, _p]),
     "mau_bn_relu_bwd_apply": (_i, [_p, _i, _p, _i, _p, _p, _p, _p, _p, _d, _p, _i, _i, _i64, _i, _p]),
     "mau_bn_bwd_rows": (_i, [_i64]),
+    "mau_bn_bwd_tickets_elems": (_sz, [_i64, _i]),
+    "mau_bn_relu_bwd_reduce_sums": (_i, [_p, _i, _p, _i, _p, _p, _p, _p, _p, _i, _p, _p, _p, _p, _d, _i, _i64, _i, _p]),
+    "mau_pool_bn_bwd_reduce_sums": (_i, [_p, _i, _p, _i, _p, _p, _i, _p, _p, _p, _p, _p, _i, _p, _p, _p, _p, _d, _i, _i, _i, _i, _i, _p]),
+    "mau_head_bn_bwd_reduce_sums": (_i, [_p, _i, _p, _p, _p, _p, _p, _p, _p, _p, _i, _p, _p, _p, _p, _p, _d, _i, _i, _i, _i, _i, _i, _p]),
     "mau_pool_bn_bwd_reduce": (_i, [_p, _i, _p, _i, _p, _p, _i, _p, _p, _p, _p, _p, _i, _i, _i, _i, _i, _i, _p]),
     "mau_pool_bn_bwd_apply": (_i, [_p, _i, _p, _i, _p, _p, _i, _p, _p, _p, _p, _p, _d, _p, _i, _i, _i, _i, _i, _i, _p]),
     "mau_head_bn_max_channels": (_i, []),
diff --git a/metadata-augmented-unet-for-lst-ndvi_amd/csrc/bn.hip b/metadata-augmented-unet-for-lst-ndvi_amd/csrc/bn.hip
--- a/metadata-augmented-unet-for-lst-ndvi_amd/csrc/bn.hip
+++ b/metadata-augmented-unet-for-lst-ndvi_amd/csrc/bn.hip
@@ -3,35 +3,6 @@
 
 namespace mau {
 
-template <int G, typename Load>
-__device__ __forceinline__ void ordered_group(int& k, int end, Load load, double& s0, double& s1) {
-  for (; k + 8 * (G - 1) + 4 < end; k += 8 * G) {
-    double a[G], b[G];
-#pragma unroll
-    for (int i = 0; i < G; ++i) {
-      a[i] = load(k + 8 * i);
-      b[i] = load(k + 8 * i + 4);
-    }
-#pragma unroll
-    for (int i = 0; i < G; ++i) {
-      s0 += a[i];
-      s1 += b[i];
-    }
-  }
-}
-template <typename Load>
-__device__ __forceinline__ void ordered_pair_sum(int first, int end, Load load, double& s0, double& s1) {
-  int k = first;
-#ifndef MAU_REDUCE_SERIAL
-  ordered_group<16>(k, end, load, s0, s1);
-  ordered_group<4>(k, end, load, s0, s1);
-#endif
-  for (; k + 4 < end; k += 8) {
-    s0 += load(k);
-    s1 += load(k + 4);
-  }
-  if (k < end) s0 += load(k);
-}
 
 template <typename InT, typename OutT>
 __global__ __launch_bounds__(256) void reduce_rows_kernel(const InT* __restrict__ slab, int rows, int M, int ldrow,
@@ -54,12 +25,6 @@
   }
 }
 
-constexpr int REDUCE_MAX_CHUNKS = 128;
-static int reduce_chunks(int rows) {
-  int c = rows / 32;
-  if (c > REDUCE_MAX_CHUNKS) c = REDUCE_MAX_CHUNKS;
-  return c < 1 ? 1 : c;
-}
 
 template <typename OutT>
 static int reduce_rows_launch(const float* slab, int rows, int M, int ldrow, OutT* out, double* ws, hipStream_t st,
@@ -366,8 +331,8 @@
                                                                  int ldy, const float* __restrict__ scale,
                                                                  const float* __restrict__ shift, const float* __restrict__ mean,
                                                                  const float* __restrict__ invstd, float* __restrict__ slab,
-                                                                 int ldslab, int64_t npix, int C) {
-  __shared__ float red[2][32][64 + 1];
+                                                                 int ldslab, int64_t npix, int C, BwdSums fin) {
+  __shared__ __align__(16) float red[2][32][64 + 1];
   const int cv = threadIdx.x & 7, ps = threadIdx.x >> 3;
   const int c0 = blockIdx.y * 64 + cv * 8;
   const int64_t p0 = (int64_t)blockIdx.x * BWD_PIX_PER_BLOCK;
@@ -427,6 +392,7 @@
     const int cc = blockIdx.y * 64 + c;
     if (cc < ldslab) slab[((size_t)blockIdx.x * 2 + which) * ldslab + cc] = s;
   }
+  if (fin.tickets != nullptr) bn_bwd_finish_sums(slab, ldslab, C, fin, reinterpret_cast<double*>(&red[0][0][0]));
 }
 
 template <typename T, bool NT>
@@ -440,7 +406,7 @@
   const PixVec m(nv);
   if (m.ps >= m.PS) return;
   if (inv_count <= 0.0) inv_count = 1.0 / sums[2 * C];
-  const int64_t p0 = (int64_t)blockIdx.x * pixb;
+  const int64_t p0 = (int64_t)bwd_apply_block(blockIdx.x, gridDim.x) * pixb;
   const int64_t p1 = p0 + pixb < npix ? p0 + pixb : npix;
   for (int vv = m.v; vv < nv; vv += m.nvl) {
     const int c = vv * 8;
@@ -609,16 +575,32 @@
 
 int mau_bn_bwd_rows(int64_t npix) { return ceil_div(npix, BWD_PIX_PER_BLOCK); }
 
-int mau_bn_relu_bwd_reduce(const void* da, int ldda, const void* y, int ldy, const float* scale, const float* shift,
-                           const float* mean, const float* invstd, float* slab, int ldslab, int dtype, int64_t npix,
-                           int C, mau_stream_t stream) {
+size_t mau_bn_bwd_tickets_elems(int64_t npix, int C) { return npix > 0 && C > 0 ? bn_bwd_tickets(mau_bn_bwd_rows(npix), C) : 0; }
+
+static int bn_relu_bwd_reduce_launch(const void* da, int ldda, const void* y, int ldy, const float* scale, const float* shift,
+                                     const float* mean, const float* invstd, float* slab, int ldslab, const BwdSums& fin, int dtype,
+                                     int64_t npix, int C, mau_stream_t stream) {
   MAU_REQUIRE(da && y && scale && shift && mean && invstd && slab && npix > 0 && C > 0, "bn_relu_bwd_reduce: bad arguments");
   MAU_REQUIRE(ldda % 8 == 0 && ldy % 8 == 0 && ldslab >= C, "bn_relu_bwd_reduce: bad ld");
   dim3 grid(mau_bn_bwd_rows(npix), ceil_div(C, 64));
   MAU_DISPATCH_DTYPE(dtype, MAU_LAUNCH(bn_relu_bwd_reduce_kernel<T>, grid, dim3(256), 0, (hipStream_t)stream,
                                                (const T*)da, ldda, (const T*)y, ldy, scale, shift, mean, invstd, slab,
-                                               ldslab, npix, C));
+                                               ldslab, npix, C, fin));
   return check_launch("bn_relu_bwd_reduce_kernel");
+}
+
+int mau_bn_relu_bwd_reduce(const void* da, int ldda, const void* y, int ldy, const float* scale, const float* shift,
+                           const float* mean, const float* invstd, float* slab, int ldslab, int dtype, int64_t npix,
+                           int C, mau_stream_t stream) {
+  return bn_relu_bwd_reduce_launch(da, ldda, y, ldy, scale, shift, mean, invstd, slab, ldslab, BwdSums{}, dtype, npix, C, stream);
+}
+
+int mau_bn_relu_bwd_reduce_sums(const void* da, int ldda, const void* y, int ldy, const float* scale, const float* shift,
+                                const float* mean, const float* invstd, float* slab, int ldslab, double* sums, float* sums32,
+                                double* ws, unsigned* tickets, double append, int dtype, int64_t npix, int C, mau_stream_t stream) {
+  MAU_REQUIRE(sums && ws && tickets && npix > 0, "bn_relu_bwd_reduce_sums: bad arguments");
+  return bn_relu_bwd_reduce_launch(da, ldda, y, ldy, scale, shift, mean, invstd, slab, ldslab,
+                                   BwdSums{sums, sums32, ws, tickets, append, reduce_chunks(mau_bn_bwd_rows(npix))}, dtype, npix, C, stream);
 }
 
 int mau_bn_relu_bwd_apply(const void* da, int ldda, const void* y, int ldy, const float* scale, const float* shift,
diff --git a/metadata-augmented-unet-for-lst-ndvi_amd/csrc/bn_fused.hip b/metadata-augmented-unet-for-lst-ndvi_amd/csrc/bn_fused.hip
--- a/metadata-augmented-unet-for-lst-ndvi_amd/csrc/bn_fused.hip
+++ b/metadata-augmented-unet-for-lst-ndvi_amd/csrc/bn_fused.hip
@@ -117,8 +117,8 @@
                                                                  const T* __restrict__ dskip, int lddskip, const float* __restrict__ scale,
                                                                  const float* __restrict__ shift, const float* __restrict__ mean,
                                                                  const float* __restrict__ invstd, float* __restrict__ slab, int ldslab,
-                                                                 int H, int W, int64_t npix, int C) {
-  __shared__ float red[2][32][64 + 1];
+                                                                 int H, int W, int64_t npix, int C, BwdSums fin) {
+  __shared__ __align__(16) float red[2][32][64 + 1];
   const int cv = threadIdx.x & 7, ps = threadIdx.x >> 3;
   const int c0 = blockIdx.y * 64 + cv * 8;
   const int64_t p0 = (int64_t)blockIdx.x * BWD_PIX_PER_BLOCK;
@@ -161,6 +161,7 @@
     }
   }
   bn_sums_to_slab(red, s1, s2, cv, ps, slab, ldslab);
+  if (fin.tickets != nullptr) bn_bwd_finish_sums(slab, ldslab, C, fin, reinterpret_cast<double*>(&red[0][0][0]));
 }
 
 struct Apply8 {
@@ -201,10 +202,11 @@
                                                                 double inv_count, T* __restrict__ dyo, int lddy, int H, int W, int C, int C8,
                                                                 int RY) {
   const int nv = C8 >> 3, Wc = (W + 1) >> 1, Hc = (H + 1) >> 1, Ho = H >> 1, Wo = W >> 1;
-  const int idx = blockIdx.x * 256 + threadIdx.x;
+  const int bx = bwd_apply_block(blockIdx.x, gridDim.x), by = bwd_apply_block(blockIdx.y, gridDim.y);
+  const int idx = bx * 256 + threadIdx.x;
   if (idx >= Wc * nv) return;
   const int xo = idx / nv, c = (idx - xo * nv) * 8;
-  const int n = blockIdx.z;
+  const int n = bwd_apply_block(blockIdx.z, gridDim.z);
   if (inv_count <= 0.0) inv_count = 1.0 / sums[2 * C];
   Apply8 k;
   k.load(scale, shift, mean, invstd, sums, inv_count, c, C);
@@ -212,7 +214,7 @@
   const bool hasx = x0 + 1 < W;
   const int x1 = hasx ? x0 + 1 : x0;
   const int xpc = xo < Wo ? xo : Wo - 1;
-  for (int yo = blockIdx.y * RY; yo < min(Hc, (int)(blockIdx.y + 1) * RY); ++yo) {
+  for (int yo = by * RY; yo < min(Hc, (by + 1) * RY); ++yo) {
     const int y0 = 2 * yo;
     const bool hasy = y0 + 1 < H;
     const size_t row0 = ((size_t)n * H + y0) * W, row1 = ((size_t)n * H + (hasy ? y0 + 1 : y0)) * W;
@@ -350,8 +352,8 @@
                                                                  const float* __restrict__ invstd, const float* __restrict__ w,
                                                                  const float* __restrict__ out, const float* __restrict__ dout,
                                                                  float* __restrict__ bn_slab, int ldslab, float* __restrict__ head_slab,
-                                                                 int tanh0, int HW, int C, int C8, int Co, int64_t npix) {
-  __shared__ float red[2][32][64 + 1];
+                                                                 int tanh0, int HW, int C, int C8, int Co, int64_t npix, BwdSums fin) {
+  __shared__ __align__(16) float red[2][32][64 + 1];
   __shared__ float hred[32 * HEAD_MAX_CO * 65];
   const int cv = threadIdx.x & 7, ps = threadIdx.x >> 3;
   const int c0 = cv * 8;
@@ -496,6 +498,7 @@
     row[threadIdx.x * (C8 + 8) + C8] = s;
   }
   bn_sums_to_slab(red, s1, s2, cv, ps, bn_slab, ldslab);
+  if (fin.tickets != nullptr) bn_bwd_finish_sums(bn_slab, ldslab, C, fin, reinterpret_cast<double*>(&red[0][0][0]));
 }
 
 template <typename T, int MC, bool EX>
@@ -516,7 +519,7 @@
   for (int o = 0; o < MC; ++o)
 #pragma unroll
     for (int j = 0; j < 8; ++j) wr[o][j] = o < Co ? coef(w + o * C, c0 + j, C) : 0.f;
-  const int64_t p0 = (int64_t)blockIdx.x * pixb;
+  const int64_t p0 = (int64_t)bwd_apply_block(blockIdx.x, gridDim.x) * pixb;
   const int64_t p1 = p0 + pixb < npix ? p0 + pixb : npix;
   int n = (int)((p0 + ps) / HW);
   int q = (int)((p0 + ps) - (int64_t)n * HW);
@@ -582,23 +585,39 @@
 
 extern "C" {
 
-int mau_pool_bn_bwd_reduce(const void* y, int ldy, const void* dpl, int lddpl, const unsigned short* argidx, const void* dskip, int lddskip, const float* scale,
-                           const float* shift, const float* mean, const float* invstd, float* slab, int ldslab, int dtype, int N, int H,
-                           int W, int C, mau_stream_t stream) {
+static int pool_bn_bwd_reduce_launch(const void* y, int ldy, const void* dpl, int lddpl, const unsigned short* argidx, const void* dskip, int lddskip,
+                                     const float* scale, const float* shift, const float* mean, const float* invstd, float* slab, int ldslab,
+                                     BwdSums fin, int dtype, int N, int H, int W, int C, mau_stream_t stream) {
   MAU_REQUIRE(y && (dpl || dskip) && (!dpl || argidx) && scale && shift && mean && invstd && slab && N > 0 && H >= 2 && W >= 2 && C > 0, "pool_bn_bwd_reduce: bad arguments");
   const int C8 = round_up(C, 8);
   MAU_REQUIRE(ldy % 8 == 0 && ldy >= C8 && (!dpl || (lddpl % 8 == 0 && lddpl >= C8)) && (!dskip || (lddskip % 8 == 0 && lddskip >= C8)) && ldslab >= C,
               "pool_bn_bwd_reduce: bad ld");
   const int64_t npix = (int64_t)N * H * W;
   dim3 grid(ceil_div(npix, BWD_PIX_PER_BLOCK), ceil_div(C, 64));
+  fin.chunks = reduce_chunks(grid.x);
 #define MAU_POOL_REDUCE(P, S)                                                                                                                  \
   MAU_DISPATCH_DTYPE(dtype, MAU_LAUNCH((pool_bn_bwd_reduce_kernel<T, P, S>), grid, dim3(256), 0, (hipStream_t)stream, (const T*)y, ldy, (const T*)dpl, \
-                                       lddpl, argidx, (const T*)dskip, lddskip, scale, shift, mean, invstd, slab, ldslab, H, W, npix, C))
+                                       lddpl, argidx, (const T*)dskip, lddskip, scale, shift, mean, invstd, slab, ldslab, H, W, npix, C, fin))
   if (dpl && dskip) MAU_POOL_REDUCE(true, true);
   else if (dpl) MAU_POOL_REDUCE(true, false);
   else MAU_POOL_REDUCE(false, true);
 #undef MAU_POOL_REDUCE
   return check_launch("pool_bn_bwd_reduce_kernel");
+}
+
+int mau_pool_bn_bwd_reduce(const void* y, int ldy, const void* dpl, int lddpl, const unsigned short* argidx, const void* dskip, int lddskip, const float* scale,
+                           const float* shift, const float* mean, const float* invstd, float* slab, int ldslab, int dtype, int N, int H,
+                           int W, int C, mau_stream_t stream) {
+  return pool_bn_bwd_reduce_launch(y, ldy, dpl, lddpl, argidx, dskip, lddskip, scale, shift, mean, invstd, slab, ldslab, BwdSums{}, dtype, N, H, W, C, stream);
+}
+
+int mau_pool_bn_bwd_reduce_sums(const void* y, int ldy, const void* dpl, int lddpl, const unsigned short* argidx, const void* dskip, int lddskip,
+                                const float* scale, const float* shift, const float* mean, const float* invstd, float* slab, int ldslab,
+                                double* sums, float* sums32, double* ws, unsigned* tickets, double append, int dtype, int N, int H, int W, int C,
+                                mau_stream_t stream) {
+  MAU_REQUIRE(sums && ws && tickets, "pool_bn_bwd_reduce_sums: bad arguments");
+  return pool_bn_bwd_reduce_launch(y, ldy, dpl, lddpl, argidx, dskip, lddskip, scale, shift, mean, invstd, slab, ldslab,
+                                   BwdSums{sums, sums32, ws, tickets, append, 0}, dtype, N, H, W, C, stream);
 }
 
 int mau_pool_bn_bwd_apply(const void* y, int ldy, const void* dpl, int lddpl, const unsigned short* argidx, const void* dskip, int lddskip, const float* scale,
@@ -648,9 +667,9 @@
   return check_launch("head_bn_fwd_kernel");
 }
 
-int mau_head_bn_bwd_reduce(const void* y, int ldy, const float* scale, const float* shift, const float* mean, const float* invstd,
-                           const float* w, const float* out, const float* dout, float* bn_slab, int ldslab, float* head_slab, int tanh0,
-                           int dtype, int N, int HW, int C, int Co, mau_stream_t stream) {
+static int head_bn_bwd_reduce_launch(const void* y, int ldy, const float* scale, const float* shift, const float* mean, const float* invstd,
+                                     const float* w, const float* out, const float* dout, float* bn_slab, int ldslab, float* head_slab, BwdSums fin,
+                                     int tanh0, int dtype, int N, int HW, int C, int Co, mau_stream_t stream) {
   MAU_REQUIRE(y && scale && shift && mean && invstd && w && out && dout && bn_slab && head_slab && N > 0 && HW > 0 && C > 0,
               "head_bn_bwd_reduce: bad arguments");
   MAU_REQUIRE(Co >= 1 && Co <= HEAD_MAX_CO && C <= mau_head_bn_max_channels(), "head_bn_bwd_reduce: out_channels in [1,%d], C <= %d", HEAD_MAX_CO,
@@ -659,15 +678,32 @@
   MAU_REQUIRE(ldy % 8 == 0 && ldy >= C8 && ldslab >= C, "head_bn_bwd_reduce: bad ld");
   MAU_REQUIRE(HW >= 32 && (int64_t)N * HW < ((int64_t)1 << 31), "head_bn_bwd_reduce: images of at least 32 pixels, fewer than 2^31 pixels in all");
   const int64_t npix = (int64_t)N * HW;
+  fin.chunks = reduce_chunks(ceil_div(npix, BWD_PIX_PER_BLOCK));
 #define MAU_HEAD_RED(MC_, EX_)                                                                                                              \
   MAU_DISPATCH_DTYPE(dtype, MAU_LAUNCH((head_bn_bwd_reduce_kernel<T, MC_, EX_>), dim3(ceil_div(npix, BWD_PIX_PER_BLOCK)), dim3(256), 0, (hipStream_t)stream, \
-                                       (const T*)y, ldy, scale, shift, mean, invstd, w, out, dout, bn_slab, ldslab, head_slab, tanh0, HW, C, C8, Co, npix))
+                                       (const T*)y, ldy, scale, shift, mean, invstd, w, out, dout, bn_slab, ldslab, head_slab, tanh0, HW, C, C8, Co, npix, fin))
   if (Co == 2) MAU_HEAD_RED(2, true);
   else if (Co == 1) MAU_HEAD_RED(2, false);
   else if (Co == HEAD_MAX_CO) MAU_HEAD_RED(HEAD_MAX_CO, true);
   else MAU_HEAD_RED(HEAD_MAX_CO, false);
 #undef MAU_HEAD_RED
   return check_launch("head_bn_bwd_reduce_kernel");
+}
+
+int mau_head_bn_bwd_reduce(const void* y, int ldy, const float* scale, const float* shift, const float* mean, const float* invstd,
+                           const float* w, const float* out, const float* dout, float* bn_slab, int ldslab, float* head_slab, int tanh0,
+                           int dtype, int N, int HW, int C, int Co, mau_stream_t stream) {
+  return head_bn_bwd_reduce_launch(y, ldy, scale, shift, mean, invstd, w, out, dout, bn_slab, ldslab, head_slab, BwdSums{}, tanh0, dtype, N, HW, C, Co,
+                                   stream);
+}
+
+int mau_head_bn_bwd_reduce_sums(const void* y, int ldy, const float* scale, const float* shift, const float* mean, const float* invstd,
+                                const float* w, const float* out, const float* dout, float* bn_slab, int ldslab, float* head_slab, double* sums,
+                                float* sums32, double* ws, unsigned* tickets, double append, int tanh0, int dtype, int N, int HW, int C, int Co,
+                                mau_stream_t stream) {
+  MAU_REQUIRE(sums && ws && tickets, "head_bn_bwd_reduce_sums: bad arguments");
+  return head_bn_bwd_reduce_launch(y, ldy, scale, shift, mean, invstd, w, out, dout, bn_slab, ldslab, head_slab,
+                                   BwdSums{sums, sums32, ws, tickets, append, 0}, tanh0, dtype, N, HW, C, Co, stream);
 }
 
 int mau_head_bn_bwd_apply(const void* y, int ldy, const float* scale, const float* shift, const float* mean, const float* invstd,
diff --git a/metadata-augmented-unet-for-lst-ndvi_amd/csrc/mau_common.h b/metadata-augmented-unet-for-lst-ndvi_amd/csrc/mau_common.h
--- a/metadata-augmented-unet-for-lst-ndvi_amd/csrc/mau_common.h
+++ b/metadata-augmented-unet-for-lst-ndvi_amd/csrc/mau_common.h
@@ -248,6 +248,106 @@
   return s_last != 0;
 }
 
+template <int G, typename Load>
+__device__ __forceinline__ void ordered_group(int& k, int end, Load load, double& s0, double& s1) {
+  for (; k + 8 * (G - 1) + 4 < end; k += 8 * G) {
+    double a[G], b[G];
+#pragma unroll
+    for (int i = 0; i < G; ++i) {
+      a[i] = load(k + 8 * i);
+      b[i] = load(k + 8 * i + 4);
+    }
+#pragma unroll
+    for (int i = 0; i < G; ++i) {
+      s0 += a[i];
+      s1 += b[i];
+    }
+  }
+}
+template <bool WIDE = true, typename Load>
+__device__ __forceinline__ void ordered_pair_sum(int first, int end, Load load, double& s0, double& s1) {
+  int k = first;
+#ifndef MAU_REDUCE_SERIAL
+  if constexpr (WIDE) ordered_group<16>(k, end, load, s0, s1);
+  ordered_group<4>(k, end, load, s0, s1);
+#endif
+  for (; k + 4 < end; k += 8) {
+    s0 += load(k);
+    s1 += load(k + 4);
+  }
+  if (k < end) s0 += load(k);
+}
+
+constexpr int REDUCE_MAX_CHUNKS = 128;
+static inline int reduce_chunks(int rows) {
+  int c = rows / 32;
+  if (c > REDUCE_MAX_CHUNKS) c = REDUCE_MAX_CHUNKS;
+  return c < 1 ? 1 : c;
+}
+
+struct BwdSums {
+  double* sums;
+  float* sums32;
+  double* part;
+  unsigned* tickets;
+  double append;
+  int chunks;
+};
+static inline size_t bn_bwd_tickets(int rows, int C) { return (size_t)((C + 63) / 64) * (reduce_chunks(rows) + 1); }
+
+__device__ __forceinline__ void bn_bwd_finish_sums(const float* slab, int ldslab, int C, const BwdSums& f, double* scr) {
+  const int rows = gridDim.x, chunks = f.chunks, M = 2 * C;
+  const int per = (rows + chunks - 1) / chunks;
+  const int k = blockIdx.x / per;
+  const int r0 = k * per, r1 = min(rows, r0 + per);
+  unsigned* tk = f.tickets + (size_t)blockIdx.y * (chunks + 1);
+  if (!last_block_of(tk + k, (unsigned)(r1 - r0))) return;
+  const int cl = threadIdx.x & 63, rl = threadIdx.x >> 6;
+  const int cc = blockIdx.y * 64 + cl;
+  auto join = [&](int which) { return scr[(which * 4 + 0) * 64 + cl] + scr[(which * 4 + 1) * 64 + cl] + scr[(which * 4 + 2) * 64 + cl] + scr[(which * 4 + 3) * 64 + cl]; };
+  auto emit = [&](int which, double v) {
+    f.sums[which * C + cc] = v;
+    if (f.sums32 != nullptr) f.sums32[which * C + cc] = (float)v;
+  };
+#pragma unroll 1
+  for (int which = 0; which < 2; ++which) {
+    double s0 = 0.0, s1 = 0.0;
+    if (cc < C && r0 + rl < r1)
+      ordered_pair_sum<false>(r0 + rl, r1, [&](int r) { return (double)slab[((size_t)r * 2 + which) * ldslab + cc]; }, s0, s1);
+    scr[(which * 4 + rl) * 64 + cl] = s0 + s1;
+  }
+  __syncthreads();
+  if (chunks == 1) {
+    if (rl < 2 && cc < C) emit(rl, join(rl));
+    if (f.append > 0.0 && blockIdx.y == 0 && threadIdx.x == 0) f.sums[M] = f.append;
+    return;
+  }
+  if (rl < 2 && cc < C) f.part[(size_t)k * M + rl * C + cc] = join(rl);
+  const int nz = (rows + per - 1) / per;
+  if (!last_block_of(tk + chunks, (unsigned)nz)) return;
+#pragma unroll 1
+  for (int which = 0; which < 2; ++which) {
+    double s0 = 0.0, s1 = 0.0;
+    if (cc < C && rl < chunks)
+      ordered_pair_sum<false>(rl, chunks, [&](int q) {
+        const double v = f.part[(size_t)(q < nz ? q : nz - 1) * M + which * C + cc];
+        return q < nz ? v : 0.0;
+      }, s0, s1);
+    scr[(which * 4 + rl) * 64 + cl] = s0 + s1;
+  }
+  __syncthreads();
+  if (rl < 2 && cc < C) emit(rl, join(rl));
+  if (f.append > 0.0 && blockIdx.y == 0 && threadIdx.x == 0) f.sums[M] = f.append;
+}
+
+__device__ __forceinline__ int bwd_apply_block(unsigned b, unsigned n) {
+#ifdef MAU_BWD_APPLY_ASCENDING
+  return (int)b;
+#else
+  return (int)(n - 1 - b);
+#endif
+}
+
 int head_fwd_fast(const void* a, int lda, const float* w, const float* b, float* out, int tanh0, int dtype, int64_t npix, int HW, int C, int Co,
                   hipStream_t stream);
 
diff --git a/metadata-augmented-unet-for-lst-ndvi_amd/functional.py b/metadata-augmented-unet-for-lst-ndvi_amd/functional.py
--- a/metadata-augmented-unet-for-lst-ndvi_amd/functional.py
+++ b/metadata-augmented-unet-for-lst-ndvi_amd/functional.py
@@ -114,6 +114,17 @@
     t = _TICKETS.get(key)
     if t is None:
         t = _TICKETS[key] = torch.zeros(lib.mau_reduce_tickets_elems(), dtype=torch.int32, device=dev)
+    return t
+
+
+_BWD_TICKETS = {}
+
+
+def _bwd_tickets(dev, elems: int) -> torch.Tensor:
+    key = (dev.index if dev.index is not None else torch.cuda.current_device(), _stream())
+    t = _BWD_TICKETS.get(key)
+    if t is None or t.numel() < elems:
+        t = _BWD_TICKETS[key] = torch.zeros(elems, dtype=torch.int32, device=dev)
     return t
 
 
@@ -265,6 +276,7 @@
 
 _OVERLAP_WGRAD = int(os.environ.get("MAU_OVERLAP_WGRAD", "2") or 0)
 _FUSED_REDUCE = True
+_FUSED_BWD_SUMS = True
 _FUSED_BN = True
 _FUSED_UP = True
 _PACK_MULTI = True
@@ -513,10 +525,21 @@
         dhw = dhb = None
         cptrs = (scale.data_ptr(), shift.data_ptr(), mean.data_ptr(), invstd.data_ptr())
 
+        own_sums = _FUSED_REDUCE and _FUSED_BWD_SUMS and not sync
+        ws = torch.empty(lib.mau_reduce_rows_ws_elems(rows, 2 * Cout), dtype=torch.float64, device=dev)
+
+        def reduce(name, args):
+            if own_sums:
+                tk = _bwd_tickets(dev, lib.mau_bn_bwd_tickets_elems(npix, Cout))
+                call(name + "_sums", *args[0], slab.data_ptr(), Cout, *args[1], sums.data_ptr(), g32.data_ptr(), ws.data_ptr(), tk.data_ptr(), 0.0,
+                     *args[2])
+            else:
+                call(name, *args[0], slab.data_ptr(), Cout, *args[1], *args[2])
+
         def finish_sums():
-            ws = torch.empty(lib.mau_reduce_rows_ws_elems(rows, 2 * Cout), dtype=torch.float64, device=dev)
-            call("mau_reduce_rows_f64_f32", slab.data_ptr(), rows, 2 * Cout, 2 * Cout, sums.data_ptr(), g32.data_ptr(), ws.data_ptr(),
-                 _tickets(dev).data_ptr() if (_FUSED_REDUCE or sync) else None, float(npix) if sync else 0.0, stream)
+            if not own_sums:
+                call("mau_reduce_rows_f64_f32", slab.data_ptr(), rows, 2 * Cout, 2 * Cout, sums.data_ptr(), g32.data_ptr(), ws.data_ptr(),
+                     _tickets(dev).data_ptr() if (_FUSED_REDUCE or sync) else None, float(npix) if sync else 0.0, stream)
             if not st.training:
                 return torch.zeros_like(sums), float(npix)
             if sync:
@@ -530,8 +553,8 @@
             dout = da.contiguous().float()
             hrows, rowlen = lib.mau_head_bwd_rows(N, H * W), lib.mau_head_bwd_rowlen(Cout, Co)
             hslab = torch.empty((hrows, rowlen), **f32)
-            call("mau_head_bn_bwd_reduce", y.data_ptr(), ldy, *cptrs, w2.data_ptr(), out.data_ptr(), dout.data_ptr(), slab.data_ptr(), Cout,
-                 hslab.data_ptr(), tanh0, code, N, H * W, Cout, Co, stream)
+            reduce("mau_head_bn_bwd_reduce", ((y.data_ptr(), ldy, *cptrs, w2.data_ptr(), out.data_ptr(), dout.data_ptr()), (hslab.data_ptr(),),
+                                              (tanh0, code, N, H * W, Cout, Co, stream)))
             sums_apply, count = finish_sums()
             red = torch.empty(rowlen, **f32)
             hws = torch.empty(lib.mau_reduce_rows_ws_elems(hrows, rowlen), dtype=torch.float64, device=dev)
@@ -547,7 +570,7 @@
             dsk = _as_nhwc(da) if da is not None else None
             pargs = (y.data_ptr(), ldy, dpl.data_ptr(), _ld(dpl), argidx.data_ptr(), dsk.data_ptr() if dsk is not None else None,
                      _ld(dsk) if dsk is not None else 0)
-            call("mau_pool_bn_bwd_reduce", *pargs, *cptrs, slab.data_ptr(), Cout, code, N, H, W, Cout, stream)
+            reduce("mau_pool_bn_bwd_reduce", ((*pargs, *cptrs), (), (code, N, H, W, Cout, stream)))
             sums_apply, count = finish_sums()
             call("mau_pool_bn_bwd_apply", *pargs, *cptrs, sums_apply.data_ptr(), count, dy.data_ptr(), ldy, code, N, H, W, Cout, stream)
         else:
@@ -588,7 +611,7 @@
             elif da is None:
                 da = torch.zeros((N, H, W, ldy), dtype=y.dtype, device=dev)
             da = _as_nhwc(da)
-            call("mau_bn_relu_bwd_reduce", da.data_ptr(), _ld(da), y.data_ptr(), ldy, *cptrs, slab.data_ptr(), Cout, code, npix, Cout, stream)
+            reduce("mau_bn_relu_bwd_reduce", ((da.data_ptr(), _ld(da), y.data_ptr(), ldy, *cptrs), (), (code, npix, Cout, stream)))
             sums_apply, count = finish_sums()
             call("mau_bn_relu_bwd_apply", da.data_ptr(), _ld(da), y.data_ptr(), ldy, *cptrs, sums_apply.data_ptr(), count, dy.data_ptr(), ldy,
                  code, npix, Cout, stream)
```

Result: slower. 2450 images/s (-4.2%).
